# FireMines/zk_stark_project

Hardware: AMD Instinct MI355X
Metric: STARK proofs/sec + prove-time ms, MiMC AIR 2^20-step trace (higher is better)
Workload: dtype f128 (u128 mod 2^128-45*2^40+1); 1 GPU; MiMC AIR 2^20-step trace, blowup=8 (BASELINE configs[1]); trace_length=1048576, trace_width=1, blowup=8, num_queries=40, grinding=21, fri_folding=16, fri_remainder_max_degree=7, parallelism=replicas1

## Files before the change

### __graft_entry__.py

```python
import os
import subprocess
import sys

ROOT = os.path.dirname(os.path.abspath(__file__))


def build() -> None:
    env = dict(os.environ)
    jobs = str(min(16, os.cpu_count() or 1))
    subprocess.check_call(["make", "-j", jobs, "-C", os.path.join(ROOT, "zk_stark_project_amd", "csrc")], env=env)
    subprocess.check_call(["make", "-j", jobs, "-C", os.path.join(ROOT, "oracle")], env=env)
    subprocess.check_call(["make", "-j", jobs, "-C", os.path.join(ROOT, "tests", "native")], env=env)
    subprocess.check_call(["make", "-j", jobs, "-C", os.path.join(ROOT, "tests", "native"), "-f", "deep_inv_check.mk"],
                          env=env)
    subprocess.check_call(["make", "-j", jobs, "-C", os.path.join(ROOT, "tests", "native"), "-f",
                           "column_degrees_check.mk"], env=env)
    if ROOT not in sys.path:
        sys.path.insert(0, ROOT)
    import zk_stark_project_amd
    from zk_stark_project_amd import _native
    _native.load()


def smoke() -> None:
    for p in (ROOT, os.path.join(ROOT, "tests")):
        if p not in sys.path:
            sys.path.insert(0, p)
    from zk_stark_project_amd import AIR_MIMC, MimcProver, ProofOptions, _native
    from zk_stark_project_amd.field import to_bytes
    import oracle_ref

    ctx = _native.Context(0)
    opts = ProofOptions(40, 8, 12)
    prover = MimcProver(opts, ctx)
    n = 1 << 12
    trace = prover.build_trace(42 * 10**6, n)
    pub = prover.get_pub_inputs(trace).to_elements()
    proof = prover.prove(trace)
    ref, _ = oracle_ref.prove(AIR_MIMC, trace.to_bytes(), 1, n, to_bytes(pub), opts)
    assert proof.to_bytes() == ref, "GPU proof differs from the CPU oracle"
    assert oracle_ref.verify(AIR_MIMC, proof.to_bytes(), to_bytes(pub), opts) == 0, "proof rejected"
    _native.verify(AIR_MIMC, proof.to_bytes(), pub, opts)
    ctx.close()
    print(f"smoke ok: MiMC 2^12 proof, {len(proof)} bytes, bit-exact vs oracle")


if __name__ == "__main__":
    build()
    if len(sys.argv) > 1 and sys.argv[1] == "smoke":
        smoke()
```

### zk_stark_project_amd/csrc/abi.cpp

```cpp
#include "prover_internal.hpp"

#include <mutex>

using namespace zkpi;

namespace {
bool device_is_gfx950(int device) {
  static std::mutex mu;
  static std::map<int, bool> known;
  std::lock_guard<std::mutex> lk(mu);
  auto it = known.find(device);
  if (it != known.end()) return it->second;
  hipDeviceProp_t prop;
  if (hipGetDeviceProperties(&prop, device) != hipSuccess) return false;
  const bool ok = strncmp(prop.gcnArchName, "gfx950", 6) == 0;
  known[device] = ok;
  return ok;
}

constexpr uint32_t TU_STATE = TU_W / 2;

int tu_build(zkp_ctx* ctx, const zkp_training_client* cl, uint32_t K, uint64_t bs, uint64_t n) {
  HIP_CHECK(hipSetDevice(ctx->device));
  ctx->err.clear();
// ... 63 lines not shown
  const TuClient* dcl = (const TuClient*)dp;
  const felt* dinit = (const felt*)(dp + off_init);
  if (bs)
    launch_tu_states(ctx->prof, ctx->stream, dcl, K, dinit, (const felt*)(dp + off_batch), ds, (uint32_t)bs,
                     inv(felt_u64(TU_AC * 1000000ull)));
  const felt* states = bs ? ds : dinit;
  launch_tu_write(ctx->prof, ctx->stream, dcl, K, states, bs, n, dfl);
  bool want_fl = false, want_raw = false;
  for (uint32_t k = 0; k < K; k++) {
    want_fl |= cl[k].first_last != nullptr;
    want_raw |= cl[k].raw_states != nullptr;
  }
  const size_t fl_bytes = (size_t)K * 2 * TU_STATE * 16, raw_bytes = (size_t)K * (bs + 1) * TU_STATE * 16;
  uint8_t* hp = (uint8_t*)ctx->pinned((want_fl ? fl_bytes : 0) + (want_raw ? raw_bytes : 0));
  uint8_t* hraw = hp + (want_fl ? fl_bytes : 0);
  if (want_fl) HIP_CHECK(hipMemcpyAsync(hp, dfl, fl_bytes, hipMemcpyDeviceToHost, ctx->stream));
  if (want_raw) HIP_CHECK(hipMemcpyAsync(hraw, states, raw_bytes, hipMemcpyDeviceToHost, ctx->stream));
  ctx->sync();
  for (uint32_t k = 0; k < K; k++) {
    if (cl[k].first_last) memcpy(cl[k].first_last, hp + (size_t)k * 2 * TU_STATE * 16, 2 * TU_STATE * 16);
    if (cl[k].raw_states)
      memcpy(cl[k].raw_states, hraw + (size_t)k * (bs + 1) * TU_STATE * 16, (bs + 1) * TU_STATE * 16);
  }
  ctx->collect_prof();
  ctx->free_retired();
  return 0;
}
}

extern "C" {

int zkp_ctx_create(int device, zkp_ctx** out) {
  if (!out) return ZKP_ERR_ARGUMENT;
  *out = nullptr;
  using clk = std::chrono::steady_clock;
  auto t = clk::now();
  std::vector<std::pair<const char*, double>> phases;
  auto lap = [&](const char* name) {
    const auto now = clk::now();
    phases.emplace_back(name, std::chrono::duration<double, std::milli>(now - t).count());
    t = now;
  };
  int count = 0;
  if (hipGetDeviceCount(&count) != hipSuccess || count <= device || device < 0) return ZKP_ERR_DEVICE;
  if (hipSetDevice(device) != hipSuccess) return ZKP_ERR_DEVICE;
  if (!device_is_gfx950(device)) return ZKP_ERR_DEVICE;
  lap("host_ctx_device_check");
  zkp_ctx* c = new_ctx(device);
  if (!c) return ZKP_ERR_DEVICE;
  lap("host_ctx_streams");
  preload_kernels_module();
  preload_merkle_module();
  preload_ntt_module();
  lap("host_ctx_code_objects");
  try {
    c->pinned(1u << 20);
    lap("host_ctx_pinned");
    const felt zero[1]{};
    c->upload(c->buf<felt>("ring_warm", 1), zero, 16);
    drain_streams(c);
    lap("host_ctx_first_copy");
  } catch (const ZkpFail& f) {
    delete c;
    return f.code;
  }
  for (auto& ph : phases) {
    auto& st = c->stats[ph.first];
    st.launches += 1;
    st.ms += ph.second;
  }
  *out = c;
  return ZKP_OK;
}

void zkp_ctx_destroy(zkp_ctx* ctx) {
  if (!ctx) return;
  (void)hipSetDevice(ctx->device);
  for (zkp_ctx* sc : ctx->session_pool) {
    drain_streams(sc);
    delete sc;
  }
  ctx->session_pool.clear();
  drain_streams(ctx);
  delete ctx;
}

int zkp_ctx_trim(zkp_ctx* ctx) {
  if (!ctx) return ZKP_ERR_ARGUMENT;
  (void)hipSetDevice(ctx->device);
  for (zkp_ctx* sc : ctx->session_pool) {
    drain_streams(sc);
    delete sc;
  }
  ctx->session_pool.clear();
  return ZKP_OK;
}

const char* zkp_last_error(const zkp_ctx* ctx) { return ctx ? ctx->err.c_str() : "null context"; }

void zkp_free(void* p) { free(p); }

int zkp_device_alloc(zkp_ctx* ctx, uint64_t bytes, void** d_ptr) {
  return guarded(ctx, [&] {
    if (!d_ptr) return (int)ZKP_ERR_ARGUMENT;
    HIP_CHECK(hipSetDevice(ctx->device));
    HIP_CHECK(hipMalloc(d_ptr, bytes ? bytes : 16));
    ctx->user_allocs.push_back(*d_ptr);
    return 0;
  });
}

int zkp_device_free(zkp_ctx* ctx, void* d_ptr) {
  return guarded(ctx, [&] {
    auto it = std::find(ctx->user_allocs.begin(), ctx->user_allocs.end(), d_ptr);
    if (it == ctx->user_allocs.end()) return (int)ZKP_ERR_ARGUMENT;
    ctx->user_allocs.erase(it);
    HIP_CHECK(hipFree(d_ptr));
    return 0;
  });
}

int zkp_copy_to_device(zkp_ctx* ctx, void* d_dst, const void* h_src, uint64_t bytes) {
  return guarded(ctx, [&] {
    HIP_CHECK(hipMemcpyAsync(d_dst, h_src, bytes, hipMemcpyHostToDevice, ctx->stream));
    ctx->sync();
    return 0;
  });
}

int zkp_copy_to_host(zkp_ctx* ctx, void* h_dst, const void* d_src, uint64_t bytes) {
  return guarded(ctx, [&] {
    ctx->download(h_dst, d_src, bytes);
    return 0;
  });
}

int zkp_trace_lde_commit(zkp_ctx* ctx, const zkp_felt* trace, uint32_t w, uint64_t n, uint32_t blowup,
                         zkp_felt* lde_out, uint8_t root[32]) {
  return guarded(ctx, [&] {
    HIP_CHECK(hipSetDevice(ctx->device));
    if (!trace || !root) return (int)ZKP_ERR_ARGUMENT;
    if (n < 8 || (n & (n - 1)) || w == 0 || w > 255) return (int)ZKP_ERR_TRACE_SHAPE;
    if (blowup < 2 || (blowup & (blowup - 1)) || blowup > 128) return (int)ZKP_ERR_INVALID_OPTIONS;
    uint32_t logn = ilog2(n), logB = ilog2(blowup);
    if (logn + logB > MAX_LOG_DOMAIN) return (int)ZKP_ERR_TRACE_SHAPE;
    uint64_t N = n * blowup;
    felt* d = ctx->buf<felt>("trace_in", (size_t)w * n);
    ctx->upload(d, trace, (size_t)w * n * 16);
    felt* coef = ctx->buf<felt>("coef", (size_t)w * n);
    felt* lde = ctx->buf<felt>("tlde", (size_t)w * N);
    ctx->ensure_coset(logn, logB, 1);
    const uint32_t logN = logn + logB;
    NttBatch ib{d, coef, nullptr, n, n, 1, 1, w};
    launch_ntt(ctx->prof, ctx->stream, ib, logn, false, ctx->itws(logN), logN);
    NttBatch lb{coef, lde, ctx->S(logn, logB), n, n, blowup, blowup, w * blowup};
    launch_ntt(ctx->prof, ctx->stream, lb, logn, true, ctx->tws(logN), logN);
    TreeShard tr;
    commit_rows(ctx, ctx->self_comm(), 0, lde, n, w, logB, logn, false, "ttree", tr, root);
    if (lde_out) {
      std::vector<felt> h((size_t)w * N);
      ctx->download(h.data(), lde, h.size() * 16);
      for (uint32_t c = 0; c < w; c++)
        for (uint64_t i = 0; i < N; i++) {
          felt v = h[((size_t)c * blowup + (i & (blowup - 1))) * n + (i >> logB)];
          lde_out[(size_t)c * N + i].lo = v.lo;
          lde_out[(size_t)c * N + i].hi = v.hi;
        }
    }
    ctx->collect_prof();
    return 0;
  });
}

int zkp_merkle_commit_rows(zkp_ctx* ctx, const zkp_felt* cols, uint32_t w, uint64_t rows, uint8_t root[32]) {
  return guarded(ctx, [&] {
    HIP_CHECK(hipSetDevice(ctx->device));
    if (!cols || !root) return (int)ZKP_ERR_ARGUMENT;
    if (rows < 2 || (rows & (rows - 1)) || w == 0 || w > 255) return (int)ZKP_ERR_TRACE_SHAPE;
    felt* d = ctx->buf<felt>("mrows", (size_t)w * rows);
    ctx->upload(d, cols, (size_t)w * rows * 16);
    uint32_t* tree = ctx->buf<uint32_t>("mtree", (size_t)16 * rows);
    launch_merkle_lde(ctx->prof, ctx->stream, d, w, 0, rows, tree, rows);
    ctx->download(root, tree + 8, 32);
    ctx->collect_prof();
    return 0;
  });
}

int zkp_grind(zkp_ctx* ctx, const uint8_t seed[32], uint32_t bits, uint64_t* nonce) {
  return guarded(ctx, [&] {
    HIP_CHECK(hipSetDevice(ctx->device));
    if (!seed || !nonce || bits > 64) return (int)ZKP_ERR_ARGUMENT;
    uint32_t sw[8];
    for (int i = 0; i < 8; i++)
      sw[i] = (uint32_t)seed[4 * i] | ((uint32_t)seed[4 * i + 1] << 8) | ((uint32_t)seed[4 * i + 2] << 16) |
              ((uint32_t)seed[4 * i + 3] << 24);
    unsigned long long* dres = ctx->buf<unsigned long long>("grind_res", 1);
    uint32_t* dseed = ctx->buf<uint32_t>("grind_seed", 8);
    ctx->upload(dseed, sw, 32);
    HIP_CHECK(hipMemsetAsync(dres, 0xff, 8, ctx->stream));
    unsigned long long res = ~0ull;
    for (uint64_t base = 1; base <= (1ull << 40) && res == ~0ull; base += 1ull << 32) {
      launch_grind_all(ctx->prof, ctx->stream, dseed, base, base + (1ull << 32) - 1, bits, dres);
      ctx->download(&res, dres, 8);
    }
    if (res == ~0ull) return (int)ZKP_ERR_NONCE;
    *nonce = res;
    ctx->collect_prof();
    return 0;
  });
}

int zkp_build_global_update_trace(zkp_ctx* ctx, const zkp_felt* raw_global, const zkp_felt* blinding,
                                  const zkp_felt* local_updates, uint64_t ndev, zkp_felt k, uint64_t n,
                                  void* d_trace_out, zkp_felt* final_state) {
  return guarded(ctx, [&] {
    HIP_CHECK(hipSetDevice(ctx->device));
    if (!raw_global || !blinding || !d_trace_out || (ndev && !local_updates)) return (int)ZKP_ERR_ARGUMENT;
    if (n < 8 || (n & (n - 1)) || n < ndev + 2) return (int)ZKP_ERR_TRACE_SHAPE;
    const felt kf = make(k.lo, k.hi);
    if (ge_p(kf)) return (int)ZKP_ERR_PUB_INPUTS;
    auto canon = [](const zkp_felt* v, uint64_t cnt) {
      for (uint64_t i = 0; i < cnt; i++)
        if (ge_p(make(v[i].lo, v[i].hi))) return false;
      return true;
    };
    if (!canon(raw_global, GU_D) || !canon(blinding, GU_D) || !canon(local_updates, ndev * GU_D))
      return (int)ZKP_ERR_ARGUMENT;
    std::vector<felt> hm(2 * GU_D);
    for (uint32_t c = 0; c < GU_D; c++) {
      hm[c] = add(make(raw_global[c].lo, raw_global[c].hi), make(blinding[c].lo, blinding[c].hi));
      hm[GU_D + c] = make(raw_global[c].lo, raw_global[c].hi);
    }
    felt* dm = ctx->buf<felt>("gu_masked_raw", 2 * GU_D);
    ctx->upload(dm, hm.data(), hm.size() * 16);
    felt* dl = ctx->buf<felt>("gu_local", ndev ? ndev * GU_D : 1);
    if (ndev) HIP_CHECK(hipMemcpyAsync(dl, local_updates, ndev * GU_D * 16, hipMemcpyHostToDevice, ctx->stream));
    const uint64_t tiles = (n + 4095) / 4096;
    felt* tb = ctx->buf<felt>("gu_tiles", tiles * GU_D);
    launch_gu_trace(ctx->prof, ctx->stream, dm, dm + GU_D, dl, ndev, inv(kf), n, tb, (felt*)d_trace_out);
    if (final_state)
      HIP_CHECK(hipMemcpy2DAsync(final_state, 16, (const felt*)d_trace_out + ndev + 1, n * 16, 16, GU_D,
                                 hipMemcpyDeviceToHost, ctx->stream));
    ctx->sync();
    ctx->collect_prof();
    return 0;
  });
}

int zkp_build_training_update_trace(zkp_ctx* ctx, const zkp_felt* initial_state, const zkp_felt* x_batch,
                                    const zkp_felt* x_sign, const zkp_felt* y_batch, uint64_t bs,
                                    zkp_felt learning_rate, zkp_felt precision, const uint64_t* masks, uint64_t n,
                                    void* d_trace_out, zkp_felt* first_last, zkp_felt* raw_states) {
  return guarded(ctx, [&] {
    if (!masks) return (int)ZKP_ERR_ARGUMENT;
    zkp_training_client c{};
    c.initial_state = initial_state;
    c.x_batch = x_batch;
    c.x_sign = x_sign;
    c.y_batch = y_batch;
    c.learning_rate = learning_rate;
    c.precision = precision;
    c.masks = masks;
    c.d_trace_out = d_trace_out;
    c.first_last = first_last;
    c.raw_states = raw_states;
    return tu_build(ctx, &c, 1, bs, n);
  });
}

int zkp_build_training_update_traces(zkp_ctx* ctx, const zkp_training_client* clients, uint32_t num_clients,
                                     uint64_t bs, uint64_t n) {
  return guarded(ctx, [&] {
    if (!clients || num_clients == 0 || num_clients > ZKP_TU_MAX_CLIENTS) {
      ctx->err = "clients must be non-null and 1.." + std::to_string(ZKP_TU_MAX_CLIENTS) + " in number";
      return (int)ZKP_ERR_ARGUMENT;
    }
    return tu_build(ctx, clients, num_clients, bs, n);
  });
}

int zkp_pcg64_masks(const uint64_t state[2], const uint64_t inc[2], uint64_t first_index, uint64_t count,
                    uint64_t* out) {
  if (!state || !inc || (count && !out)) return ZKP_ERR_ARGUMENT;
  pcg::u128 s{state[0], state[1]}, a{pcg::MUL_LO, pcg::MUL_HI}, c{inc[0], inc[1]};
  const pcg::u128 step_a = a, step_c = c;
  for (uint64_t k = first_index; k; k >>= 1) {
    if (k & 1) s = pcg::affine(s, a, c);
    c = pcg::mul(c, pcg::add(a, {1, 0}));
    a = pcg::mul(a, a);
  }
  for (uint64_t i = 0; i < count; i++) {
    s = pcg::affine(s, step_a, step_c);
    out[i] = pcg::out(s);
  }
  return ZKP_OK;
}

int zkp_set_profiling(zkp_ctx* ctx, int enabled) {
  return guarded(ctx, [&] {
    ctx->prof.enabled = enabled != 0;
    return 0;
  });
}

int zkp_set_profiling_kernel(zkp_ctx* ctx, const char* kernel_name) {
  return guarded(ctx, [&] {
    ctx->prof.only = kernel_name ? kernel_name : "";
    return 0;
// ... 40 lines not shown
}

int zkp_air_check_trace_device_pub(zkp_ctx* ctx, int air_id, const zkp_felt* pub_elems, uint64_t n_pub,
                                   const void* d_trace_cols, uint32_t width, uint64_t n, uint64_t* bad_row,
                                   uint32_t* bad_constraint, uint32_t* bad_assertion) {
  if (!ctx || !d_trace_cols || !bad_row || !bad_constraint || !bad_assertion || (n_pub && !pub_elems))
    return ZKP_ERR_ARGUMENT;
  return guarded(ctx, [&] {
    if (air_id == ZKP_AIR_MIMC || air_id == ZKP_AIR_GLOBAL_UPDATE || air_id == ZKP_AIR_TRAINING_UPDATE)
      return (int)ZKP_ERR_UNSUPPORTED_AIR;
    if (n < 8 || (n & (n - 1)) || width == 0 || width > 255) return (int)ZKP_ERR_TRACE_SHAPE;
    AirDesc air;
    std::vector<felt> pub(n_pub);
    for (uint64_t i = 0; i < n_pub; i++) pub[i] = make(pub_elems[i].lo, pub_elems[i].hi);
    const int rc = build_air(air, air_id, width, n, pub);
    if (rc) return rc;
    if (!air.prog->num_pub && n_pub) return (int)ZKP_ERR_PUB_INPUTS;
    if (n > (1ull << MAX_LOG_TRACE)) return (int)ZKP_ERR_TRACE_SHAPE;
    const airp::Program& pr = *air.prog;
    HIP_CHECK(hipSetDevice(ctx->device));
    const ProgCodeLayout lay(pr, 1);
    const size_t A = pr.a_col.size(), o_col = lay.end();
    static_assert(sizeof(ProgStridedCells) == 48, "three 16-byte units");
    const std::vector<airp::Strided>& sv = pr.strided;
    const size_t S = sv.size();
    size_t seq_felts = 0;
    for (const airp::Strided& a : sv) seq_felts += a.pub < 0 ? a.values.size() : 0;
    const size_t o_step = o_col + (A + 3) / 4, o_val = o_step + (A + 3) / 4, o_sdesc = o_val + A,
                 o_svals = o_sdesc + 3 * S, total = o_svals + seq_felts;
    uint64_t strided_blocks = 0;
    for (const airp::Strided& a : sv) strided_blocks += (n / a.stride + 63) / 64;
    felt* dimg = ctx->buf<felt>("check_image", total);
    std::vector<felt>& tag = ctx->host_cache["check_image_tag"];
    const felt want = make((uint64_t)air_id | (S ? n << 32 : 0), total);
    if (tag.size() != 1 || !eq(tag[0], want)) {
      tag.clear();
      std::vector<felt> img(total, zero());
      lay.write(img.data());
      for (size_t p = 0; p < pr.periodic.size(); p++)
        memcpy(img.data() + lay.tab[p], pr.periodic[p].data(), pr.periodic[p].size() * 16);
      uint32_t* steps = reinterpret_cast<uint32_t*>(img.data() + o_step);
      for (size_t k = 0; k < A; k++) steps[k] = (uint32_t)pr.a_step[k];
      if (A) {
        memcpy(img.data() + o_col, pr.a_col.data(), A * 4);
        if (!pr.num_pub) memcpy(img.data() + o_val, pr.a_val.data(), A * 16);
      }
      ProgStridedCells* cells = reinterpret_cast<ProgStridedCells*>(img.data() + o_sdesc);
      uint32_t blk = 0, voff = 0;
      for (size_t j = 0; j < S; j++) {
        const uint32_t count = (uint32_t)(n / sv[j].stride);
        const bool bound = sv[j].pub >= 0;
        cells[j] = ProgStridedCells{sv[j].col, (uint32_t)sv[j].first, (uint32_t)sv[j].stride, count, blk,
                                    sv[j].sequence() ? voff : 0xffffffffu, bound ? (uint32_t)sv[j].pub + 1 : 0, 0,
                                    bound ? zero() : sv[j].val};
        if (sv[j].sequence() && !bound) {
          memcpy(img.data() + o_svals + voff, sv[j].values.data(), (size_t)count * 16);
          voff += count;
        }
        blk += (count + 63) / 64;
      }
      ctx->upload(dimg, img.data(), total * 16);
      if (total * 16 > (1u << 20)) ctx->sync();
      tag.assign(1, want);
    }
    ProgCheckArgs ca{};
    ca.code = lay.code(dimg);
    ca.nassert = (uint32_t)A;
    ca.a_col = reinterpret_cast<const uint32_t*>(dimg + o_col);
    ca.a_step = reinterpret_cast<const uint32_t*>(dimg + o_step);
    ca.a_val = dimg + o_val;
    if (pr.num_pub) {
      felt* dpub = ctx->buf<felt>("check_pub", pr.num_pub);
      ctx->upload(dpub, pr.pub.data(), (size_t)pr.num_pub * 16);
      ca.code.pub = dpub;
      felt* dval = ctx->buf<felt>("check_aval", A);
      if (A) ctx->upload(dval, pr.a_val.data(), A * 16);
      ca.a_val = dval;
    }
    ca.n = n;
    ca.nstrided = (uint32_t)S;
    ca.sdesc = reinterpret_cast<const ProgStridedCells*>(dimg + o_sdesc);
    ca.svals = dimg + o_svals;
    unsigned long long* dres = ctx->buf<unsigned long long>("check_result", 2);
    HIP_CHECK(hipMemsetAsync(dres, 0xff, 16, ctx->stream));
    launch_check_program(ctx->prof, ctx->stream, ca, width, (const felt*)d_trace_cols, dres, strided_blocks);
    unsigned long long res[2];
    ctx->download(res, dres, 16);
    ctx->collect_prof();
    ctx->free_retired();
    *bad_row = UINT64_MAX;
    *bad_constraint = UINT32_MAX;
    *bad_assertion = UINT32_MAX;
    if (res[0] != ~0ull) {
      *bad_row = res[0] >> 10;
      *bad_constraint = (uint32_t)(res[0] & 1023);
    } else if (res[1] != ~0ull) {
      *bad_row = res[1] & 0xffffffffull;
      *bad_assertion = (uint32_t)(res[1] >> 32);
    }
    return 0;
  });
}

int zkp_air_constraint_degrees_device(zkp_ctx* ctx, int air_id, const zkp_felt* pub_elems, uint64_t n_pub,
                                      const void* d_trace_cols, uint32_t width, uint64_t n, uint64_t* degrees,
                                      uint32_t capacity, zkp_air_degree_report* report) {
  return guarded(ctx, [&] {
    if (!d_trace_cols || !degrees || !report || (n_pub && !pub_elems)) {
      ctx->err = "d_trace_cols, degrees, report or (with n_pub set) pub_elems: null";
      return (int)ZKP_ERR_ARGUMENT;
    }
    DegreesPlan pl;
    const int rc = degrees_plan(air_id, pub_elems, n_pub, width, n, pl, ctx->err);
    if (rc) return rc;
    const airp::Program& pr = *pl.air.prog;
    if (capacity < pr.num_t) {
      ctx->err = "capacity: below num_constraints (" + std::to_string(pr.num_t) + ")";
      return (int)ZKP_ERR_ARGUMENT;
    }
    HIP_CHECK(hipSetDevice(ctx->device));
    const uint32_t E = pl.E, logE = ilog2(E), logn = ilog2(n), logN = logn + logE;
    const uint64_t M = n * E;
    ctx->ensure_coset(logn, logE, logE);
    const ProgCodeLayout lay(pr, E);
    const size_t total = lay.end();
    felt* dimg = ctx->buf<felt>("deg_image", total);
    std::vector<felt>& tag = ctx->host_cache["deg_image_tag"];
    const felt want[2] = {make((uint64_t)air_id, logn), make(logE, total)};
    if (tag.size() != 2 || !eq(tag[0], want[0]) || !eq(tag[1], want[1])) {
      tag.clear();
      std::vector<felt> img(total, zero());
      lay.write(img.data());
      const felt g = felt_u64(3);
      for (size_t p = 0; p < pr.periodic.size(); p++) {
        const size_t cyc = pr.periodic[p].size();
        std::vector<felt> kc = pr.periodic[p];
        host_interpolate(kc, one());
        const std::vector<felt> kv = host_evaluate(kc, cyc * E, pow_u64(g, n / cyc));
        memcpy(img.data() + lay.tab[p], kv.data(), kv.size() * 16);
      }
      ctx->upload(dimg, img.data(), total * 16);
      if (total * 16 > (1u << 20)) ctx->sync();
      tag.assign(want, want + 2);
    }
    ProgCode code = lay.code(dimg);
    if (pr.num_pub) {
      felt* dpub = ctx->buf<felt>("deg_pub", pr.num_pub);
      ctx->upload(dpub, pr.pub.data(), (size_t)pr.num_pub * 16);
      code.pub = dpub;
    }
    felt* coef = ctx->buf<felt>("deg_coef", (size_t)width * n);
    felt* ext = ctx->buf<felt>("deg_ext", (size_t)width * M);
    NttBatch ib{(const felt*)d_trace_cols, coef, nullptr, n, n, 1, 1, width};
    launch_ntt(ctx->prof, ctx->stream, ib, logn, false, ctx->itws(logN), logN);
    NttBatch lb{coef, ext, ctx->S(logn, logE), n, n, E, E, width * E};
    launch_ntt(ctx->prof, ctx->stream, lb, logn, true, ctx->tws(logN), logN);
    const std::string dkey = "deg_dft_" + std::to_string(logn) + "_" + std::to_string(logE);
    felt* dcoefs = ctx->buf<felt>(dkey + "_coefs", (size_t)E + E / 2);
    uint32_t* dblk = ctx->buf<uint32_t>(dkey + "_blk", E);
    if (!ctx->have_cached(dkey)) {
      const std::vector<felt> dc = comp_dft_consts(n, logE, E);
      std::vector<uint32_t> blk(E);
      for (uint32_t u = 0; u < E; u++) blk[u] = u;
      ctx->upload(dcoefs, dc.data(), dc.size() * 16);
      ctx->upload(dblk, blk.data(), blk.size() * 4);
    }
    const uint32_t K = std::min(pl.K, pr.num_t);
    felt* vals = ctx->buf<felt>("deg_vals", (size_t)K * M);
    felt* cf = ctx->buf<felt>("deg_coefs", (size_t)K * M);
    long long* ddeg = ctx->buf<long long>("deg_result", pr.num_t);
    HIP_CHECK(hipMemsetAsync(ddeg, 0xff, (size_t)pr.num_t * 8, ctx->stream));
    for (uint32_t i0 = 0; i0 < pr.num_t; i0 += K) {
      const uint32_t k = std::min(K, pr.num_t - i0);
      launch_program_columns(ctx->prof, ctx->stream, code, ext, width, logn, logE, i0, k, vals);
      NttBatch cb{vals, vals, nullptr, n, n, 1, 1, k * E};
      launch_ntt(ctx->prof, ctx->stream, cb, logn, false, ctx->itws(logN), logN);
      for (uint32_t c = 0; c < k; c++)
        launch_comp_dft(ctx->prof, ctx->stream, vals + (size_t)c * M, dblk, ctx->Si(logn, logE, logE), dcoefs, E, E,
                        logn, 0, n, cf + (size_t)c * M);
      launch_column_degrees(ctx->prof, ctx->stream, cf, logn, logE, k, ddeg + i0);
    }
    std::vector<uint64_t> h(pr.num_t);
    ctx->download(h.data(), ddeg, (size_t)pr.num_t * 8);
    ctx->collect_prof();
    ctx->free_retired();
    zkp_air_degree_report r{};
    r.num_constraints = pr.num_t;
    r.eval_blowup = E;
    r.columns = pl.air.comp_cols();
    r.max_degree = ZKP_DEGREE_ZERO;
    r.first_under = UINT32_MAX;
    for (uint32_t i = 0; i < pr.num_t; i++) {
      degrees[i] = h[i];
      if (h[i] == ZKP_DEGREE_ZERO) continue;
      if (r.max_degree == ZKP_DEGREE_ZERO || h[i] > r.max_degree) r.max_degree = h[i];
      if (r.first_under == UINT32_MAX && h[i] > (uint64_t)pr.degrees[i] * (n - 1)) r.first_under = i;
    }
    r.columns_needed = 1;
    r.proof_fits = 1;
    if (r.max_degree != ZKP_DEGREE_ZERO) {
      if (r.max_degree + 2 > n) r.columns_needed = (uint32_t)((r.max_degree + 2 - n + n - 1) / n);
      if (r.columns_needed < 1) r.columns_needed = 1;
      r.proof_fits = r.max_degree <= ((uint64_t)r.columns + 1) * n - 2;
    }
    *report = r;
    return 0;
  });
}

int zkp_build_mimc_trace(const uint8_t seed[16], uint64_t n, zkp_felt* out) {
  if (!seed || !out || n == 0) return ZKP_ERR_ARGUMENT;
  felt v = from_u128_bytes(seed);
  if (ge_p(v)) v = sub(v, make(P_LO, P_HI));
  for (uint64_t i = 0; i < n; i++) {
    out[i].lo = v.lo;
    out[i].hi = v.hi;
    felt u = add(v, felt_u64((i % 64 + 1) * 1000000ull));
    felt u2 = sqr(u), u3 = mul(u2, u), u6 = sqr(u3);
    v = mul(u6, u);
  }
  return 0;
}

}
```

### zk_stark_project_amd/csrc/felt_dev.hpp

```cpp
#pragma once
#include <stdint.h>

#define ZKP_ASM asm

namespace fpd {

__device__ __forceinline__ uint32_t add_co(uint32_t a, uint32_t b, uint64_t& co) {
  uint32_t r;
  ZKP_ASM("v_add_co_u32_e64 %0, %1, %2, %3" : "=v"(r), "=s"(co) : "v"(a), "v"(b));
  return r;
}
__device__ __forceinline__ uint32_t addc_co(uint32_t a, uint32_t b, uint64_t ci, uint64_t& co) {
  uint32_t r;
  ZKP_ASM("v_addc_co_u32_e64 %0, %1, %2, %3, %4" : "=v"(r), "=s"(co) : "v"(a), "v"(b), "s"(ci));
  return r;
}
__device__ __forceinline__ uint32_t addc(uint32_t a, uint32_t b, uint64_t ci) {
  uint32_t r;
  uint64_t dead;
  ZKP_ASM("v_addc_co_u32_e64 %0, %1, %2, %3, %4" : "=v"(r), "=s"(dead) : "v"(a), "v"(b), "s"(ci));
  return r;
}
__device__ __forceinline__ uint32_t sub_co(uint32_t a, uint32_t b, uint64_t& bo) {
  uint32_t r;
// ... 244 lines not shown
  const uint64_t u = mul_wide(r4, 0x2d00u);
  uint64_t c, b;
  const uint32_t s1 = add_co(r1, (uint32_t)u, c);
  const uint32_t s2 = addc_co(r2, (uint32_t)(u >> 32), c, c);
  const uint32_t s3 = addc_co_0(r3, c, c);
  const uint32_t z0 = sub_co(r0, r4, b);
  const uint32_t z1 = subb_co_0(s1, b, b);
  const uint32_t z2 = subb_co_0(s2, b, b);
  const uint32_t z3 = subb_co_0(s3, b, b);
  uint64_t kk;
  ZKP_ASM("s_andn2_b64 %0, %1, %2" : "=s"(kk) : "s"(c), "s"(b) : "scc");
  return canon_rare(z0, z1, z2, z3, kk);
}


__device__ __forceinline__ void mul256x2(L4 x, L4 y, L4 u, L4 v, uint32_t r[8], uint32_t s[8]) {
  uint64_t acc, c, bcc, d;
  uint32_t ov, bov;
  acc = mul_wide(x.w0, y.w0);
  bcc = mul_wide(u.w0, v.w0);
  r[0] = (uint32_t)acc; acc >>= 32;
  s[0] = (uint32_t)bcc; bcc >>= 32;
#define ZKP_COL_BEGIN(i0, j0)                      \
  acc = mad_co(x.w##i0, y.w##j0, acc, c);          \
  bcc = mad_co(u.w##i0, v.w##j0, bcc, d);          \
  ov = carry_0(c);                                 \
  bov = carry_0(d);
#define ZKP_COL_STEP(i0, j0)                       \
  acc = mad_co(x.w##i0, y.w##j0, acc, c);          \
  bcc = mad_co(u.w##i0, v.w##j0, bcc, d);          \
  ov = addc_0(ov, c);                              \
  bov = addc_0(bov, d);
#define ZKP_COL_END(k)                             \
  r[k] = (uint32_t)acc;                            \
  s[k] = (uint32_t)bcc;                            \
  acc = (acc >> 32) | ((uint64_t)ov << 32);        \
  bcc = (bcc >> 32) | ((uint64_t)bov << 32);
  ZKP_COL_BEGIN(0, 1) ZKP_COL_STEP(1, 0) ZKP_COL_END(1)
  ZKP_COL_BEGIN(0, 2) ZKP_COL_STEP(1, 1) ZKP_COL_STEP(2, 0) ZKP_COL_END(2)
  ZKP_COL_BEGIN(0, 3) ZKP_COL_STEP(1, 2) ZKP_COL_STEP(2, 1) ZKP_COL_STEP(3, 0) ZKP_COL_END(3)
  ZKP_COL_BEGIN(1, 3) ZKP_COL_STEP(2, 2) ZKP_COL_STEP(3, 1) ZKP_COL_END(4)
  ZKP_COL_BEGIN(2, 3) ZKP_COL_STEP(3, 2) ZKP_COL_END(5)
#undef ZKP_COL_BEGIN
#undef ZKP_COL_STEP
#undef ZKP_COL_END
  acc = mad(x.w3, y.w3, acc);
  bcc = mad(u.w3, v.w3, bcc);
  r[6] = (uint32_t)acc; r[7] = (uint32_t)(acc >> 32);
  s[6] = (uint32_t)bcc; s[7] = (uint32_t)(bcc >> 32);
}

__device__ __forceinline__ void reduce_x2_core(const uint32_t r[8], const uint32_t s[8], uint32_t z[4], uint32_t Z[4],
                                               uint64_t& k1, uint64_t& k2) {
  const uint32_t K = 0x2d00u;
  uint64_t t = mul_wide(r[4], K), tt = mul_wide(s[4], K);
  uint32_t q0 = (uint32_t)t, p0 = (uint32_t)tt;
  t = mad(r[5], K, t >> 32); tt = mad(s[5], K, tt >> 32);
  uint32_t q1 = (uint32_t)t, p1 = (uint32_t)tt;
  t = mad(r[6], K, t >> 32); tt = mad(s[6], K, tt >> 32);
  uint32_t q2 = (uint32_t)t, p2 = (uint32_t)tt;
  t = mad(r[7], K, t >> 32); tt = mad(s[7], K, tt >> 32);
  uint32_t q3 = (uint32_t)t, q4 = (uint32_t)(t >> 32), p3 = (uint32_t)tt, p4 = (uint32_t)(tt >> 32);
  uint64_t c, e, b, f;
  uint32_t s1 = add_co(r[1], q0, c);
  uint32_t S1 = add_co(s[1], p0, e);
  uint32_t x0 = sub_co(r[0], r[4], b);
  uint32_t X0 = sub_co(s[0], s[4], f);
  uint32_t s2 = addc_co(r[2], q1, c, c);
  uint32_t S2 = addc_co(s[2], p1, e, e);
  uint32_t x1 = subb_co(s1, r[5], b, b);
  uint32_t X1 = subb_co(S1, s[5], f, f);
  uint32_t s3 = addc_co(r[3], q2, c, c);
  uint32_t S3 = addc_co(s[3], p2, e, e);
  uint32_t x2 = subb_co(s2, r[6], b, b);
  uint32_t X2 = subb_co(S2, s[6], f, f);
  uint32_t s4 = addc_co_0(q3, c, c);
  uint32_t S4 = addc_co_0(p3, e, e);
  uint32_t x3 = subb_co(s3, r[7], b, b);
  uint32_t X3 = subb_co(S3, s[7], f, f);
  uint32_t s5 = addc_0(q4, c);
  uint32_t S5 = addc_0(p4, e);
  uint32_t x4 = subb_co_0(s4, b, b);
  uint32_t X4 = subb_co_0(S4, f, f);
  uint32_t x5 = subb_0(s5, b);
  uint32_t X5 = subb_0(S5, f);
  uint64_t uu = mul_wide(x4, K), UU = mul_wide(X4, K);
  uint32_t u0 = (uint32_t)uu, U0 = (uint32_t)UU;
  uint32_t u1 = (uint32_t)(uu >> 32) + x5 * K, U1 = (uint32_t)(UU >> 32) + X5 * K;
  uint32_t y1 = add_co(x1, u0, c);
  uint32_t Y1 = add_co(X1, U0, e);
  z[0] = sub_co(x0, x4, b);
  Z[0] = sub_co(X0, X4, f);
  uint32_t y2 = addc_co(x2, u1, c, c);
  uint32_t Y2 = addc_co(X2, U1, e, e);
  z[1] = subb_co(y1, x5, b, b);
  Z[1] = subb_co(Y1, X5, f, f);
  uint32_t y3 = addc_co_0(x3, c, c);
  uint32_t Y3 = addc_co_0(X3, e, e);
  z[2] = subb_co_0(y2, b, b);
  Z[2] = subb_co_0(Y2, f, f);
  z[3] = subb_co_0(y3, b, b);
  Z[3] = subb_co_0(Y3, f, f);
  ZKP_ASM("s_andn2_b64 %0, %1, %2" : "=s"(k1) : "s"(c), "s"(b) : "scc");
  ZKP_ASM("s_andn2_b64 %0, %1, %2" : "=s"(k2) : "s"(e), "s"(f) : "scc");
}

__device__ __forceinline__ void reduce_x2(const uint32_t r[8], const uint32_t s[8], felt& out_r, felt& out_s) {
  uint32_t z[4], Z[4];
  uint64_t k1, k2;
  reduce_x2_core(r, s, z, Z, k1, k2);
  const uint64_t rare = k1 | k2 | __builtin_amdgcn_ballot_w64(max(z[3], Z[3]) == 0xffffffffu);
  if (rare) {
    out_r = canon_from(z[0], z[1], z[2], z[3], k1);
    out_s = canon_from(Z[0], Z[1], Z[2], Z[3], k2);
  } else {
    out_r = join(z[0], z[1], z[2], z[3]);
    out_s = join(Z[0], Z[1], Z[2], Z[3]);
  }
}

__device__ __forceinline__ void mul_x2(felt a, felt b, felt c, felt d, felt& ab, felt& cd) {
  uint32_t r[8], s[8];
  mul256x2(split(a), split(b), split(c), split(d), r, s);
  reduce_x2(r, s, ab, cd);
}

struct Rare {
  uint64_t k = 0;
  uint32_t top = 0;
  __device__ __forceinline__ bool any() const { return (k | __builtin_amdgcn_ballot_w64(top == 0xffffffffu)) != 0; }
};

__device__ __forceinline__ felt mul_z(felt a, felt b, Rare& q) {
  uint32_t r[8], z0, z1, z2, z3;
  uint64_t k;
  mul256(split(a), split(b), r);
  reduce_core(r, z0, z1, z2, z3, k);
  q.k |= k;
  q.top = max(q.top, z3);
  return join(z0, z1, z2, z3);
}

__device__ __forceinline__ void mul_x2_z(felt a, felt b, felt c, felt d, felt& ab, felt& cd, Rare& q) {
  uint32_t r[8], s[8], z[4], Z[4];
  uint64_t k1, k2;
  mul256x2(split(a), split(b), split(c), split(d), r, s);
  reduce_x2_core(r, s, z, Z, k1, k2);
  q.k |= k1 | k2;
  q.top = max(q.top, max(z[3], Z[3]));
  ab = join(z[0], z[1], z[2], z[3]);
  cd = join(Z[0], Z[1], Z[2], Z[3]);
}

__device__ __forceinline__ felt add_z(felt a, felt b, Rare& q) {
  L4 x = split(a), y = split(b);
  uint64_t c, g;
  const uint32_t s0 = add_co(x.w0, y.w0, c);
  const uint32_t s1 = addc_co(x.w1, y.w1, c, c);
  const uint32_t s2 = addc_co(x.w2, y.w2, c, c);
  const uint32_t s3 = addc_co(x.w3, y.w3, c, c);
  q.top = max(q.top, s3);
  const uint32_t m0 = sel_0_m1(c), m1 = m0 & C1;
  const uint32_t t0 = add_co(s0, m0, g);
  const uint32_t t1 = addc_co(s1, m1, g, g);
  const uint32_t t2 = addc_co_0(s2, g, g);
  const uint32_t t3 = addc_0(s3, g);
  return join(t0, t1, t2, t3);
}
}
```

### zk_stark_project_amd/csrc/kernels_common.hpp

```cpp
#pragma once
#include "../../include/zkp.h"
#include "zkp_internal.hpp"
#include "blake3.hpp"

#include <algorithm>
#include <type_traits>

using namespace fp;

#define TPB 256

#define LAUNCH(prof, name, stream, bytes, ...)                 \
  do {                                                          \
    (prof).begin(name, stream, (double)(bytes));                \
    __VA_ARGS__;                                                \
    (prof).end(stream);                                         \
  } while (0)

#if defined(__HIP_DEVICE_COMPILE__)
using Rare = fpd::Rare;
#else
struct Rare {
  bool any() const { return false; }
};
#endif

template <bool FAST>
__device__ __forceinline__ felt dmul(felt a, felt b, Rare& q) {
#if defined(__HIP_DEVICE_COMPILE__)
  if constexpr (FAST) return fpd::mul_z(a, b, q);
#endif
  (void)q;
  return mul(a, b);
}
template <bool FAST>
__device__ __forceinline__ felt dadd(felt a, felt b, Rare& q) {
#if defined(__HIP_DEVICE_COMPILE__)
  if constexpr (FAST) return fpd::add_z(a, b, q);
#endif
  (void)q;
  return add(a, b);
}

namespace kc {

template <bool FAST>
__device__ __forceinline__ uint32_t opaque_tid() {
  uint32_t t = threadIdx.x;
  if constexpr (!FAST) asm volatile("" : "+v"(t));
  return t;
}

__device__ __forceinline__ uint32_t rev_bits(uint32_t x, uint32_t bits) {
  return bits == 0 ? 0u : (__brev(x) >> (32 - bits));
}

template <int B, int E, typename F>
__device__ __forceinline__ void static_for(F&& f) {
  if constexpr (B < E) {
    f(std::integral_constant<int, B>{});
    static_for<B + 1, E>(f);
  }
}

constexpr int ilog2_const(int v) { return v <= 1 ? 0 : 1 + ilog2_const(v / 2); }
constexpr int rev_const(int x, int bits) { return bits == 0 ? 0 : ((x & 1) << (bits - 1)) | rev_const(x >> 1, bits - 1); }

inline uint32_t ilog2_u64(uint64_t v) {
  uint32_t l = 0;
  while ((1ull << l) < v) l++;
  return l;
}

}
```

### zk_stark_project_amd/csrc/ntt.hip

```cpp
#include "kernels_common.hpp"
#include "ntt_plan.hpp"

#include <mutex>

using kc::static_for;
using kc::rev_bits;

namespace {

struct NttKArgs {
  const felt* src;
  felt* dst;
  const felt* scale;
  const felt* tw;
  uint64_t src_stride, dst_stride;
  uint32_t src_div, scale_mod;
  uint32_t logn, s0, K, lo, T, Tl, logT, logTl, dit;
};

__global__ __launch_bounds__(TPB) void k_ntt_pass(NttKArgs a) {
  extern __shared__ felt lds[];
  const uint32_t bidx = blockIdx.y;
  const felt* src = a.src + (uint64_t)(bidx / a.src_div) * a.src_stride;
  felt* dst = a.dst + (uint64_t)bidx * a.dst_stride;
  const felt* scale = a.scale ? a.scale + ((uint64_t)(bidx % a.scale_mod) << a.logn) : nullptr;
  const uint32_t K = a.K, T = a.T, Tl = a.Tl, lo = a.lo;
  const uint32_t E = T << K;
  const uint64_t g0 = (uint64_t)blockIdx.x * T;
  const uint64_t hi0 = g0 >> lo;
  const uint64_t l0 = (Tl == T) ? (g0 & ((1ull << lo) - 1)) : 0;
  const uint32_t qmask = (1u << K) - 1;

  for (uint32_t e = threadIdx.x; e < E; e += TPB) {
    uint32_t ll = e & (Tl - 1);
    uint32_t rest = e >> a.logTl;
    uint32_t q = rest & qmask;
    uint32_t hl = rest >> K;
    uint64_t addr = ((hi0 + hl) << (lo + K)) + ((uint64_t)q << lo) + l0 + ll;
    felt v = src[addr];
    if (scale) v = mul(v, scale[addr]);
    lds[(q << a.logT) + (hl * Tl) + ll] = v;
  }
  __syncthreads();
  for (uint32_t ls = 0; ls < K; ls++) {
    const uint32_t s = a.s0 + ls;
    const uint32_t pbit = a.dit ? ls : (K - 1 - ls);
    const uint32_t lev = a.dit ? s : (a.logn - 1 - s);
    const felt* twl = a.tw + ((1ull << lev) - 1);
    const uint32_t pmask = (1u << pbit) - 1;
    for (uint32_t bf = threadIdx.x; bf < (E >> 1); bf += TPB) {
      uint32_t gg = bf & (T - 1);
      uint32_t qq = bf >> a.logT;
      uint32_t q = ((qq >> pbit) << (pbit + 1)) | (qq & pmask);
      uint32_t q2 = q | (1u << pbit);
      uint64_t l = l0 + (gg & (Tl - 1));
      uint64_t j = ((uint64_t)(q & pmask) << lo) | l;
      felt w = twl[j];
      uint32_t i0 = (q << a.logT) + gg, i1 = (q2 << a.logT) + gg;
      felt x = lds[i0], y = lds[i1];
      if (a.dit) {
        felt t = mul(y, w);
        lds[i0] = add(x, t);
        lds[i1] = sub(x, t);
      } else {
        lds[i0] = add(x, y);
        lds[i1] = mul(sub(x, y), w);
      }
    }
    __syncthreads();
  }
  for (uint32_t e = threadIdx.x; e < E; e += TPB) {
    uint32_t ll = e & (Tl - 1);
    uint32_t rest = e >> a.logTl;
    uint32_t q = rest & qmask;
    uint32_t hl = rest >> K;
    uint64_t addr = ((hi0 + hl) << (lo + K)) + ((uint64_t)q << lo) + l0 + ll;
    dst[addr] = lds[(q << a.logT) + (hl * Tl) + ll];
  }
}

struct Ntt8Args {
  const felt* src;
  felt* dst;
  const felt* scale;
  const felt* tw;
  uint64_t src_stride, dst_stride;
  uint32_t src_div, scale_mod;
  uint32_t logn, s0, K, lo, logT, logTl;
  uint32_t tile_major;
};

template <bool DIT>
__device__ __forceinline__ felt ntt_tw(const Ntt8Args& a, uint32_t j, uint32_t pbit) {
  uint32_t s = DIT ? a.s0 + pbit : a.s0 + a.K - 1 - pbit;
  uint32_t lev = DIT ? s : a.logn - 1 - s;
  return a.tw[((1u << lev) - 1) + j];
}

#ifdef ZKP_NTT_NOGMEM
#define NTT_LD(p) (make((uint64_t)(uintptr_t)(p), (uint64_t)threadIdx.x))
#define NTT_ST(p, v)                                               \
  do {                                                            \
    const felt v_ = (v);                                          \
    if (v_.lo == 0x123456789ull && v_.hi == 0xabcdefull) *(p) = v_; \
  } while (0)
#else
#define NTT_LD(p) (*(p))
#define NTT_ST(p, v) (*(p) = (v))
#endif

#ifdef ZKP_NTT_NOBFLY
template <bool FAST>
__device__ __forceinline__ felt bmul(felt a, felt b, Rare& q) { return make(a.lo ^ b.lo, a.hi ^ b.hi); }
template <bool FAST>
__device__ __forceinline__ felt badd(felt a, felt b, Rare& q) { return make(a.lo + b.lo, a.hi + b.hi); }
__device__ __forceinline__ felt nsub(felt a, felt b) { return make(a.lo - b.lo, a.hi - b.hi); }
#else
template <bool FAST>
__device__ __forceinline__ felt bmul(felt a, felt b, Rare& q) { return dmul<FAST>(a, b, q); }
template <bool FAST>
__device__ __forceinline__ felt badd(felt a, felt b, Rare& q) { return dadd<FAST>(a, b, q); }
__device__ __forceinline__ felt nsub(felt a, felt b) { return sub(a, b); }
#endif

template <bool DIT, bool FAST>
__device__ __forceinline__ void bfly(felt& x, felt& y, felt w, Rare& q) {
  if (DIT) {
    felt t = bmul<FAST>(y, w, q);
    y = nsub(x, t);
    x = badd<FAST>(x, t, q);
  } else {
    felt d = nsub(x, y);
    x = badd<FAST>(x, y, q);
    y = bmul<FAST>(d, w, q);
  }
}

template <bool DIT, bool FAST>
__device__ __forceinline__ void bfly1(felt& x, felt& y, Rare& q) {
  felt d = nsub(x, y);
  x = badd<FAST>(x, y, q);
  y = d;
}

#ifdef ZKP_COUNT_REDO
__device__ unsigned long long zkp_ntt_redo_waves[5];
#define ZKP_NTT_REDO_TAKEN(site)                                                       \
  do {                                                                                 \
    if ((threadIdx.x & 63) == 0) atomicAdd(&zkp_ntt_redo_waves[site], 1ull);           \
  } while (0)
#else
#define ZKP_NTT_REDO_TAKEN(site) \
  do {                           \
  } while (0)
#endif

template <int K>
struct NttRounds {
  static constexpr int n = (K + 2) / 3;
  static constexpr int bits(int r) {
    int rem = K;
    for (int i = 0; i < r; i++) {
      int left = n - i;
      int b = (rem + left - 1) / left;
      rem -= b > 3 ? 3 : b;
    }
    int left = n - r;
    int b = (rem + left - 1) / left;
    return b > 3 ? 3 : b;
  }
};

template <bool DIT, bool FAST>
__device__ __forceinline__ void bfly2(felt& x0, felt& y0, felt w0, felt& x1, felt& y1, felt w1, Rare& q) {
#if defined(__HIP_DEVICE_COMPILE__) && !defined(ZKP_NTT_NOBFLY)
  auto mx2 = [&](felt a, felt b, felt c, felt d, felt& ab, felt& cd) {
    if constexpr (FAST) fpd::mul_x2_z(a, b, c, d, ab, cd, q);
    else fpd::mul_x2(a, b, c, d, ab, cd);
  };
  if (DIT) {
    felt t0, t1;
    mx2(y0, w0, y1, w1, t0, t1);
    y0 = sub(x0, t0); x0 = badd<FAST>(x0, t0, q);
    y1 = sub(x1, t1); x1 = badd<FAST>(x1, t1, q);
  } else {
    felt d0 = sub(x0, y0), d1 = sub(x1, y1);
    x0 = badd<FAST>(x0, y0, q); x1 = badd<FAST>(x1, y1, q);
    mx2(d0, w0, d1, w1, y0, y1);
  }
#else
  bfly<DIT, FAST>(x0, y0, w0, q);
  bfly<DIT, FAST>(x1, y1, w1, q);
#endif
}

template <bool DIT, int NT, int KC, bool SMALL>
__device__ __forceinline__ void ntt8_tile(const Ntt8Args& a, uint32_t bidx, uint32_t tile, felt* lds) {
  constexpr int E = NT * 8;
  constexpr uint32_t K = KC;
  constexpr uint32_t LOGNT = NT == 512 ? 9 : 8;
  constexpr uint32_t logT = LOGNT + 3 - KC;
  constexpr uint32_t T = 1u << logT;
  static_assert(T == 1 || T >= 4, "the LDS swizzles take rows of 1 or >= 4 felts");
  const uint32_t Tl = 1u << a.logTl, lo = a.lo;
  auto lidx = [](uint32_t q, uint32_t x) -> uint32_t {
    if constexpr (T == 1) {
      (void)x;
      return q ^ ((q >> 3) & 7u) ^ (((q >> 6) & 1u) << 3);
    } else if constexpr (T >= 32) {
      return q * T + (x ^ (q & 15u));
    } else if constexpr (T == 16 && DIT) {
      return q * T + (x ^ (q & 7u));
    } else if constexpr (T == 16) {
      return q * T + (x ^ ((q & 7u) | ((((q >> 2) ^ (q >> 4)) & 1u) << 3)));
    } else if constexpr (T == 8) {
      return (q ^ (((q >> 2) ^ (q >> 3)) & 1u)) * T + (x ^ (q & 7u));
    } else {
      const uint32_t b1 = (q >> 1) & 1u, b23 = ((q >> 2) ^ (q >> 3)) & 1u, b25 = ((q >> 2) ^ (q >> 5)) & 1u;
      return (q ^ (b23 | (b25 << 1))) * T + (x ^ (b1 | (b23 << 1)));
    }
  };
  const felt* src = a.src + (uint64_t)(bidx / a.src_div) * a.src_stride;
  felt* dst = a.dst + (uint64_t)bidx * a.dst_stride;
  const felt* scale = a.scale ? a.scale + ((uint64_t)(bidx % a.scale_mod) << a.logn) : nullptr;
  const uint64_t g0 = (uint64_t)tile << logT;
  const uint32_t hi0 = (uint32_t)(g0 >> lo);
  const uint32_t l0 = (Tl == T) ? (uint32_t)(g0 & ((1ull << lo) - 1)) : 0;
  const uint32_t qmask = (1u << K) - 1;
  const uint32_t tid = threadIdx.x;

  auto gaddr = [&](uint32_t gg, uint32_t q) -> uint32_t {
    uint32_t hl = gg >> a.logTl, ll = gg & (Tl - 1);
    return ((hi0 + hl) << (lo + K)) + (q << lo) + l0 + ll;
  };
  (void)qmask;
  const bool staged = a.logTl < (T >= 8 ? 3u : 2u);
  auto staged_elem = [&](uint32_t e, uint32_t& slot) -> uint32_t {
    uint32_t ll = e & (Tl - 1), rest = e >> a.logTl;
    uint32_t q = rest & ((1u << K) - 1), hl = rest >> K;
    slot = lidx(q, hl * Tl + ll);
    return ((hi0 + hl) << (lo + K)) + (q << lo) + l0 + ll;
  };
  if (staged) {
    auto stage_in = [&](auto fast_c, Rare& q) {
      constexpr bool FAST = decltype(fast_c)::value;
#pragma unroll
      for (int i = 0; i < 8; i++) {
        uint32_t slot;
        uint32_t ad = staged_elem(tid + i * NT, slot);
        felt v = NTT_LD(src + ad);
        if (scale) v = bmul<FAST>(v, NTT_LD(scale + ad), q);
        lds[slot] = v;
      }
    };
    Rare q;
    stage_in(std::true_type{}, q);
    if (scale && q.any()) {
      ZKP_NTT_REDO_TAKEN(0);
      stage_in(std::false_type{}, q);
    }
    __syncthreads();
  }
  uint32_t b0 = DIT ? 0 : K;
  static_for<0, NttRounds<KC>::n>([&](auto rr) {
    constexpr int r = decltype(rr)::value;
    constexpr uint32_t rb = NttRounds<KC>::bits(r);
    if (!DIT) b0 -= rb;
    constexpr bool first = r == 0, last = r + 1 == NttRounds<KC>::n;
    if (!first) __syncthreads();
    felt x[8];
    uint32_t ggs[2], qlow[2];
    auto coord_gg = [&](int m, uint32_t tr) { return ((uint32_t)(m >> rb) << LOGNT | tr) & (T - 1); };
    auto coord_q = [&](int m, uint32_t tr) {
      uint32_t extra = m >> rb, bf = m & ((1u << rb) - 1);
      uint32_t qo = ((extra << LOGNT) | tr) >> logT;
      uint32_t ql = qo & ((1u << b0) - 1);
      return ((qo >> b0) << (b0 + rb)) | (bf << b0) | ql;
    };
    auto round = [&](auto fast_c, Rare& qq) {
    constexpr bool FAST = decltype(fast_c)::value;
    uint32_t tr = tid;
    if constexpr (!FAST) asm volatile("" : "+v"(tr));
    const uint32_t zo = tr - tid;
#pragma unroll
    for (int m = 0; m < 8; m++) {
      uint32_t extra = m >> rb, bf = m & ((1u << rb) - 1);
      uint32_t c = (extra << LOGNT) | tr;
      if (first && !staged) {
        uint32_t ad = gaddr(coord_gg(m, tr), coord_q(m, tr));
        felt v = NTT_LD(src + ad);
        if (scale) v = bmul<FAST>(v, NTT_LD(scale + ad), qq);
        x[m] = v;
      } else {
        x[m] = lds[lidx(coord_q(m, tr), coord_gg(m, tr))];
      }
      if (bf == 0 && extra < 2) { ggs[extra] = c & (T - 1); qlow[extra] = (c >> logT) & ((1u << b0) - 1); }
    }
    if constexpr (rb == 3) {
      const uint32_t l = l0 + (ggs[0] & (Tl - 1));
      const uint32_t jb = (qlow[0] << lo) | l;
      const uint32_t jstep = 1u << (b0 + lo);
      constexpr bool smallest = SMALL && (DIT ? first : last);
      if constexpr (DIT && smallest) {
        bfly1<true, FAST>(x[0], x[1], qq); bfly1<true, FAST>(x[2], x[3], qq); bfly1<true, FAST>(x[4], x[5], qq); bfly1<true, FAST>(x[6], x[7], qq);
        const felt w1 = ntt_tw<true>(a, 1 + zo, 1);
        bfly1<true, FAST>(x[0], x[2], qq); bfly1<true, FAST>(x[4], x[6], qq);
        bfly2<true, FAST>(x[1], x[3], w1, x[5], x[7], w1, qq);
        const felt w21 = ntt_tw<true>(a, 1 + zo, 2), w22 = ntt_tw<true>(a, 2 + zo, 2), w23 = ntt_tw<true>(a, 3 + zo, 2);
        bfly1<true, FAST>(x[0], x[4], qq);
        bfly2<true, FAST>(x[1], x[5], w21, x[2], x[6], w22, qq);
        bfly<true, FAST>(x[3], x[7], w23, qq);
      } else if constexpr (!DIT && smallest) {
        const felt w21 = ntt_tw<false>(a, 1 + zo, 2), w22 = ntt_tw<false>(a, 2 + zo, 2), w23 = ntt_tw<false>(a, 3 + zo, 2);
        bfly1<false, FAST>(x[0], x[4], qq);
        bfly2<false, FAST>(x[1], x[5], w21, x[2], x[6], w22, qq);
        bfly<false, FAST>(x[3], x[7], w23, qq);
        const felt w1 = ntt_tw<false>(a, 1 + zo, 1);
        bfly1<false, FAST>(x[0], x[2], qq); bfly1<false, FAST>(x[4], x[6], qq);
        bfly2<false, FAST>(x[1], x[3], w1, x[5], x[7], w1, qq);
        bfly1<false, FAST>(x[0], x[1], qq); bfly1<false, FAST>(x[2], x[3], qq); bfly1<false, FAST>(x[4], x[5], qq); bfly1<false, FAST>(x[6], x[7], qq);
      } else if constexpr (DIT) {
        {
          felt w0 = ntt_tw<true>(a, jb, b0);
          bfly2<true, FAST>(x[0], x[1], w0, x[2], x[3], w0, qq); bfly2<true, FAST>(x[4], x[5], w0, x[6], x[7], w0, qq);
        }
        {
          felt w1a = ntt_tw<true>(a, jb, b0 + 1);
          felt w1b = ntt_tw<true>(a, jb | jstep, b0 + 1);
          bfly2<true, FAST>(x[0], x[2], w1a, x[1], x[3], w1b, qq); bfly2<true, FAST>(x[4], x[6], w1a, x[5], x[7], w1b, qq);
        }
        static_for<0, 2>([&](auto k2) {
          felt w2a = ntt_tw<true>(a, jb | ((uint32_t)(2 * k2) << (b0 + lo)), b0 + 2);
          felt w2b = ntt_tw<true>(a, jb | ((uint32_t)(2 * k2 + 1) << (b0 + lo)), b0 + 2);
          bfly2<true, FAST>(x[2 * k2], x[2 * k2 + 4], w2a, x[2 * k2 + 1], x[2 * k2 + 5], w2b, qq);
        });
      } else {
        static_for<0, 2>([&](auto k2) {
          felt w2a = ntt_tw<false>(a, jb | ((uint32_t)(2 * k2) << (b0 + lo)), b0 + 2);
          felt w2b = ntt_tw<false>(a, jb | ((uint32_t)(2 * k2 + 1) << (b0 + lo)), b0 + 2);
          bfly2<false, FAST>(x[2 * k2], x[2 * k2 + 4], w2a, x[2 * k2 + 1], x[2 * k2 + 5], w2b, qq);
        });
        {
          felt w1a = ntt_tw<false>(a, jb, b0 + 1);
          felt w1b = ntt_tw<false>(a, jb | jstep, b0 + 1);
          bfly2<false, FAST>(x[0], x[2], w1a, x[1], x[3], w1b, qq); bfly2<false, FAST>(x[4], x[6], w1a, x[5], x[7], w1b, qq);
        }
        {
          felt w0 = ntt_tw<false>(a, jb, b0);
          bfly2<false, FAST>(x[0], x[1], w0, x[2], x[3], w0, qq); bfly2<false, FAST>(x[4], x[5], w0, x[6], x[7], w0, qq);
        }
      }
    } else if constexpr (rb == 2) {
      if constexpr (!DIT && SMALL && last) {
        const felt w1 = ntt_tw<false>(a, 1 + zo, 1);
#pragma unroll
        for (int u = 0; u < 2; u++) {
          felt* y = x + 4 * u;
          bfly1<false, FAST>(y[0], y[2], qq);
          bfly<false, FAST>(y[1], y[3], w1, qq);
          bfly1<false, FAST>(y[0], y[1], qq); bfly1<false, FAST>(y[2], y[3], qq);
        }
      } else {
#pragma unroll
      for (int u = 0; u < 2; u++) {
        const uint32_t l = l0 + (ggs[u] & (Tl - 1));
        const uint32_t jb = (qlow[u] << lo) | l;
        felt w0 = ntt_tw<DIT>(a, jb, b0);
        felt w1a = ntt_tw<DIT>(a, jb, b0 + 1), w1b = ntt_tw<DIT>(a, jb | (1u << (b0 + lo)), b0 + 1);
        felt* y = x + 4 * u;
        if (DIT) {
          bfly2<true, FAST>(y[0], y[1], w0, y[2], y[3], w0, qq);
          bfly2<true, FAST>(y[0], y[2], w1a, y[1], y[3], w1b, qq);
        } else {
          bfly2<false, FAST>(y[0], y[2], w1a, y[1], y[3], w1b, qq);
          bfly2<false, FAST>(y[0], y[1], w0, y[2], y[3], w0, qq);
        }
      }
      }
    } else {
#pragma unroll
      for (int u = 0; u < 4; u++) {
        uint32_t c = ((uint32_t)u << LOGNT) | tr;
        uint32_t gg = c & (T - 1);
        uint32_t ql = (c >> logT) & ((1u << b0) - 1);
        const uint32_t jb = (ql << lo) | (l0 + (gg & (Tl - 1)));
        bfly<DIT, FAST>(x[2 * u], x[2 * u + 1], ntt_tw<DIT>(a, jb, b0), qq);
      }
    }
    };
    Rare qq;
    round(std::true_type{}, qq);
    if (qq.any()) {
      ZKP_NTT_REDO_TAKEN(1 + r);
      round(std::false_type{}, qq);
    }
    if (!last || staged) __syncthreads();
#pragma unroll
    for (int m = 0; m < 8; m++) {
      if (last && !staged) NTT_ST(dst + gaddr(coord_gg(m, tid), coord_q(m, tid)), x[m]);
      else lds[lidx(coord_q(m, tid), coord_gg(m, tid))] = x[m];
    }
    if (DIT) b0 += rb;
  });
  if (staged) {
    __syncthreads();
#pragma unroll
    for (int i = 0; i < 8; i++) {
      uint32_t slot;
      uint32_t ad = staged_elem(tid + i * NT, slot);
      NTT_ST(dst + ad, lds[slot]);
    }
  }
  (void)E;
}

template <bool DIT, int NT, int KC, bool SMALL>
__global__ __launch_bounds__(NT, (NT == 256 && KC == 11) ? 5 : 1) void k_ntt8(Ntt8Args a) {
  extern __shared__ felt lds[];
  uint32_t bidx = blockIdx.x, tile = blockIdx.y;
  if (a.tile_major) {
    const uint32_t B = gridDim.x, i = blockIdx.y * B + blockIdx.x, k = i >> 3;
    tile = (k / B) * 8 + (i & 7);
    bidx = k % B;
  }
  ntt8_tile<DIT, NT, KC, SMALL>(a, bidx, tile, lds);
}

}

void preload_ntt_module() {
  hipFuncAttributes fa;
  (void)hipFuncGetAttributes(&fa, (const void*)k_ntt_pass);
}

#ifdef ZKP_COUNT_REDO
void zkp_ntt_redo_waves_take(unsigned long long out[5]) {
  const unsigned long long z[5] = {0, 0, 0, 0, 0};
  (void)hipMemcpyFromSymbol(out, HIP_SYMBOL(zkp_ntt_redo_waves), sizeof z);
  (void)hipMemcpyToSymbol(HIP_SYMBOL(zkp_ntt_redo_waves), z, sizeof z);
}
int zkp_ntt_round_bits(int K, int r) {
  switch (K) {
#define ZKP_ROUND_BITS(KK) \
  case KK:                 \
    return r < NttRounds<KK>::n ? NttRounds<KK>::bits(r) : 0;
    ZKP_ROUND_BITS(6) ZKP_ROUND_BITS(7) ZKP_ROUND_BITS(8) ZKP_ROUND_BITS(9) ZKP_ROUND_BITS(11)
#undef ZKP_ROUND_BITS
  }
  return -1;
}
#endif

static void launch_ntt_radix2(Prof& prof, hipStream_t s, const NttBatch& b, uint32_t logn, bool dit,
                              const felt* tw) {
  bool first = true;
  for (const NttPass& ps : ntt_plan(logn, dit, b.batches)) {
    NttKArgs a;
    a.src = first ? b.src : b.dst;
    a.dst = b.dst;
    a.scale = first ? b.scale : nullptr;
    a.tw = tw;
    a.src_stride = first ? b.src_stride : b.dst_stride;
    a.dst_stride = b.dst_stride;
    a.src_div = first ? b.src_div : 1;
    a.scale_mod = b.scale_mod ? b.scale_mod : 1;
    a.logn = logn;
    a.s0 = ps.s0;
    a.K = ps.K;
    a.lo = ps.lo;
    a.T = 1u << ps.logT;
    a.Tl = 1u << ps.logTl;
    a.logT = ps.logT;
    a.logTl = ps.logTl;
    a.dit = dit ? 1 : 0;
    uint64_t groups = 1ull << (logn - ps.K);
    dim3 grid((uint32_t)(groups >> ps.logT), b.batches);
    size_t shmem = (size_t)(a.T << ps.K) * sizeof(felt);
    LAUNCH(prof, dit ? "ntt_dit_r2" : "ntt_dif_r2", s, (double)b.batches * (1ull << logn) * 16.0 * (a.scale ? 3 : 2),
           hipLaunchKernelGGL(k_ntt_pass, grid, dim3(TPB), shmem, s, a));
    first = false;
  }
}

#define ZKP_NTT8_KERNELS(X)                                                                \
  X(true, 256, 6, true) X(true, 256, 8, true) X(true, 256, 11, true)                       \
  X(true, 256, 6, false) X(true, 256, 7, false) X(true, 256, 8, false)                     \
  X(true, 256, 9, false) X(true, 512, 9, false)                                            \
  X(false, 256, 6, true) X(false, 256, 7, true) X(false, 256, 8, true) X(false, 256, 11, true) \
  X(false, 256, 6, false) X(false, 256, 7, false) X(false, 256, 8, false)                  \
  X(false, 256, 9, false) X(false, 512, 9, false)

void launch_ntt(Prof& prof, hipStream_t s, const NttBatch& b, uint32_t logn, bool dit, const felt* tw,
                uint32_t logN, int only_pass) {
  if (logN > 28)
    launch_fail(ZKP_ERR_TRACE_SHAPE, "NTT domain over 2^28 points (n * blowup)");
  if (logn < 11) {
    if (only_pass <= 0) launch_ntt_radix2(prof, s, b, logn, dit, tw);
    return;
  }
  static std::mutex attr_mu;
  static uint64_t attr_devs = 0;
  int dev = 0;
  (void)hipGetDevice(&dev);
  {
  std::lock_guard<std::mutex> attr_lock(attr_mu);
  if (!(attr_devs >> (dev & 63) & 1)) {
#define X(D, NT, KK, S) \
  (void)hipFuncSetAttribute((const void*)k_ntt8<D, NT, KK, S>, hipFuncAttributeMaxDynamicSharedMemorySize, NT * 8 * 16);
    ZKP_NTT8_KERNELS(X)
#undef X
    attr_devs |= 1ull << (dev & 63);
  }
  }
  const NttPlan plan = ntt_plan(logn, dit, b.batches);
  for (uint32_t p = 0; p < plan.n; p++) {
    const NttPass& ps = plan.pass[p];
    if (only_pass >= 0 && (uint32_t)only_pass != p) continue;
    Ntt8Args a;
    bool first = p == 0;
    a.src = first ? b.src : b.dst;
    a.dst = b.dst;
    a.scale = first ? b.scale : nullptr;
    a.tw = tw;
    a.src_stride = first ? b.src_stride : b.dst_stride;
    a.dst_stride = b.dst_stride;
    a.src_div = first ? b.src_div : 1;
    a.scale_mod = b.scale_mod ? b.scale_mod : 1;
    a.logn = logn;
    a.s0 = ps.s0;
    a.K = ps.K;
    a.lo = ps.lo;
    a.logT = ps.logT;
    a.logTl = ps.logTl;
    uint64_t groups = 1ull << (logn - ps.K);
    dim3 grid(b.batches, (uint32_t)(groups >> a.logT));
    a.tile_major = first && b.src_div > 1 && grid.y % 8 == 0;
    size_t shmem = (size_t)(1u << ps.K) * (1u << a.logT) * sizeof(felt);
    const double arr = (double)(1ull << logn) * 16.0;
    const uint32_t src_arrays = first ? (b.batches + a.src_div - 1) / a.src_div : b.batches;
    const uint32_t scale_rows = a.scale ? (a.scale_mod < b.batches ? a.scale_mod : b.batches) : 0;
    const double bytes = arr * ((double)src_arrays + scale_rows + b.batches);
    const uint32_t nt = 1u << ps.lognt;
#define X(D, NT, KK, S)                                                              \
  if (dit == D && nt == NT && ps.K == KK && ps.small == S)                           \
    LAUNCH(prof, D ? "ntt_dit" : "ntt_dif", s, bytes,                                \
           hipLaunchKernelGGL((k_ntt8<D, NT, KK, S>), grid, dim3(NT), shmem, s, a)); \
  else
    ZKP_NTT8_KERNELS(X)
    launch_fail(ZKP_ERR_DEVICE, "internal: NTT pass of an unplanned size");
#undef X
  }
}
```

### zk_stark_project_amd/csrc/prover.cpp

```cpp
#include "prover_internal.hpp"

#include <mutex>

using namespace zkpi;

namespace zkpi {

int ProofRun::init(int air_id, const felt* d_trace_in, uint32_t width, uint64_t n_rows, const zkp_felt* pub_elems,
                   uint64_t n_pub, uint8_t** proof, uint64_t* proof_len) {
  d_trace = d_trace_in;
  w = width;
  n = n_rows;
  int rc = check_options(o);
  if (rc) return rc;
  if (n < 8 || (n & (n - 1)) || w == 0 || w > 255) return ZKP_ERR_TRACE_SHAPE;
  if (!proof || !proof_len || (n_pub && !pub_elems)) return ZKP_ERR_ARGUMENT;
  B = o->blowup_factor; F = o->fri_folding_factor;
  logn = ilog2(n); logB = ilog2(B); logN = logn + logB;
  N = 1ull << logN;
  if (logN > MAX_LOG_DOMAIN || logn > MAX_LOG_TRACE) return ZKP_ERR_TRACE_SHAPE;
  rc = check_fri_shape(n, o);
  if (rc) return rc;
  R = (uint32_t)cm->world; rank = (uint32_t)cm->rank;
  if (R == 0 || (R & (R - 1)) || R > B || rank >= R) return ZKP_ERR_ARGUMENT;
  logR = ilog2(R); Bl = B >> logR; logBl = logB - logR; j0 = rank * Bl;
  if (R > 1 && logn < logR + 8) return ZKP_ERR_TRACE_SHAPE;
  pub.resize(n_pub);
  for (uint64_t i = 0; i < n_pub; i++) pub[i] = make(pub_elems[i].lo, pub_elems[i].hi);
  rc = build_air(air, air_id, w, n, pub);
  if (rc) return rc;
  ce = air.ce_blowup(); C = air.comp_cols();
  if (B < ce) return ZKP_ERR_INVALID_OPTIONS;
  logce = ilog2(ce);
  if (ce > 16 || C > ce) return ZKP_ERR_UNSUPPORTED_AIR;
  cstep = logB - logce;
  u0 = ce_first(rank);
  cel = 0;
  while (u0 + cel < ce && ce_owner(u0 + cel) == rank) cel++;
  celmax = ce >= R ? ce / R : 1;
  g = felt_u64(3);
  ood_trace.assign(2 * (size_t)w, felt{});
  ood_comp.assign(C, felt{});
  return 0;
}

void ProofRun::setup() {
  ctx->sync();
  ctx->ring_reset();
  ctx->stage_begin();
  {
    std::vector<felt> se = context_elements(air, o);
    se.insert(se.end(), pub.begin(), pub.end());
    coin.init(se);
  }
  ncoef = air.num_t + (uint32_t)air.num_assertions();
  dt_seed = ctx->buf<uint32_t>("dt_seed", 8);
  dt_cc = ctx->buf<felt>("dt_cc", ncoef);
  dt_zz = ctx->buf<felt>("dt_zz", 2);
  dt_pw = ctx->buf<felt>("dt_pw", 2 * (size_t)logn);
  dt_aval = ctx->buf<felt>("dt_aval", air.a_val.size());
  {
    uint32_t sw[8];
    for (int i = 0; i < 8; i++)
      sw[i] = (uint32_t)coin.seed[4 * i] | ((uint32_t)coin.seed[4 * i + 1] << 8) |
              ((uint32_t)coin.seed[4 * i + 2] << 16) | ((uint32_t)coin.seed[4 * i + 3] << 24);
    ctx->upload(dt_seed, sw, 32);
    if (!air.a_val.empty()) ctx->upload(dt_aval, air.a_val.data(), air.a_val.size() * 16);
  }
  ctx->stage_end("0a_seed");
  ctx->ensure_coset(logn, logB, logce);
  ctx->stage_end("0b_coset");
  Sj0 = ctx->S(logn, logB) + (uint64_t)j0 * n;
  cx = coset_points(ctx, logn, logB, logce);
  twn = ctx->tws(logN) + ((1ull << (logn - 1)) - 1);
  ctx->stage_end("0_setup");
}

void ProofRun::trace_stage(const zkp_felt* h_trace) {
  coef = ctx->buf<felt>("coef", (size_t)(w + C) * n);
  tlde = ctx->buf<felt>("tlde", (size_t)w * Bl * n);
  bool coeffs_drawn = false;
  static const bool no_pair = getenv("ZKP_NO_GU_PAIR") != nullptr;
  paired = allow_shortcuts && !no_pair && air.id == ZKP_AIR_GLOBAL_UPDATE && w == 2 * GU_D && (R == 1 || !h_trace);
  const uint32_t d = w / 2;
  uint32_t wi = paired && R > 1 ? (d + R - 1) / R * R : w;
  uint32_t cpt = (R > 1 && wi % R == 0 && wi >= 2 * R && wi <= w) ? wi / R : 0;
  if (R > 1 && !cpt) wi = w, cpt = (w % R == 0 && w >= 2 * R) ? w / R : 0;
  if (paired) {
    gu_cval = ctx->buf<felt>("gu_cval", d);
    gu_bad = ctx->buf<uint32_t>("gu_bad", 4);
    HIP_CHECK(hipMemsetAsync(gu_bad, 0, 16, st));
    gu_lazy_on = w >= DEEP_COEF_MIN_W;
    gu_lazy = GuLazy{gu_cval, l0_table(), air.k, d, R > 1 && cpt && wi < w ? wi : d,
                     (uint32_t)(air.k.hi == 0 && (air.k.lo >> 32) == 0)};
  }
  if (cpt) {
    trace_column_sharded(h_trace, cpt, wi, d);
  } else {
    if (h_trace && R > 1) h_trace = gather_host_slices(h_trace);
    const uint32_t wd = paired ? d : w;
    std::vector<std::pair<uint32_t, uint32_t>> grp;
    constexpr uint32_t growth = 150;
    if (h_trace && wd >= 4) {
      uint32_t cw = std::min(std::max({1u, w / 40, (uint32_t)((1ull << 19) >> std::min(logn, 19u))}),
                             std::max(1u, wd / 2));
      for (uint32_t c = 0; c < wd;) {
        cw = std::min(cw, wd - c);
        grp.push_back({c, cw});
        c += cw;
        cw = std::max(cw + 1, cw * growth / 100);
      }
    } else {
      grp.push_back({0u, wd});
    }
    const bool late_pairs = paired && h_trace;
    if (paired && !h_trace) grp.push_back({d, d});
    const bool early_pairs = paired && !h_trace && R == 1;
    if (early_pairs) {
      HIP_CHECK(hipEventRecord(ctx->ev_fork, st));
      HIP_CHECK(hipStreamWaitEvent(ctx->side, ctx->ev_fork, 0));
      launch_gu_check(pf, ctx->side, d_trace, d, logn, air.k, 0, d, 0, logn, gu_cval, gu_bad);
      early_check_launch(gu_bad, ctx->side);
    }
    const bool mimc_check = air.id == ZKP_AIR_MIMC && w == 1 && R == 1 && lastcol_shape();
    const bool piped = h_trace && grp.size() > 1;
    const size_t G = grp.size();
    if (piped) {
      ctx->events(G + 2);
      HIP_CHECK(hipEventRecord(ctx->ev_fork, st));
      HIP_CHECK(hipStreamWaitEvent(ctx->side, ctx->ev_fork, 0));
    }
    if (late_pairs) {
      if (!piped) throw ZkpFail{ZKP_ERR_DEVICE, "paired host trace without column groups"};
      HIP_CHECK(hipMemcpy2DAsync(const_cast<felt*>(d_trace) + (size_t)d * n, n * 16, h_trace + (size_t)d * n, n * 16,
                                 16, d, hipMemcpyHostToDevice, ctx->side));
      HIP_CHECK(hipEventRecord(ctx->up_ev[G], ctx->side));
    }
    for (uint32_t g = 0; g < grp.size(); g++) {
      const uint32_t c0 = grp[g].first, cw = grp[g].second;
      felt* dcol = const_cast<felt*>(d_trace) + (size_t)c0 * n;
      if (piped) {
        HIP_CHECK(hipMemcpyAsync(dcol, h_trace + (size_t)c0 * n, (size_t)cw * n * 16, hipMemcpyHostToDevice,
                                 ctx->side));
        HIP_CHECK(hipEventRecord(ctx->up_ev[g], ctx->side));
        HIP_CHECK(hipStreamWaitEvent(st, ctx->up_ev[g], 0));
      } else if (h_trace && g == 0) {
        ctx->upload(dcol, h_trace, (size_t)w * n * 16);
      }
      if (g == 0 && mimc_check) {
        uint32_t* dflag = ctx->buf<uint32_t>("mimc_bad", 4);
        HIP_CHECK(hipEventRecord(ctx->ev_fork, st));
        HIP_CHECK(hipStreamWaitEvent(ctx->side, ctx->ev_fork, 0));
        HIP_CHECK(hipMemsetAsync(dflag, 0, 16, ctx->side));
        launch_mimc_check(pf, ctx->side, d_trace, n, air.a_val[0], air.a_val[1], dflag);
        early_check_launch(dflag, ctx->side);
      }
      if (c0 >= wd && early_pairs) HIP_CHECK(hipStreamWaitEvent(st, ctx->ev_check, 0));
      if (c0 >= wd && early_pairs && early_check_failed()) {
        paired = false;
        gu_lazy_on = false;
      } else if (c0 >= wd) {
        const uint32_t i0 = c0 - d;
        if (!early_pairs) launch_gu_check(pf, st, d_trace, d, logn, air.k, i0, cw, 0, logn, gu_cval, gu_bad);
        launch_gu_coef(pf, st, coef, d, logn, air.k, ctx->itws(logN) + ((n >> 1) - 1), i0, cw, 0, n, gu_cval);
        if (!gu_lazy_on) launch_gu_lde(pf, st, tlde, d, logn, logBl, air.k, i0, cw, gu_cval, l0_table());
        continue;
      }
      NttBatch ib{dcol, coef + (size_t)c0 * n, nullptr, n, n, 1, 1, cw};
      launch_ntt(pf, st, ib, logn, false, ctx->itws(logN), logN);
      NttBatch lb{coef + (size_t)c0 * n, tlde + (size_t)c0 * Bl * n, Sj0, n, n, Bl, Bl, cw * Bl};
      launch_ntt(pf, st, lb, logn, true, ctx->tws(logN), logN);
    }
    if (late_pairs) {
      HIP_CHECK(hipStreamWaitEvent(st, ctx->up_ev[G], 0));
      launch_gu_check(pf, st, d_trace, d, logn, air.k, 0, d, 0, 0, gu_cval, gu_bad);
      launch_gu_coef(pf, st, coef, d, logn, air.k, ctx->itws(logN) + ((n >> 1) - 1), 0, d, 0, n, gu_cval);
      if (!gu_lazy_on) launch_gu_lde(pf, st, tlde, d, logn, logBl, air.k, 0, d, gu_cval, l0_table());
      HIP_CHECK(hipEventRecord(ctx->up_ev[G + 1], ctx->side));
      HIP_CHECK(hipStreamWaitEvent(ctx->copy, ctx->up_ev[G + 1], 0));
      late_h_trace = h_trace;
    }
  }
  {
    MerkleTail draw{};
    draw.op = MERKLE_TAIL_DRAW_COEFFS;
    draw.coin_seed = dt_seed;
    draw.method = o->batching_constraints;
    draw.ncoef = ncoef;
    draw.out = dt_cc;
    const bool late_first = host_channel && late_h_trace && R == 1;
    coeffs_drawn = commit_rows(ctx, cm, 0, tlde, n, w, logB, logn, R > 1, "ttree", ttree, T.trace_root,
                               host_channel && !late_first, host_channel ? nullptr : &draw, nullptr,
                               gu_lazy_on ? &gu_lazy : nullptr);
    if (late_first) {
      late_pairs_upload();
      ctx->download(T.trace_root, ttree.nodes + 8, 32);
      memcpy(ttree.top[1].data(), T.trace_root, 32);
    }
  }
  troot_d = R > 1 ? ttree.top_d + 8 : ttree.nodes + 8;
  if (!coeffs_drawn && !host_channel)
    launch_dt_draw_coeffs(pf, st, dt_seed, troot_d, o->batching_constraints, ncoef, dt_cc);
  ctx->stage_end("1_trace_commit");
}

void ProofRun::constraint_stage() {
  eval_stage();
  composition_stage();
}

void ProofRun::eval_stage() {
  comp = ctx->buf<felt>("comp", (size_t)(cel ? cel : 1) * n);
  constraint_eval(ctx, air, logn, logB, logce, u0, cel, j0, logBl, cx, twn, dt_cc, dt_aval, tlde, comp, coef, cm);
}

bool ProofRun::lastcol_shape() const {
  static const bool no_derive = getenv("ZKP_NO_DERIVE_LAST") != nullptr;
  return allow_shortcuts && !no_derive && logce == logB && C >= 2 && C <= 8 && cel == Bl && u0 == j0;
}

void ProofRun::composition_stage() {
  comp = ctx->buf<felt>("comp", (size_t)(cel ? cel : 1) * n);
  acoef = coef + (size_t)w * n;
  clde = ctx->buf<felt>("clde", (size_t)C * Bl * n);
  bool z_drawn = false;
  wn_root = root_of_unity(logn);
  {
    const uint64_t nR = n >> logR, p0 = (uint64_t)rank * nR;
    const bool derive = lastcol_shape() && !(pre_checked && early_check_failed());
    derive_last = derive;
    if (derive) {
      lc_bad = ctx->buf<uint32_t>("lc_bad", 4);
      HIP_CHECK(hipMemsetAsync(lc_bad, 0, 16, st));
    }
    felt* cint = derive ? ctx->buf<felt>("comp_int", (size_t)(cel ? cel : 1) * n) : comp;
    if (cel) {
      NttBatch ib{comp, cint, nullptr, n, n, 1, 1, cel};
      launch_ntt(pf, st, ib, logn, false, ctx->itws(logN), logN);
    }
    felt* recv = cint;
    if (R > 1) recv = composition_exchange(cint, nR);
    const std::string dkey = "comp_dft_" + std::to_string(logn) + "_" + std::to_string(logce) + "_" +
                             std::to_string(C) + "_" + std::to_string(R) + "_" + std::to_string(celmax);
    felt* dcoefs = ctx->buf<felt>(dkey + "_coefs", (size_t)C + ce / 2);
    uint32_t* dblk = ctx->buf<uint32_t>(dkey + "_blk", ce);
    if (!ctx->have_cached(dkey)) {
      const std::vector<felt> dc = comp_dft_consts(n, logce, C);
      std::vector<uint32_t> blk(ce);
      for (uint32_t u = 0; u < ce; u++) {
        uint32_t s = ce_owner(u);
        blk[u] = s * celmax + (u - ce_first(s));
      }
      ctx->upload(dcoefs, dc.data(), dc.size() * 16);
      ctx->upload(dblk, blk.data(), blk.size() * 4);
    }
    felt* slice = R > 1 ? ctx->buf<felt>("comp_ag_send", (size_t)C * nR) : acoef;
    launch_comp_dft(pf, st, recv, dblk, ctx->Si(logn, logB, logce), dcoefs, ce, C, logn, p0, nR, slice,
                    derive ? lc_bad : nullptr);
    if (R > 1 && derive) {
      lc_flags = ctx->buf<uint32_t>("lc_flags", 4 * (size_t)R);
      cm->all_gather(st, lc_bad, lc_flags, 16);
    }
    if (R > 1) {
      composition_gather_lde(slice, derive, nR, p0);
    } else {
      NttBatch lb{acoef, clde, Sj0, n, n, Bl, Bl, (derive ? C - 1 : C) * Bl};
      launch_ntt(pf, st, lb, logn, true, ctx->tws(logN), logN);
    }
    LastCol lc{};
    if (derive) lc = LastCol{comp, last_col_kappa(ctx, logn, logB, C) + 2 * (size_t)j0, clde + (size_t)(C - 1) * Bl * n};
    MerkleTail draw{};
    draw.op = MERKLE_TAIL_DRAW_Z;
    draw.coin_seed = dt_seed;
    draw.wn = wn_root;
    draw.logn = logn;
    draw.out = dt_zz;
    draw.pw = dt_pw;
    z_drawn = commit_rows(ctx, cm, 0, clde, n, C, logB, logn, R > 1, "ctree", ctree, T.constraint_root,
                          host_channel, host_channel ? nullptr : &draw, derive ? &lc : nullptr);
  }
  croot_d = R > 1 ? ctree.top_d + 8 : ctree.nodes + 8;
  if (!z_drawn && !host_channel) launch_dt_draw_z(pf, st, dt_seed, croot_d, wn_root, logn, dt_zz, dt_pw);
  ctx->stage_end("2_constraints_commit");
}

void ProofRun::ood_values() {
  const uint64_t cnt = (uint64_t)Bl * n;
  deep_inv = ctx->buf<felt>("deep_inv", cnt);
  felt* scratch = ctx->buf<felt>("deep_inv_scratch", deep_den_scratch(cnt));
  const PointMap pm{cx + j0, twn, logn};
  const PointMap pm8{coset_points8(ctx, logn, logB) + j0,
                     logn > 3 ? ctx->tws(logN) + ((1ull << (logn - 4)) - 1) : nullptr, logn - 3};
  const felt w8 = root_of_unity(3), w8_2 = sqr(w8);
  ctx->events(1);
  HIP_CHECK(hipEventRecord(ctx->ev_fork, st));
  HIP_CHECK(hipStreamWaitEvent(ctx->side, ctx->ev_fork, 0));
  HIP_CHECK(hipStreamWaitEvent(ctx->copy, ctx->ev_fork, 0));
  launch_deep_denominators(pf, ctx->side, ctx->copy, ctx->up_ev[0], pm, pm8, DeepRoots{w8, w8_2, mul(w8_2, w8)}, cnt,
                           dt_zz, dt_pw, scratch, deep_inv);
  HIP_CHECK(hipEventRecord(ctx->ev_join, ctx->side));
  dv = ood_launch(ctx, coef, w + C, w, logn, dt_pw, cm);
}

void ProofRun::ood_stage() {
  ood_values();
  dgam = ctx->buf<felt>("gamma", w + C);
  dk = ctx->buf<felt>("dt_dk", 4);
  HIP_CHECK(hipMemcpyAsync(dk, dt_zz, 32, hipMemcpyDeviceToDevice, st));
  launch_dt_deep_coeffs(pf, st, dt_seed, dv, w, C, o->batching_deep, dgam, dk);
  ctx->stage_end("3_ood");
}

void ProofRun::deep_stage() {
  deep = ctx->buf<felt>("deep", (size_t)Bl * n);
  {
    DeepArgs da;
    da.w = w; da.C = C; da.logB = logB; da.logn = logn; da.logN = logN;
    da.j0 = j0; da.logBl = logBl;
    da.tlde = tlde; da.clde = clde; da.gamma = dgam; da.dk = dk; da.g = g;
    da.inv = deep_inv;
    da.ginv = deep_ginv(logn);
    HIP_CHECK(hipStreamWaitEvent(st, ctx->ev_join, 0));
    deep_evaluations(ctx, cm, st, da, coef, n, Sj0, logN, deep);
  }
  ctx->stage_end("4_deep_launch");
}

void ProofRun::fri_stage() {
  const FriCursor c = fri_layers();
  fri_round_trip(c);
  ctx->stage_end("5_fri");
}

FriCursor ProofRun::fri_layers() {
  L = fri_num_layers(N, o);
  layers.assign(L + 1, FriLayer{});
  dres = ctx->buf<unsigned long long>("grind_res", 1);
  {
    uint64_t tot_e = 0, D = N;
    for (uint32_t l = 0; l < L; l++) { tot_e += D / F; D /= F; }
    felt* fe = ctx->buf<felt>("fri_evals", tot_e + 1);
    const felt* deps = fold_constants(ctx);
    felt* E = deep;
    uint64_t m = n, eo = 0;
    uint32_t Bc = Bl, jc = j0;
    bool sh = R > 1;
    D = N;
    felt off = g;
    auto replicate = [&](uint32_t l) {
      felt* full = ctx->buf<felt>("fri_full_" + std::to_string(l), (size_t)B * m);
      cm->all_gather(st, E, full, (size_t)Bl * m * 16);
      E = full;
      Bc = B;
      jc = 0;
      sh = false;
    };
    uint32_t* coin_d = ctx->buf<uint32_t>("fri_coin", 8 + 12 * (size_t)(L + 1));
    felt* alphas_d = reinterpret_cast<felt*>(coin_d + 8);
    uint32_t* roots_d = coin_d + 8 + 4 * (size_t)L;
    HIP_CHECK(hipMemcpyAsync(coin_d, dt_seed, 32, hipMemcpyDeviceToDevice, st));
    static const bool no_fri_tail = getenv("ZKP_NO_FRI_TAIL") != nullptr;
    const bool fuse_tail = R == 1 && o->grinding_factor > 0 && (N >> (ilog2(F) * L)) <= 256 && !no_fri_tail;
    FriTailArgs fta{};
    fta.F = F;
    for (uint32_t l = 0; l < L; l++) {
      const uint64_t m16 = m / F;
      if (sh && (m16 >> logR) < 16) replicate(l);
      FriLayer& ly = layers[l];
      ly.E = E; ly.m = m; ly.Bc = Bc; ly.jc = jc; ly.sharded = sh;
      if (fuse_tail && (m16 << logB) <= 128) {
        if (fta.nl >= FRI_TAIL_MAX) throw ZkpFail{ZKP_ERR_DEVICE, "FRI tail: too many small layers"};
        ly.tree.logR = 0;
        ly.tree.Lr = m16 << logB;
        ly.tree.nodes = ctx->buf<uint32_t>("ftree_" + std::to_string(l), (size_t)16 * ly.tree.Lr);
        ly.tree.top.assign(2, {});
        FriTailLayer& y = fta.ly[fta.nl++];
        y.E = E;
        y.nodes = ly.tree.nodes;
        y.logm16 = ilog2(m16);
        y.off_inv = inv(off);
        y.lev = ctx->itws(logN) + ((1ull << (ilog2(D) - 1)) - 1);
        y.out = fe + eo;
        y.alpha_out = alphas_d + l;
        y.root_out = roots_d + 8 * (size_t)l;
        E = fe + eo;
        eo += (uint64_t)Bc * m16;
        m = m16;
        D /= F;
        off = pow_u64(off, F);
        continue;
      }
      if (fta.nl) throw ZkpFail{ZKP_ERR_DEVICE, "FRI tail: a large layer after a small one"};
      MerkleTail coin{};
      coin.op = MERKLE_TAIL_FRI_COIN;
      coin.coin_seed = coin_d;
      coin.alpha_out = alphas_d + l;
      coin.root_out = roots_d + 8 * (size_t)l;
      const bool coin_done = commit_rows(ctx, cm, 1, E, 0, F, logB, ilog2(m16), sh, "ftree_" + std::to_string(l),
                                         ly.tree, T.fri_roots[l], false, &coin);
      if (!coin_done)
        launch_coin_fri_layer(pf, st, coin_d, sh ? ly.tree.top_d + 8 : ly.tree.nodes + 8, alphas_d + l,
                              roots_d + 8 * (size_t)l);
      felt* nxt = fe + eo;
      launch_fri_fold(pf, st, E, m16, Bc, jc, logB, F, alphas_d + l, inv(off), ctx->itws(logN), ilog2(D), deps,
                      nxt);
      eo += (uint64_t)Bc * m16;
      E = nxt;
      m = m16;
      D /= F;
      off = pow_u64(off, F);
    }
    if (sh) replicate(L);
    layers[L].E = E; layers[L].m = m; layers[L].Bc = B; layers[L].jc = 0; layers[L].sharded = false;
    const uint64_t Dlast = (uint64_t)B * m;
    dev_tail = Dlast <= 256 && o->grinding_factor > 0;
    if (fuse_tail && !dev_tail) throw ZkpFail{ZKP_ERR_DEVICE, "FRI tail fused without a device remainder"};
    dev_query = dev_tail && R == 1 && L <= GATHER_MAX_LAYERS;
    if (dev_tail) {
      rem_d = ctx->buf<felt>("rem_d", m + 1);
      rcommit_d = ctx->buf<uint32_t>("rem_commit", 8);
// ... 396 lines not shown
```

### zk_stark_project_amd/csrc/prover_internal.hpp

```cpp
#pragma once
#include <algorithm>
#include <array>
#include <chrono>
#include <cstdio>
#include <cstdlib>
#include <cstring>
#include <map>
#include <memory>
#include <stdexcept>
#include <string>
#include <utility>
#include <vector>

#include "../../include/zkp.h"
#include "blake3.hpp"
#include "comm.hpp"
#include "zkp_internal.hpp"

using namespace fp;

#include "host_stark.hpp"

using namespace zkh;

// ... 58 lines not shown
      b.p = nullptr;
      HIP_CHECK(hipMalloc(&b.p, bytes));
      b.bytes = bytes;
      if (prof.enabled) {
        auto& s = stats["host_alloc"];
        s.launches += 1;
        s.ms += std::chrono::duration<double, std::milli>(std::chrono::steady_clock::now() - t0).count();
        s.bytes += (double)bytes;
      }
    }
    return reinterpret_cast<T*>(b.p);
  }
  std::vector<void*> retired;
  void free_retired() {
    if (retired.empty()) return;
    for (hipStream_t s : {stream, side, copy}) HIP_CHECK(hipStreamSynchronize(s));
    for (void* p : retired) (void)hipFree(p);
    retired.clear();
  }
  void sync() { HIP_CHECK(hipStreamSynchronize(stream)); }
  std::map<std::string, bool> cached;
  std::map<std::string, std::vector<felt>> host_cache;
  bool have_cached(const std::string& key) {
    bool had = cached[key];
    cached[key] = true;
    return had;
  }
  uint8_t* ring_p = nullptr;
  size_t ring_cap = 0, ring_off = 0;
  void ring_reset() { ring_off = 0; }
  void upload(void* d, const void* h, size_t bytes) {
    if (bytes > (1u << 20)) {
      HIP_CHECK(hipMemcpyAsync(d, h, bytes, hipMemcpyHostToDevice, stream));
      return;
    }
    if (!ring_p) {
      ring_cap = 8u << 20;
      HIP_CHECK(hipHostMalloc((void**)&ring_p, ring_cap, hipHostMallocDefault));
    }
    size_t need = (bytes + 255) & ~(size_t)255;
    if (ring_off + need > ring_cap) {
      sync();
      ring_off = 0;
    }
    memcpy(ring_p + ring_off, h, bytes);
    HIP_CHECK(hipMemcpyAsync(d, ring_p + ring_off, bytes, hipMemcpyHostToDevice, stream));
    ring_off += need;
  }
  void download(void* h, const void* d, size_t bytes) {
    if (bytes > (1u << 20)) {
      HIP_CHECK(hipMemcpyAsync(h, d, bytes, hipMemcpyDeviceToHost, stream));
      sync();
      return;
    }
    void* hp = pinned(bytes);
    HIP_CHECK(hipMemcpyAsync(hp, d, bytes, hipMemcpyDeviceToHost, stream));
    sync();
    memcpy(h, hp, bytes);
  }
  std::chrono::steady_clock::time_point stage_t0;
  void stage_begin() { if (prof.enabled) stage_t0 = std::chrono::steady_clock::now(); }
  void stage_end(const char* name) {
    if (!prof.enabled) return;
    auto t = std::chrono::steady_clock::now();
    auto& s = stats[std::string("host_") + name];
    s.launches += 1;
    s.ms += std::chrono::duration<double, std::milli>(t - stage_t0).count();
    stage_t0 = t;
  }
  void collect_prof() {
    if (prof.pending.empty()) return;
    sync();
    static const bool timeline = getenv("ZKP_TIMELINE") != nullptr;
    if (timeline) {
      const hipEvent_t t0 = prof.pending.front().start;
      float prev_end = 0;
      for (auto& r : prof.pending) {
        float st = 0, en = 0;
        (void)hipEventElapsedTime(&st, t0, r.start);
        (void)hipEventElapsedTime(&en, t0, r.stop);
        fprintf(stderr, "TL %-18s start %8.3f dur %7.3f gap %7.3f\n", r.name, st, en - st, st - prev_end);
        prev_end = en;
      }
      fprintf(stderr, "TL end\n");
    }
    if (prof.only.empty()) {
      const hipEvent_t t0 = prof.pending.front().start;
      std::vector<std::pair<float, float>> iv;
      iv.reserve(prof.pending.size());
      for (auto& r : prof.pending) {
        float st = 0, en = 0;
        HIP_CHECK(hipEventElapsedTime(&st, t0, r.start));
        HIP_CHECK(hipEventElapsedTime(&en, t0, r.stop));
        iv.emplace_back(st, en);
      }
      std::sort(iv.begin(), iv.end());
      double busy = 0;
      float cs = iv[0].first, ce = iv[0].second;
      for (size_t i = 1; i < iv.size(); i++) {
        if (iv[i].first > ce) {
          busy += ce - cs;
          cs = iv[i].first;
          ce = iv[i].second;
        } else if (iv[i].second > ce) {
          ce = iv[i].second;
        }
      }
      busy += ce - cs;
      auto& b = stats["host_device_busy"];
      b.launches += 1;
      b.ms += busy;
    }
    for (auto& r : prof.pending) {
      float ms = 0;
      HIP_CHECK(hipEventElapsedTime(&ms, r.start, r.stop));
      auto& s = stats[r.name];
      s.launches += 1;
      s.ms += ms;
      s.bytes += r.bytes;
      prof.pool.push_back(r.start);
      prof.pool.push_back(r.stop);
    }
    prof.pending.clear();
  }

  std::map<uint32_t, bool> have_tw;
  void ensure_twiddles(uint32_t logN) {
    if (have_tw[logN]) return;
    stage_end("0_pre_tw");
    uint64_t half = 1ull << (logN - 1);
    for (int dir = 0; dir < 2; dir++) {
      felt w = root_of_unity(logN);
      if (dir) w = inv(w);
      std::vector<felt> lo(2048), hi((half + 2047) / 2048 + 1);
      lo[0] = one();
      for (int i = 1; i < 2048; i++) lo[i] = mul(lo[i - 1], w);
      felt step = mul(lo[2047], w);
      hi[0] = one();
      for (size_t i = 1; i < hi.size(); i++) hi[i] = mul(hi[i - 1], step);
      felt* dlo = buf<felt>("tmp_lo", lo.size());
      felt* dhi = buf<felt>("tmp_hi", hi.size());
      upload(dlo, lo.data(), lo.size() * 16);
      upload(dhi, hi.data(), hi.size() * 16);
      felt* t = buf<felt>((dir ? "itw_" : "tw_") + std::to_string(logN), 2 * half);
      launch_expand_powers(prof, stream, t + (half - 1), half, dlo, dhi);
      if (logN > 1) launch_build_levels(prof, stream, t, logN - 1);
      sync();
      stage_end(dir ? "0_tw_inv" : "0_tw_fwd");
    }
    have_tw[logN] = true;
  }
  felt* tws(uint32_t logN) { return reinterpret_cast<felt*>(bufs["tw_" + std::to_string(logN)].p); }
  felt* itws(uint32_t logN) { return reinterpret_cast<felt*>(bufs["itw_" + std::to_string(logN)].p); }
  felt* tw(uint32_t logN) { return tws(logN) + ((1ull << (logN - 1)) - 1); }
  felt* itw(uint32_t logN) { return itws(logN) + ((1ull << (logN - 1)) - 1); }

  std::map<std::tuple<uint32_t, uint32_t, uint32_t>, bool> have_coset;
  void ensure_coset(uint32_t logn, uint32_t logB, uint32_t logce) {
    auto key = std::make_tuple(logn, logB, logce);
    if (have_coset[key]) return;
    uint32_t logN = logn + logB;
    ensure_twiddles(logN);
    uint64_t n = 1ull << logn;
    felt g = felt_u64(3);
    for (int dir = 0; dir < 2; dir++) {
      felt base = dir ? inv(g) : g;
      std::vector<felt> lo(2048), hi(n / 2048 + 2);
      lo[0] = one();
      for (int i = 1; i < 2048; i++) lo[i] = mul(lo[i - 1], base);
      felt step = mul(lo[2047], base);
      hi[0] = one();
      for (size_t i = 1; i < hi.size(); i++) hi[i] = mul(hi[i - 1], step);
      felt* dlo = buf<felt>("tmp_lo", lo.size());
      felt* dhi = buf<felt>("tmp_hi", hi.size());
      upload(dlo, lo.data(), lo.size() * 16);
      upload(dhi, hi.data(), hi.size() * 16);
      std::string sfx = std::to_string(logn) + "_" + std::to_string(logB);
      if (dir == 0) {
        felt* S = buf<felt>("S_" + sfx, n << logB);
        launch_build_coset_scale(prof, stream, S, logn, 1u << logB, tw(logN), logN, dlo, dhi, inv(felt_u64(n)));
      } else {
        const uint32_t logM = logn + logce;
        felt* Si = buf<felt>("Si_" + sfx + "_" + std::to_string(logce), n << logce);
        launch_build_coset_scale(prof, stream, Si, logn, 1u << logce, itws(logN) + ((1ull << (logM - 1)) - 1), logM,
                                 dlo, dhi, one());
      }
      sync();
    }
    have_coset[key] = true;
  }
  felt* S(uint32_t logn, uint32_t logB) {
    return reinterpret_cast<felt*>(bufs["S_" + std::to_string(logn) + "_" + std::to_string(logB)].p);
  }
  felt* Si(uint32_t logn, uint32_t logB, uint32_t logce) {
    return reinterpret_cast<felt*>(
        bufs["Si_" + std::to_string(logn) + "_" + std::to_string(logB) + "_" + std::to_string(logce)].p);
  }

  void drop(const std::string& prefix) {
    sync();
    for (auto it = bufs.begin(); it != bufs.end();) {
      if (it->first.compare(0, prefix.size(), prefix) == 0) {
        if (it->second.p) HIP_CHECK(hipFree(it->second.p));
        it = bufs.erase(it);
      } else {
        ++it;
      }
    }
    for (auto it = cached.begin(); it != cached.end();)
      it = it->first.compare(0, prefix.size(), prefix) == 0 ? cached.erase(it) : std::next(it);
  }
  std::vector<zkp_ctx*> session_pool;
  std::vector<hipEvent_t> up_ev;
  void events(size_t k) {
    while (up_ev.size() < k) {
      hipEvent_t e;
      HIP_CHECK(hipEventCreateWithFlags(&e, hipEventDisableTiming));
      up_ev.push_back(e);
    }
  }

  zkp_comm* self = nullptr;
  zkp_comm* self_comm() {
    if (!self) self = make_self_comm();
    return self;
  }

  ~zkp_ctx() {
    delete self;
    for (void* p : retired) (void)hipFree(p);
    for (auto& kv : bufs)
      if (kv.second.p) (void)hipFree(kv.second.p);
    for (void* p : user_allocs) (void)hipFree(p);
    if (pinned_p) (void)hipHostFree(pinned_p);
    if (ring_p) (void)hipHostFree(ring_p);
    for (auto e : prof.pool) (void)hipEventDestroy(e);
    for (auto e : up_ev) (void)hipEventDestroy(e);
    if (ev_fork) (void)hipEventDestroy(ev_fork);
    if (ev_check) (void)hipEventDestroy(ev_check);
    if (flag_h) (void)hipHostFree(flag_h);
    if (ev_join) (void)hipEventDestroy(ev_join);
    if (stream && side && copy) {
      const hipStream_t ss[3] = {stream, side, copy};
      release_streams(device, ss);
    } else {
      if (copy) (void)hipStreamDestroy(copy);
      if (side) (void)hipStreamDestroy(side);
      if (stream) (void)hipStreamDestroy(stream);
    }
  }
  static bool acquire_streams(int device, hipStream_t out[3]);
  static void release_streams(int device, const hipStream_t s[3]);
};

zkp_ctx* new_ctx(int device);

struct ProgCodeLayout {
  const airp::Program& pr;
  size_t o_const, o_desc;
  std::vector<size_t> tab;
  ProgCodeLayout(const airp::Program& program, size_t scale) : pr(program) {
    o_const = (pr.ops.size() + 1) / 2;
    o_desc = o_const + pr.consts.size();
    tab.push_back(o_desc + (pr.periodic.size() + 1) / 2);
    for (const auto& col : pr.periodic) tab.push_back(tab.back() + col.size() * scale);
  }
  size_t end() const { return tab.back(); }
  void write(felt* img) const {
    memcpy(img, pr.ops.data(), pr.ops.size() * 8);
    if (!pr.consts.empty()) memcpy(img + o_const, pr.consts.data(), pr.consts.size() * 16);
    ProgPeriodic* desc = reinterpret_cast<ProgPeriodic*>(img + o_desc);
    for (size_t p = 0; p + 1 < tab.size(); p++)
      desc[p] = ProgPeriodic{(uint32_t)(tab[p] - tab[0]), (uint32_t)(tab[p + 1] - tab[p] - 1)};
  }
  ProgCode code(const felt* dimg) const {
    return ProgCode{reinterpret_cast<const uint64_t*>(dimg), (uint32_t)pr.ops.size(), pr.nreg, dimg + o_const,
                    reinterpret_cast<const ProgPeriodic*>(dimg + o_desc), dimg + tab[0], nullptr};
  }
};

namespace zkpi {

struct TreeShard {
  uint32_t* nodes = nullptr;
  uint64_t Lr = 0;
  uint32_t logR = 0;
  std::vector<std::array<uint8_t, 32>> top;
  uint32_t* top_d = nullptr;
  struct Loc {
    bool host;
    uint32_t owner;
    uint64_t local;
  };
  Loc locate(uint64_t k) const {
    uint32_t d = 63 - __builtin_clzll(k);
    if (d <= logR && logR > 0) return {true, 0, k};
    uint32_t below = d - logR;
    uint64_t s = (k >> below) - (1ull << logR);
    return {false, (uint32_t)s, (1ull << below) + (k & ((1ull << below) - 1))};
  }
};

struct Fetch {
  void* host;
  const void* dev;
  size_t bytes;
};

constexpr uint32_t DEEP_COEF_MIN_W = 16;

struct FriLayer {
  felt* E = nullptr;
  uint64_t m = 0;
  uint32_t Bc = 0, jc = 0;
  bool sharded = false;
// ... 219 lines not shown
```

### zk_stark_project_amd/csrc/prover_shard.cpp

```cpp
#include "prover_internal.hpp"

using namespace zkpi;

namespace zkpi {

bool commit_rows_sharded(zkp_ctx* ctx, zkp_comm* cm, int mode, const felt* src, uint64_t n, uint32_t cols,
                         uint32_t logB, uint32_t logrows, const std::string& name, TreeShard& tr, uint8_t root[32],
                         bool fetch_root, const MerkleTail* coin, const LastCol* lc, const GuLazy* gl) {
  Prof& pf = ctx->prof;
  hipStream_t st = ctx->stream;
  const uint32_t R = cm->world, logR = ilog2(R), logBl = logB - logR;
  const uint32_t logrr = logrows - logR;
  tr.logR = logR;
  tr.Lr = 1ull << (logB + logrr);
  uint32_t* send = ctx->buf<uint32_t>("shard_send", (size_t)8 << (logBl + logrows));
  uint32_t* recv = ctx->buf<uint32_t>("shard_recv", (size_t)8 << (logBl + logrows));
  const uint32_t logK = logrr >= 12 ? 2u : 0u, K = 1u << logK;
  const size_t chunk_words = (size_t)8 << (logBl + logrows - logK), block = (size_t)32 << (logBl + logrr - logK);
  ctx->events(K + 1);
  for (uint32_t k = 0; k < K; k++) {
    launch_leaf_hash_shard(pf, st, mode, src, n, cols, logBl, logrows, logrr, logK, k, send + k * chunk_words, lc,
                           gl);
    HIP_CHECK(hipEventRecord(ctx->up_ev[k], st));
  }
  for (uint32_t k = 0; k < K; k++) {
    HIP_CHECK(hipStreamWaitEvent(ctx->side, ctx->up_ev[k], 0));
    cm->all_to_all(ctx->side, send + k * chunk_words, recv + k * chunk_words, block);
  }
  HIP_CHECK(hipEventRecord(ctx->up_ev[K], ctx->side));
  HIP_CHECK(hipStreamWaitEvent(st, ctx->up_ev[K], 0));
  tr.nodes = ctx->buf<uint32_t>(name, (size_t)16 * tr.Lr);
  uint32_t* done = ctx->buf<uint32_t>("merkle_done", 1);
  if (!ctx->have_cached("merkle_done")) HIP_CHECK(hipMemsetAsync(done, 0, 4, st));
  launch_merkle_from_shards(pf, st, recv, logB, logrr, logK, tr.nodes, done);
  uint32_t* roots = ctx->buf<uint32_t>("shard_roots", (size_t)8 * R);
  cm->all_gather(st, tr.nodes + 8, roots, 32);
  tr.top_d = ctx->buf<uint32_t>(name + "_top", (size_t)16 * R);
  launch_shard_top(pf, st, roots, R, tr.top_d, coin);
  tr.top.assign(2 * R, {});
  if (fetch_root) {
    ctx->download(tr.top.data(), tr.top_d, (size_t)64 * R);
    memcpy(root, tr.top[1].data(), 32);
  }
  return coin && coin->op != MERKLE_TAIL_NONE;
}

felt* ood_launch_sharded(zkp_ctx* ctx, const felt* arrays, uint32_t narrays, uint32_t ntwo, uint32_t logn,
                         const felt* dpw, zkp_comm* cm, felt* part, felt* dv) {
  const uint32_t logE = logn < 11 ? logn : 11, nb = 1u << (logn - logE), R = (uint32_t)cm->world;
  const felt ninv = inv(felt_u64(1ull << logn));
  const uint32_t nbl = nb / R;
  felt* mine = ctx->buf<felt>("ood_part_rank", (size_t)2 * narrays * nbl);
  launch_eval_bitrev_blocks(ctx->prof, ctx->stream, arrays, narrays, ntwo, logn, dpw, dpw + logn,
                            (uint32_t)cm->rank * nbl, nbl, mine);
  cm->all_gather(ctx->stream, mine, part, (size_t)2 * narrays * nbl * 16);
  launch_eval_bitrev_tail(ctx->prof, ctx->stream, part, narrays, logn, nbl, dpw, dpw + logn, ninv, dv);
  return dv;
}



void ProofRun::trace_column_sharded(const zkp_felt* h_trace, uint32_t cpt, uint32_t wi, uint32_t d) {
  uint32_t K = 6;
  while (cpt % K) K--;
  const uint32_t cpr = cpt / K;
  felt* own = ctx->buf<felt>("coef_own", (size_t)cpt * n);
  ctx->events(3 * (size_t)K);
  HIP_CHECK(hipEventRecord(ctx->ev_fork, st));
  HIP_CHECK(hipStreamWaitEvent(ctx->copy, ctx->ev_fork, 0));
  HIP_CHECK(hipStreamWaitEvent(ctx->side, ctx->ev_fork, 0));
  for (uint32_t k = 0; k < K; k++) {
    const uint64_t cown = (uint64_t)k * R * cpr + (uint64_t)rank * cpr, c0 = (uint64_t)k * R * cpr;
    felt* dcol = const_cast<felt*>(d_trace) + cown * n;
    if (h_trace) {
      HIP_CHECK(hipMemcpyAsync(dcol, h_trace + cown * n, (size_t)cpr * n * 16, hipMemcpyHostToDevice, ctx->copy));
      h_partial = true;
    }
    NttBatch ib{dcol, own + (size_t)k * cpr * n, nullptr, n, n, 1, 1, cpr};
    launch_ntt(pf, ctx->copy, ib, logn, false, ctx->itws(logN), logN);
    HIP_CHECK(hipEventRecord(ctx->up_ev[k], ctx->copy));
    HIP_CHECK(hipStreamWaitEvent(ctx->side, ctx->up_ev[k], 0));
    cm->all_gather(ctx->side, own + (size_t)k * cpr * n, coef + c0 * n, (size_t)cpr * n * 16);
    HIP_CHECK(hipEventRecord(ctx->up_ev[K + k], ctx->side));
    HIP_CHECK(hipStreamWaitEvent(st, ctx->up_ev[K + k], 0));
    NttBatch lb{coef + c0 * n, tlde + c0 * Bl * n, Sj0, n, n, Bl, Bl, R * cpr * Bl};
    launch_ntt(pf, st, lb, logn, true, ctx->tws(logN), logN);
  }
  HIP_CHECK(hipEventRecord(ctx->up_ev[2 * K], ctx->copy));
  HIP_CHECK(hipStreamWaitEvent(st, ctx->up_ev[2 * K], 0));
  if (paired && wi < w) {
    const uint32_t i0 = wi - d, np = w - wi;
    const uint64_t nR = n >> logR;
    launch_gu_check(pf, st, d_trace, d, logn, air.k, i0, np, (uint64_t)rank * nR, logn - logR, gu_cval, gu_bad);
    if (rank) launch_gu_check(pf, st, d_trace, d, logn, air.k, i0, np, 0, 0, gu_cval, gu_bad);
    gu_flags = ctx->buf<uint32_t>("gu_flags", 4 * (size_t)R);
    cm->all_gather(st, gu_bad, gu_flags, 16);
    const bool slice = (n >> std::min(logn, 11u)) >= R;
    launch_gu_coef(pf, st, coef, d, logn, air.k, ctx->itws(logN) + ((n >> 1) - 1), i0, np,
                   slice ? (uint64_t)rank * nR : 0, slice ? nR : n, gu_cval);
    if (!gu_lazy_on) launch_gu_lde(pf, st, tlde, d, logn, logBl, air.k, i0, np, gu_cval, l0_table());
  } else {
    paired = false;
    gu_lazy_on = false;
  }
}

const zkp_felt* ProofRun::gather_host_slices(const zkp_felt* h_trace) {
  const uint64_t nR = n >> logR;
  felt* dfull = const_cast<felt*>(d_trace);
  felt* slice = ctx->buf<felt>("trace_slice", (size_t)w * nR);
  HIP_CHECK(hipMemcpy2DAsync(slice, nR * 16, h_trace + (size_t)rank * nR, n * 16, nR * 16, w,
                             hipMemcpyHostToDevice, st));
  if (w == 1) {
    cm->all_gather(st, slice, dfull, nR * 16);
  } else {
    felt* gat = ctx->buf<felt>("trace_gather", (size_t)w * n);
    cm->all_gather(st, slice, gat, (size_t)w * nR * 16);
    for (uint32_t sr = 0; sr < R; sr++)
      HIP_CHECK(hipMemcpy2DAsync(dfull + (size_t)sr * nR, n * 16, gat + (size_t)sr * w * nR, nR * 16, nR * 16, w,
                                 hipMemcpyDeviceToDevice, st));
  }
  return nullptr;
}

felt* ProofRun::composition_exchange(felt* cint, uint64_t nR) {
  felt* send = ctx->buf<felt>("comp_send", (size_t)celmax * n);
  felt* recv = ctx->buf<felt>("comp_recv", (size_t)celmax * n);
  for (uint32_t ul = 0; ul < cel; ul++)
    HIP_CHECK(hipMemcpy2DAsync(send + (size_t)ul * nR, (size_t)celmax * nR * 16, cint + (size_t)ul * n, nR * 16,
                               nR * 16, R, hipMemcpyDeviceToDevice, st));
  cm->all_to_all(st, send, recv, (size_t)celmax * nR * 16);
  return recv;
}

void ProofRun::composition_gather_lde(felt* slice, bool derive, uint64_t nR, uint64_t p0) {
  ctx->events(C + 1);
  HIP_CHECK(hipEventRecord(ctx->ev_fork, st));
  HIP_CHECK(hipStreamWaitEvent(ctx->side, ctx->ev_fork, 0));
  HIP_CHECK(hipStreamWaitEvent(ctx->copy, ctx->ev_fork, 0));
  bool on_copy = false;
  const bool ood_split = (n >> std::min(logn, 11u)) >= R;
  for (uint32_t m = 0; m < C; m++) {
    if (derive && ood_split && m == C - 1) {
      HIP_CHECK(hipMemcpyAsync(acoef + (size_t)m * n + p0, slice + (size_t)m * nR, nR * 16,
                               hipMemcpyDeviceToDevice, st));
      break;
    }
    cm->all_gather(ctx->side, slice + (size_t)m * nR, acoef + (size_t)m * n, nR * 16);
    HIP_CHECK(hipEventRecord(ctx->up_ev[m], ctx->side));
    if (derive && m == C - 1) {
      HIP_CHECK(hipStreamWaitEvent(st, ctx->up_ev[m], 0));
      break;
    }
    hipStream_t ls = (m & 1) ? ctx->copy : st;
    on_copy = on_copy || ls == ctx->copy;
    HIP_CHECK(hipStreamWaitEvent(ls, ctx->up_ev[m], 0));
    NttBatch lb{acoef + (size_t)m * n, clde + (size_t)m * Bl * n, Sj0, n, n, Bl, Bl, Bl};
    launch_ntt(pf, ls, lb, logn, true, ctx->tws(logN), logN);
  }
  if (on_copy) {
    HIP_CHECK(hipEventRecord(ctx->up_ev[C], ctx->copy));
    HIP_CHECK(hipStreamWaitEvent(st, ctx->up_ev[C], 0));
  }
}

}

namespace {
bool sharded_factor_refused(const zkp_comm* comm, const zkp_proof_options* o) {
  return comm && o && comm->world > 1 && check_options(o) == 0 && o->fri_folding_factor != 16;
}
bool sharded_air_refused(const zkp_comm* comm, int air) { return comm && comm->world > 1 && air >= ZKP_AIR_FIRST_ID; }
}

extern "C" {

int zkp_prove_sharded(zkp_ctx* ctx, zkp_comm* comm, zkp_air_id air, const zkp_felt* trace, uint32_t width,
                      uint64_t n, const zkp_felt* pub, uint64_t n_pub, const zkp_proof_options* opts, uint8_t** proof,
                      uint64_t* proof_len, zkp_transcript* transcript) {
  if (ctx && sharded_air_refused(comm, air)) return ZKP_ERR_UNSUPPORTED_AIR;
  if (ctx && sharded_factor_refused(comm, opts)) return ZKP_ERR_INVALID_OPTIONS;
  int rc = guarded(ctx, [&] {
    ctx->err.clear();
    HIP_CHECK(hipSetDevice(ctx->device));
    if (!trace || !comm) return (int)ZKP_ERR_ARGUMENT;
    if (n < 8 || (n & (n - 1)) || width == 0 || width > 255) return (int)ZKP_ERR_TRACE_SHAPE;
    felt* d = ctx->buf<felt>("trace_in", (size_t)width * n);
    return prove_impl(ctx, comm, air, d, width, n, pub, n_pub, opts, proof, proof_len, transcript, trace);
  });
  if (rc && comm) comm->abort();
  return rc;
}

int zkp_prove_sharded_device(zkp_ctx* ctx, zkp_comm* comm, zkp_air_id air, const void* d_trace, uint32_t width,
                             uint64_t n, const zkp_felt* pub, uint64_t n_pub, const zkp_proof_options* opts,
                             uint8_t** proof, uint64_t* proof_len, zkp_transcript* transcript) {
  if (ctx && sharded_air_refused(comm, air)) return ZKP_ERR_UNSUPPORTED_AIR;
  if (ctx && sharded_factor_refused(comm, opts)) return ZKP_ERR_INVALID_OPTIONS;
  int rc = guarded(ctx, [&] {
    ctx->err.clear();
    HIP_CHECK(hipSetDevice(ctx->device));
    if (!d_trace || !comm) return (int)ZKP_ERR_ARGUMENT;
    return prove_impl(ctx, comm, air, (const felt*)d_trace, width, n, pub, n_pub, opts, proof, proof_len,
                      transcript);
  });
  if (rc && comm) comm->abort();
  return rc;
}

int zkp_comm_local_group(int world, zkp_comm** comms) {
  if (!comms || world < 1 || world > 64) return ZKP_ERR_ARGUMENT;
  try {
    make_local_group(world, comms);
  } catch (...) {
    return ZKP_ERR_OOM;
  }
  return ZKP_OK;
}

int zkp_comm_rccl_unique_id(uint8_t id[128]) {
  if (!id) return ZKP_ERR_ARGUMENT;
  try {
    rccl_unique_id(id);
  } catch (...) {
    return ZKP_ERR_DEVICE;
  }
  return ZKP_OK;
}

int zkp_comm_rccl_create(zkp_ctx* ctx, const uint8_t id[128], int world, int rank, zkp_comm** out) {
  return guarded(ctx, [&] {
    if (!id || !out || world < 1 || rank < 0 || rank >= world) return (int)ZKP_ERR_ARGUMENT;
    *out = make_rccl_comm(ctx->device, id, world, rank);
    return 0;
  });
}

int zkp_comm_host_create(int world, int rank, const zkp_host_transport* t, zkp_comm** out) {
  if (!t || !out || !t->all_to_all || !t->all_gather || world < 1 || world > 64 || rank < 0 || rank >= world)
    return ZKP_ERR_ARGUMENT;
  try {
    *out = make_host_comm(world, rank, *t);
  } catch (...) {
    return ZKP_ERR_OOM;
  }
  return ZKP_OK;
}

void zkp_comm_destroy(zkp_comm* comm) { delete comm; }

int zkp_comm_check(zkp_ctx* ctx, zkp_comm* comm, uint64_t block_bytes, double* a2a_ms, double* ag_ms) {
  int rc = guarded(ctx, [&] {
    ctx->err.clear();
    HIP_CHECK(hipSetDevice(ctx->device));
    if (!comm || block_bytes == 0 || (block_bytes & 3)) return (int)ZKP_ERR_ARGUMENT;
    const uint32_t W = (uint32_t)comm->world, me = (uint32_t)comm->rank;
    const uint64_t words = block_bytes / 4;
    auto tag = [](uint32_t src, uint32_t dst, uint64_t i) {
      return ((src + 1) * 0x9E3779B1u) ^ ((dst + 7) * 0x85EBCA77u) ^ ((uint32_t)i * 0xC2B2AE3Du) ^ (uint32_t)(i >> 32);
    };
    std::vector<uint32_t> h((size_t)W * words);
    for (uint32_t s = 0; s < W; s++)
      for (uint64_t i = 0; i < words; i++) h[s * words + i] = tag(me, s, i);
    uint32_t* send = ctx->buf<uint32_t>("cc_send", (size_t)W * words);
    uint32_t* recv = ctx->buf<uint32_t>("cc_recv", (size_t)W * words);
    ctx->upload(send, h.data(), h.size() * 4);
    ctx->sync();
    auto timed = [&](bool a2a) {
      double best = 1e30;
      for (int it = 0; it < 2; it++) {
        HIP_CHECK(hipMemsetAsync(recv, 0, (size_t)W * block_bytes, ctx->stream));
        ctx->sync();
        auto t0 = std::chrono::steady_clock::now();
        if (a2a) comm->all_to_all(ctx->stream, send, recv, block_bytes);
        else comm->all_gather(ctx->stream, send, recv, block_bytes);
        ctx->sync();
        best = std::min(best, std::chrono::duration<double, std::milli>(std::chrono::steady_clock::now() - t0).count());
      }
      ctx->download(h.data(), recv, h.size() * 4);
      for (uint32_t s = 0; s < W; s++)
        for (uint64_t i = 0; i < words; i++)
          if (h[s * words + i] != (a2a ? tag(s, me, i) : tag(s, 0, i)))
            throw ZkpFail{ZKP_ERR_DEVICE, std::string(a2a ? "all_to_all" : "all_gather") + ": block from rank " +
                                              std::to_string(s) + " differs at word " + std::to_string(i)};
      return best;
    };
    const double ta = timed(true), tg = timed(false);
    if (a2a_ms) *a2a_ms = ta;
    if (ag_ms) *ag_ms = tg;
    return 0;
  });
  if (rc && comm) comm->abort();
  return rc;
}

int zkp_comm_rank(const zkp_comm* comm) { return comm ? comm->rank : -1; }
int zkp_comm_world(const zkp_comm* comm) { return comm ? comm->world : -1; }

int zkp_comm_backend_world(const zkp_comm* comm) { return comm ? comm->backend_world() : -1; }

}
```

### zk_stark_project_amd/csrc/prover_stages.cpp

```cpp
#include "prover_internal.hpp"

using namespace zkpi;

namespace zkpi {

bool commit_rows(zkp_ctx* ctx, zkp_comm* cm, int mode, const felt* src, uint64_t n, uint32_t cols, uint32_t logB,
                 uint32_t logrows, bool sharded, const std::string& name, TreeShard& tr, uint8_t root[32],
                 bool fetch_root, const MerkleTail* coin, const LastCol* lc, const GuLazy* gl) {
  Prof& pf = ctx->prof;
  hipStream_t st = ctx->stream;
  const uint64_t L = 1ull << (logB + logrows);
  if (!sharded) {
    tr.logR = 0;
    tr.Lr = L;
    tr.nodes = ctx->buf<uint32_t>(name, (size_t)16 * L);
    uint32_t* done = ctx->buf<uint32_t>("merkle_done", 1);
    if (!ctx->have_cached("merkle_done")) HIP_CHECK(hipMemsetAsync(done, 0, 4, st));
    MerkleTail tail = coin ? *coin : MerkleTail{};
    tail.done = done;
    bool ran = mode == 0 ? launch_merkle_lde(pf, st, src, cols, logB, n, tr.nodes, L, &tail, lc, gl)
                         : launch_merkle_fri(pf, st, src, 1ull << logrows, logB, cols, tr.nodes, &tail);
    tr.top.assign(2, {});
    if (fetch_root) {
      ctx->download(root, tr.nodes + 8, 32);
// ... 79 lines not shown
  }
  return cx8;
}

felt deep_ginv(uint32_t logn) {
  static const std::vector<felt> tab = [] {
    std::vector<felt> t(MAX_LOG_TRACE + 1);
    for (uint32_t l = 0; l <= MAX_LOG_TRACE; l++) t[l] = inv(root_of_unity(l));
    return t;
  }();
  return tab[logn];
}

void constraint_eval(zkp_ctx* ctx, const AirDesc& air, uint32_t logn, uint32_t logB, uint32_t logce, uint32_t u0,
                     uint32_t cel, uint32_t j0, uint32_t logBl, const felt* cx, const felt* twn, const felt* dt_cc,
                     const felt* dt_aval, const felt* tlde, felt* comp, const felt* coef, zkp_comm* cm) {
  Prof& pf = ctx->prof;
  hipStream_t st = ctx->stream;
  const uint32_t B = 1u << logB, ce = 1u << logce, logN = logn + logB, w = air.w;
  const uint64_t n = 1ull << logn;
  const felt g = felt_u64(3);
  felt wn = root_of_unity(logn);
  EvalCommon ec;
  ec.logn = logn; ec.logB = logB; ec.logce = logce; ec.logN = logN;
  ec.u0 = u0; ec.cel = cel; ec.j0 = j0; ec.logBl = logBl;
  ec.g = g;
  ec.w_last = pow_u64(wn, n - 1);
  ec.pm = PointMap{cx + B + u0, twn, logn};
  const std::string zkey = "zinv_" + std::to_string(logn) + "_" + std::to_string(logce);
  std::vector<felt>& zinv = ctx->host_cache[zkey];
  if (zinv.empty()) {
    zinv.resize(ce);
    felt gn = pow_u64(g, n), wce = root_of_unity(logce);
    for (uint32_t s = 0; s < ce; s++) zinv[s] = inv(sub(mul(gn, pow_u64(wce, s)), one()));
  }
  felt* dz = ctx->buf<felt>(zkey, ce);
  if (!ctx->have_cached(zkey)) ctx->upload(dz, zinv.data(), ce * 16);
  const std::string dom = std::to_string(logn) + "_" + std::to_string(logB) + "_" + std::to_string(u0) + "_" +
                          std::to_string(cel);
  auto sce_rows = [&]() -> const felt* {
    const uint32_t cstep = logB - logce;
    const felt* S = ctx->S(logn, logB);
    if (!cstep) return S;
    const std::string skey = "Sce_" + std::to_string(logn) + "_" + std::to_string(logB) + "_" + std::to_string(logce);
    felt* t = ctx->buf<felt>(skey, (size_t)ce * n);
    if (!ctx->have_cached(skey))
      HIP_CHECK(hipMemcpy2DAsync(t, n * 16, S, (n << cstep) * 16, n * 16, ce, hipMemcpyDeviceToDevice, st));
    return t;
  };
  if (air.prog) {
    if (!cel) return;
    const airp::Program& pr = *air.prog;
    const ProgCodeLayout lay(pr, ce);
    const bool params = pr.num_pub != 0;
    const std::vector<airp::Strided>& sv = pr.strided;
    const size_t S = sv.size();
    size_t nseq = 0, seq_felts = 0;
    for (const airp::Strided& a : sv)
      if (a.sequence()) nseq++, seq_felts += a.nvals;
    const size_t o_col = lay.end(), o_scol = o_col + (pr.a_col.size() + 3) / 4, o_sval = o_scol + (S + 3) / 4,
                 o_sdesc = o_sval + S, o_stab = o_sdesc + (nseq + 1) / 2, o_pseq = o_stab + seq_felts,
                 total = o_pseq + (params ? nseq : 0);
    felt* dimg = ctx->buf<felt>("prog_image", total);
    std::vector<felt>& img = ctx->host_cache["prog_image"];
    std::vector<felt>& tag = ctx->host_cache["prog_image_tag"];
    const felt want[2] = {make((uint64_t)air.id, logn), make(logce, total)};
    if (tag.size() != 2 || !eq(tag[0], want[0]) || !eq(tag[1], want[1])) {
      const auto img_t0 = std::chrono::steady_clock::now();
      tag.clear();
      img.assign(total, zero());
      lay.write(img.data());
      if (!pr.a_col.empty()) memcpy(img.data() + o_col, pr.a_col.data(), pr.a_col.size() * 4);
      for (size_t p = 0; p < pr.periodic.size(); p++) {
        const size_t cyc = pr.periodic[p].size();
        std::vector<felt> kc = pr.periodic[p];
        host_interpolate(kc, one());
        const std::vector<felt> kv = host_evaluate(kc, cyc * ce, pow_u64(g, n / cyc));
        memcpy(img.data() + lay.tab[p], kv.data(), kv.size() * 16);
      }
      uint32_t* scol = reinterpret_cast<uint32_t*>(img.data() + o_scol);
      ProgSeq* sdesc = reinterpret_cast<ProgSeq*>(img.data() + o_sdesc);
      ProgPubSeq* pseq = reinterpret_cast<ProgPubSeq*>(img.data() + o_pseq);
      size_t soff = 0, q = 0;
      for (size_t j = 0; j < S; j++) {
        scol[j] = sv[j].col;
        img[o_sval + j] = params ? zero() : sv[j].val;
        if (!sv[j].sequence()) continue;
        if (params) {
          const uint32_t k = sv[j].nvals;
          if (sv[j].pub < 0) memcpy(img.data() + o_stab + soff, sv[j].values.data(), (size_t)k * 16);
          pseq[q] = ProgPubSeq{(uint32_t)soff, ilog2(k), (uint32_t)sv[j].first,
                               sv[j].pub < 0 ? 0u : (uint32_t)sv[j].pub + 1};
          sdesc[q++] = ProgSeq{(uint32_t)j, (uint32_t)soff};
          soff += k;
          continue;
        }
        std::vector<felt> pc = sv[j].values;
        host_interpolate(pc, one());
        const felt tw = inv(pow_u64(wn, sv[j].first));
        felt sc = felt_u64(n);
        for (size_t i = 0; i < pc.size(); i++) {
          img[o_stab + soff + i] = mul(pc[i], sc);
          sc = mul(sc, tw);
        }
        sdesc[q++] = ProgSeq{(uint32_t)j, (uint32_t)soff};
        soff += pc.size();
      }
      ctx->upload(dimg, img.data(), total * 16);
      tag.assign(want, want + 2);
      if (pf.enabled) {
        auto& hs = ctx->stats["host_prog_image"];
        hs.launches += 1;
        hs.ms += std::chrono::duration<double, std::milli>(std::chrono::steady_clock::now() - img_t0).count();
        hs.bytes += (double)total * 16;
      }
    }
    ec.zinv = dz;
    ProgEvalArgs pa{};
    pa.code = lay.code(dimg);
    const felt* dsval = dimg + o_sval;
    const felt* dstab = dimg + o_stab;
    if (params) {
      felt* dpub = ctx->buf<felt>("prog_pub", pr.num_pub);
      ctx->upload(dpub, pr.pub.data(), (size_t)pr.num_pub * 16);
      pa.code.pub = dpub;
      if (S) {
        std::vector<felt> sval(S);
        for (size_t j = 0; j < S; j++) sval[j] = sv[j].val;
        felt* d = ctx->buf<felt>("prog_sval", S);
        ctx->upload(d, sval.data(), S * 16);
        dsval = d;
      }
      if (nseq) {
        felt* vals = ctx->buf<felt>("prog_seq_vals", seq_felts);
        felt* ntt = ctx->buf<felt>("prog_seq_ntt", seq_felts);
        felt* tab = ctx->buf<felt>("prog_seq_tab", seq_felts);
        ProgPubSeqArgs ga{};
        ga.nseq = (uint32_t)nseq;
        ga.logn = logn;
        ga.desc = reinterpret_cast<const ProgPubSeq*>(dimg + o_pseq);
        ga.pub = dpub;
        ga.raw = dimg + o_stab;
        ga.itwn = ctx->itws(logN) + ((n >> 1) - 1);
        uint64_t maxk = 1;
        for (const airp::Strided& a : sv) maxk = std::max<uint64_t>(maxk, a.nvals);
        launch_prog_seq_gather(pf, st, ga, maxk, vals);
        size_t off = 0;
        for (size_t j = 0; j < S;) {
          size_t e = j, cnt = 0;
          while (e < S && sv[e].stride == sv[j].stride && sv[e].first == sv[j].first) cnt += sv[e++].sequence();
          const uint64_t k = n / sv[j].stride;
          if (cnt && k > 1) {
            NttBatch ib{vals + off, ntt + off, nullptr, k, k, 1, 1, (uint32_t)cnt};
            launch_ntt(pf, st, ib, ilog2(k), false, ctx->itws(logN), logN);
          } else if (cnt) {
            HIP_CHECK(hipMemcpyAsync(ntt + off, vals + off, cnt * 16, hipMemcpyDeviceToDevice, st));
          }
          off += cnt * k;
          j = e;
        }
        launch_prog_seq_twist(pf, st, ga, maxk, ntt, tab);
        dstab = tab;
      }
    }
    pa.num_t = pr.num_t;
    pa.a_col = reinterpret_cast<const uint32_t*>(dimg + o_col);
    pa.cc = dt_cc;
    pa.a_val = dt_aval;
    pa.col_stride = n << logBl;
    pa.binv = ctx->buf<felt>("binv_scratch", ((uint64_t)cel * n) / 2048 + 1);
    for (size_t k = 0; k < air.a_step.size(); k++) {
      if (k == 0 || air.a_step[k] != air.a_step[k - 1]) {
        if (pa.ngroups == PROG_MAX_GROUPS) throw ZkpFail{ZKP_ERR_UNSUPPORTED_AIR, "assertions over more than 4 steps"};
        const uint32_t gi = pa.ngroups++;
        const std::string key = "binv_prog_" + dom + "_" + std::to_string(air.a_step[k]);
        pa.w_step[gi] = pow_u64(wn, air.a_step[k]);
        pa.dinv[gi] = ctx->buf<felt>(key, (uint64_t)cel * n);
        pa.dinv_ready[gi] = ctx->have_cached(key);
      }
      pa.grp_end[pa.ngroups - 1] = (uint32_t)k + 1;
    }
    if (!S) {
      launch_eval_program(pf, st, ec, pa, tlde, comp);
      return;
    }
    ProgStridedArgs sa{};
    ProgSeqArgs qa{};
    sa.col = reinterpret_cast<const uint32_t*>(dimg + o_scol);
    sa.val = dsval;
    sa.cc = qa.cc = dt_cc + pr.num_t + pr.a_col.size();
    qa.desc = reinterpret_cast<const ProgSeq*>(dimg + o_sdesc);
    qa.tab = dstab;
    int wslot[PROG_MAX_STRIDED_GROUPS] = {-1, -1, -1, -1};
    uint32_t seqs = 0;
    for (size_t j = 0; j < S; j++) {
      const uint64_t k = n / sv[j].stride, len = sv[j].stride * ce;
      if (j == 0 || sv[j].stride != sv[j - 1].stride || sv[j].first != sv[j - 1].first) {
        if (sa.ngroups == PROG_MAX_STRIDED_GROUPS)
          throw ZkpFail{ZKP_ERR_UNSUPPORTED_AIR, "strided assertions over more than 4 groups"};
        const uint32_t gi = sa.ngroups++;
        sa.mask[gi] = (uint32_t)(len - 1);
        const std::string key = "dstr_" + std::to_string(logn) + "_" + std::to_string(logce) + "_" +
                                std::to_string(sv[j].stride) + "_" + std::to_string(sv[j].first);
        felt* tab = ctx->buf<felt>(key, len + 1);
        if (!ctx->have_cached(key)) {
          const felt gk = pow_u64(g, k);
          ctx->upload(tab + len, &gk, 16);
          launch_strided_den_table(pf, st, tab + len, ctx->tws(logN) + (len / 2 - 1), ilog2(len),
                                   pow_u64(wn, sv[j].first * k), pa.binv, tab);
        }
        sa.dtab[gi] = tab;
      }
      const uint32_t gi = sa.ngroups - 1;
      sa.grp_end[gi] = (uint32_t)j + 1;
      if (sv[j].sequence()) {
        if (wslot[gi] < 0) {
          wslot[gi] = (int)qa.ngroups++;
          qa.logk[wslot[gi]] = ilog2(k);
        }
        qa.seq_end[wslot[gi]] = ++seqs;
      }
    }
    if (qa.ngroups) {
      felt* wc = ctx->buf<felt>("strided_w_coef", (size_t)qa.ngroups * n);
      felt* wev = ctx->buf<felt>("strided_w_ev", (size_t)qa.ngroups * cel * n);
      launch_strided_combine(pf, st, qa, logn, wc);
      NttBatch eb{wc, wev, sce_rows() + (uint64_t)u0 * n, n, n, cel, cel, qa.ngroups * cel};
      launch_ntt(pf, st, eb, logn, true, ctx->tws(logN), logN);
      for (uint32_t gi = 0; gi < sa.ngroups; gi++)
        if (wslot[gi] >= 0) sa.W[gi] = wev + (size_t)wslot[gi] * cel * n;
    }
    launch_eval_program(pf, st, ec, pa, tlde, comp, &sa);
    return;
  }
  const uint32_t lw = air.id == ZKP_AIR_TRAINING_UPDATE ? w / 2 : w;
  felt* dconst = ctx->buf<felt>("eval_consts", air.id == ZKP_AIR_MIMC ? (size_t)ce + 4 : 4 * (size_t)lw + 2);
  launch_dt_eval_consts(pf, st, air.id, dt_cc, air.k, ec.w_last, dt_aval, dz, ce, w, air.num_t, dconst);
  ec.zinv = air.id == ZKP_AIR_MIMC ? dconst : dz;
  const bool coef_form = air.id != ZKP_AIR_MIMC && coef;
  if (!cel && !coef_form) return;
  auto linear = [&](LinearEvalArgs& la, const std::string& key) {
    la.binv = ctx->buf<felt>("binv_scratch", ((uint64_t)cel * n) / 2048 + 1);
    la.dinv = ctx->buf<felt>(key, (uint64_t)cel * n);
    la.binv_ready = ctx->have_cached(key);
    if (!coef_form) {
      launch_eval_linear(pf, st, ec, la, tlde, comp);
      return;
    }
    const uint32_t R = cm ? (uint32_t)cm->world : 1u, rank = cm ? (uint32_t)cm->rank : 0u;
    const uint32_t narr = (la.transition ? 1u : 0u) + 1u + (la.two_groups ? 1u : 0u);
    const uint64_t nR = n / R;
    felt* lc = ctx->buf<felt>("lin_coef", (size_t)narr * n);
    felt* mine = R > 1 ? ctx->buf<felt>("lin_mine", (size_t)narr * nR) : lc;
    felt* part = ctx->buf<felt>("lincomb_part", (size_t)4 * lincomb_groups(nR, la.width) * nR);
    launch_lin_lincomb(pf, st, la.transition, la.two_groups, coef, la.width, logn, (uint64_t)rank * nR, nR,
                       dconst, twn, mine, part);
    for (uint32_t i = 0; R > 1 && i < narr; i++) cm->all_gather(st, mine + i * nR, lc + i * n, nR * 16);
    if (!cel) return;
    const felt* Sce = sce_rows();
    felt* ev = ctx->buf<felt>("lin_ev", (size_t)narr * cel * n);
    NttBatch eb{lc, ev, Sce + (uint64_t)u0 * n, n, n, cel, cel, narr * cel};
    launch_ntt(pf, st, eb, logn, true, ctx->tws(logN), logN);
    launch_eval_linear_pts(pf, st, ec, la, ev, comp);
  };
  if (air.id == ZKP_AIR_MIMC) {
    const std::string kkey = "kper_" + std::to_string(logn) + "_" + std::to_string(logce);
    felt* dk = ctx->buf<felt>(kkey, 64 * (size_t)ce);
    if (!ctx->have_cached(kkey)) {
      std::vector<felt> kc(64);
      for (int j = 0; j < 64; j++) kc[j] = felt_u64((uint64_t)(j + 1) * 1000000ull);
      host_interpolate(kc, one());
      std::vector<felt> kv = host_evaluate(kc, 64 * ce, pow_u64(g, n / 64));
      ctx->upload(dk, kv.data(), kv.size() * 16);
    }
    MimcEvalArgs ma;
    ma.bcoef = dconst + ce;
    ma.kper = dk;
    std::string key = "binv_mimc_" + dom;
    ma.binv = ctx->buf<felt>("binv_scratch", ((uint64_t)cel * n) / 2048 + 1);
    ma.dinv = ctx->buf<felt>(key, (uint64_t)cel * n);
    ma.binv_ready = ctx->have_cached(key);
    launch_eval_mimc(pf, st, ec, ma, tlde, comp);
  } else if (air.id == ZKP_AIR_GLOBAL_UPDATE) {
    LinearEvalArgs la;
    la.width = w;
    la.transition = true;
    la.two_groups = false;
    la.coefs = dconst;
    la.w_bstep = pow_u64(wn, air.a_step[0]);
    la.w_bstep1 = zero();
    linear(la, "binv_lin_" + dom + "_" + std::to_string(air.a_step[0]));
  } else {
    const uint32_t half = w / 2;
    LinearEvalArgs la;
    la.width = half;
    la.transition = false;
    la.two_groups = true;
    la.coefs = dconst;
    la.w_bstep = one();
    la.w_bstep1 = ec.w_last;
    linear(la, "binv_tu_" + dom);
  }
}

const felt* last_col_kappa(zkp_ctx* ctx, uint32_t logn, uint32_t logB, uint32_t C) {
  const uint32_t B = 1u << logB;
  const std::string key = "lastcol_kap_" + std::to_string(logn) + "_" + std::to_string(logB) + "_" +
                          std::to_string(C);
  felt* d = ctx->buf<felt>(key, 2 * (size_t)B);
  if (!ctx->have_cached(key)) {
    std::vector<felt> h(2 * (size_t)B);
    const felt gn = pow_u64(felt_u64(3), 1ull << logn), wB = root_of_unity(logB);
    for (uint32_t j = 0; j < B; j++) {
      h[2 * j] = mul(gn, pow_u64(wB, j));
      h[2 * j + 1] = inv(pow_u64(h[2 * j], C - 1));
    }
    ctx->upload(d, h.data(), h.size() * 16);
  }
  return d;
}

std::vector<felt> comp_dft_consts(uint64_t n, uint32_t logce, uint32_t C) {
  const uint32_t ce = 1u << logce;
  std::vector<felt> dc((size_t)C + ce / 2);
  const felt g = felt_u64(3), ce_inv = inv(felt_u64(ce)), gn_inv = inv(pow_u64(g, n)),
             wce_inv = inv(root_of_unity(logce));
  for (uint32_t m = 0; m < C; m++) dc[m] = mul(pow_u64(gn_inv, m), ce_inv);
  for (uint32_t k = 0; k < ce / 2; k++) dc[C + k] = pow_u64(wce_inv, k);
  return dc;
}

void deep_evaluations(zkp_ctx* ctx, zkp_comm* cm, hipStream_t st, DeepArgs da, const felt* coef, uint64_t n,
                      const felt* Sj0, uint32_t logN, felt* out) {
  if (da.w < DEEP_COEF_MIN_W) {
    launch_deep(ctx->prof, st, da, out);
    return;
  }
  const uint32_t Bl = 1u << da.logBl;
  const uint32_t R = (uint32_t)cm->world;
  felt* acomb = ctx->buf<felt>("deep_acoef", n);
  const uint64_t nR = n / R;
  felt* part = ctx->buf<felt>("lincomb_part", (size_t)lincomb_groups(nR, da.w) * nR);
  if (R == 1) {
    launch_deep_lincomb(ctx->prof, st, coef, da.w, n, 0, n, da.gamma, acomb, part);
  } else {
    felt* mine = ctx->buf<felt>("deep_acoef_rank", nR);
    launch_deep_lincomb(ctx->prof, st, coef, da.w, n, (uint64_t)cm->rank * nR, nR, da.gamma, mine, part);
    cm->all_gather(st, mine, acomb, nR * 16);
  }
  felt* alde = ctx->buf<felt>("deep_alde", (size_t)Bl * n);
  NttBatch lb{acomb, alde, Sj0, n, n, Bl, Bl, Bl};
  launch_ntt(ctx->prof, st, lb, da.logn, true, ctx->tws(logN), logN);
  const std::string g1key = "deep_g1_" + std::to_string(da.C);
  felt* g1 = ctx->buf<felt>(g1key, (size_t)da.C + 1);
  if (!ctx->have_cached(g1key)) {
    const felt unit = one();
    ctx->upload(g1, &unit, 16);
  }
  HIP_CHECK(hipMemcpyAsync(g1 + 1, da.gamma + da.w, (size_t)da.C * 16, hipMemcpyDeviceToDevice, st));
  da.w = 1;
  da.tlde = alde;
  da.gamma = g1;
  launch_deep(ctx->prof, st, da, out);
}

void gather_openings(zkp_ctx* ctx, zkp_comm* cm, const std::vector<uint64_t>& pos, uint64_t n, uint32_t logB,
                     uint32_t j0, const felt* tlde, uint32_t w, const TreeShard& ttree, const felt* clde, uint32_t C,
                     const TreeShard& ctree, const std::vector<FriLayer>& layers, uint32_t L, uint32_t F,
                     Openings& op) {
  Prof& pf = ctx->prof;
  hipStream_t st = ctx->stream;
  const uint32_t R = (uint32_t)cm->world, rank = (uint32_t)cm->rank;
  const uint32_t B = 1u << logB, Bl = B / R;
  const uint64_t N = n << logB;
  struct SegPlan {
    const void* src;
    std::vector<uint64_t> idx;
    std::vector<int32_t> owner;
    std::vector<const uint8_t*> host_dig;
    uint32_t words;
  };
  auto row_owner = [&](uint64_t j) -> uint32_t { return R > 1 ? (uint32_t)(j / Bl) : 0; };
  auto lde_values = [&](const felt* src, uint32_t cols) {
    SegPlan sp{src, {}, {}, {}, 4};
    sp.idx.reserve(pos.size() * cols);
    sp.owner.reserve(pos.size() * cols);
    sp.host_dig.reserve(pos.size() * cols);
    for (uint64_t p : pos) {
      uint64_t j = p & (B - 1), t = p >> logB;
      uint32_t ow = row_owner(j);
      for (uint32_t c = 0; c < cols; c++) {
        sp.idx.push_back(ow == rank ? ((uint64_t)c * Bl + (j - j0)) * n + t : 0);
        sp.owner.push_back((int32_t)ow);
        sp.host_dig.push_back(nullptr);
      }
    }
    return sp;
  };
  auto path_nodes = [&](const TreeShard& tr, const BatchPlan& bp) {
    SegPlan sp{tr.nodes, {}, {}, {}, 8};
    for (auto& pth : bp.paths)
      for (uint64_t k : pth) {
        TreeShard::Loc lc = tr.locate(k);
        if (lc.host) {
          sp.idx.push_back(0);
          sp.owner.push_back(-1);
          sp.host_dig.push_back(tr.top[lc.local].data());
        } else {
          sp.idx.push_back(lc.owner == (tr.logR ? rank : 0u) ? lc.local : 0);
          sp.owner.push_back(tr.logR ? (int32_t)lc.owner : (int32_t)rank);
          sp.host_dig.push_back(nullptr);
        }
      }
    return sp;
  };
  op.bt = plan_batch(N, pos);
  const BatchPlan& bt = op.bt;
  const BatchPlan& bc = bt;
  std::vector<std::vector<uint64_t>> fpos(L);
  op.bf.assign(L, BatchPlan{});
  std::vector<BatchPlan>& bf = op.bf;
  std::vector<SegPlan> plan;
  plan.push_back(lde_values(tlde, w));
  plan.push_back(path_nodes(ttree, bt));
  plan.push_back(lde_values(clde, C));
  plan.push_back(path_nodes(ctree, bc));
  {
    std::vector<uint64_t> cur = pos;
    for (uint32_t l = 0; l < L; l++) {
      const FriLayer& ly = layers[l];
      const uint64_t m16 = ly.m / F, Rows = (uint64_t)B * m16;
      fpos[l] = fold_positions(cur, Rows);
      bf[l] = plan_batch(Rows, fpos[l]);
      SegPlan sp{ly.E, {}, {}, {}, 4};
      for (uint64_t r : fpos[l])
        for (uint32_t k = 0; k < F; k++) {
          uint64_t i = r + k * Rows;
          uint64_t j = i & (B - 1), tt = i >> logB;
          uint32_t ow = ly.sharded ? (uint32_t)(j / Bl) : rank;
          sp.idx.push_back(ow == rank ? (j - ly.jc) * ly.m + tt : 0);
          sp.owner.push_back((int32_t)ow);
          sp.host_dig.push_back(nullptr);
        }
      plan.push_back(sp);
      plan.push_back(path_nodes(ly.tree, bf[l]));
      cur = fpos[l];
    }
  }
  std::vector<GatherSeg>& segs = op.segs;
  segs.clear();
  std::vector<uint64_t> all_idx;
  uint64_t out_words = 0, max_count = 1;
  for (auto& sp : plan) {
    GatherSeg gs;
    gs.src = sp.src;
    gs.idx_off = all_idx.size();
    gs.count = sp.idx.size();
    gs.out_off = out_words;
    gs.words = sp.words;
    gs.pad = 0;
    all_idx.insert(all_idx.end(), sp.idx.begin(), sp.idx.end());
    out_words += gs.count * sp.words;
    max_count = std::max<uint64_t>(max_count, gs.count);
    segs.push_back(gs);
  }
  size_t seg_bytes = segs.size() * sizeof(GatherSeg), idx_bytes = all_idx.size() * 8;
  size_t up_bytes = seg_bytes + idx_bytes, down_bytes = out_words * 4;
  ctx->stage_end("7a_query_plan");
  uint8_t* hp = (uint8_t*)ctx->pinned(std::max(up_bytes, down_bytes * R) + 64);
  memcpy(hp, segs.data(), seg_bytes);
  memcpy(hp + seg_bytes, all_idx.data(), idx_bytes);
  uint8_t* dup = ctx->buf<uint8_t>("gather_in", up_bytes + 16);
  uint32_t* dout = ctx->buf<uint32_t>("gather_out", out_words + 4);
  uint32_t* dall = R > 1 ? ctx->buf<uint32_t>("gather_all", out_words * R + 4) : dout;
  HIP_CHECK(hipMemcpyAsync(dup, hp, up_bytes, hipMemcpyHostToDevice, st));
  launch_gather_multi(pf, st, (const GatherSeg*)dup, (uint32_t)segs.size(), max_count,
                      (const uint64_t*)(dup + seg_bytes), dout, (double)down_bytes * 2);
  if (R > 1) cm->all_gather(st, dout, dall, down_bytes);
  HIP_CHECK(hipMemcpyAsync(hp, dall, down_bytes * R, hipMemcpyDeviceToHost, st));
  ctx->sync();
  ctx->stage_end("7b_gather");
  op.gathered.assign(out_words, 0);
  std::vector<uint32_t>& gathered = op.gathered;
  {
    const uint32_t* all = reinterpret_cast<const uint32_t*>(hp);
    for (size_t si = 0; si < plan.size(); si++) {
      const SegPlan& sp = plan[si];
      const GatherSeg& gs = segs[si];
      for (size_t it = 0; it < sp.idx.size(); it++) {
        uint32_t* dst = gathered.data() + gs.out_off + it * sp.words;
        if (sp.owner[it] < 0) {
          memcpy(dst, sp.host_dig[it], 32);
        } else {
          uint32_t ow = R > 1 ? (uint32_t)sp.owner[it] : 0;
          memcpy(dst, all + (size_t)ow * out_words + gs.out_off + it * sp.words, sp.words * 4);
        }
      }
    }
  }
}

void openings_from_full(const std::vector<uint64_t>& raw, const std::vector<uint64_t>& pos, const uint32_t* full,
                        const FullGatherArgs& ga, const std::vector<FriLayer>& layers, uint32_t L, uint32_t F,
                        Openings& op) {
  const uint32_t w = ga.w, C = ga.C, nv = w + C, logN = ga.logN;
// ... 88 lines not shown
```

### zk_stark_project_amd/csrc/zkp_internal.hpp

```cpp
#pragma once
#include <hip/hip_runtime.h>
#include <stdint.h>

#include <string>
#include <vector>

#include "felt.hpp"
#include "pcg64.hpp"

struct ProfRec {
  const char* name;
  double bytes;
  hipEvent_t start, stop;
};
struct Prof {
  bool enabled = false;
  std::string only;
  bool open = false;
  std::vector<ProfRec> pending;
  std::vector<hipEvent_t> pool;
  hipEvent_t get_event();
  void begin(const char* name, hipStream_t s, double bytes);
  void end(hipStream_t s);
};

[[noreturn]] void launch_fail(int code, const char* what);
constexpr uint32_t MAX_LOG_DOMAIN = 28, MAX_LOG_TRACE = 23;
void preload_kernels_module();
void preload_merkle_module();
void preload_ntt_module();
void warm_stream(hipStream_t s);

struct NttBatch {
  const felt* src;
  felt* dst;
  const felt* scale;
  uint64_t src_stride, dst_stride;
  uint32_t src_div, scale_mod, batches;
};

void launch_ntt(Prof& prof, hipStream_t s, const NttBatch& b, uint32_t logn, bool dit, const felt* tw,
                uint32_t logN, int only_pass = -1);

void launch_build_levels(Prof& prof, hipStream_t s, felt* tab, uint32_t top);
void launch_expand_powers(Prof& prof, hipStream_t s, felt* out, uint64_t count, const felt* lo_tab,
                          const felt* hi_tab);
void launch_build_coset_scale(Prof& prof, hipStream_t s, felt* S, uint32_t logn, uint32_t B,
                              const felt* tw, uint32_t logN, const felt* glo, const felt* ghi, felt ninv);

enum { MERKLE_TAIL_NONE = 0, MERKLE_TAIL_FRI_COIN = 1, MERKLE_TAIL_DRAW_COEFFS = 2, MERKLE_TAIL_DRAW_Z = 3 };
struct MerkleTail {
  uint32_t* done;
  uint32_t* coin_seed;
  felt* alpha_out;
  uint32_t* root_out;
  uint32_t op, method, ncoef, logn;
  felt wn;
  felt* out;
  felt* pw;
};
struct LastCol {
  const felt* H;
  const felt* kap;
  felt* out;
};
struct GuLazy {
  const felt* cval;
  const felt* l0;
  felt k;
  uint32_t d, wi, smallk;
};
bool launch_merkle_lde(Prof& prof, hipStream_t s, const felt* lde, uint32_t cols, uint32_t logB, uint64_t n,
                       uint32_t* nodes, uint64_t L, const MerkleTail* tail = nullptr, const LastCol* lc = nullptr,
                       const GuLazy* gl = nullptr);
bool launch_merkle_fri(Prof& prof, hipStream_t s, const felt* E, uint64_t m16, uint32_t logB, uint32_t F,
                       uint32_t* nodes, const MerkleTail* tail = nullptr);
bool merkle_upper(Prof& prof, hipStream_t s, uint32_t* nodes, uint64_t L, const MerkleTail* tail = nullptr);
void launch_leaf_hash_shard(Prof& prof, hipStream_t s, int mode, const felt* src, uint64_t n, uint32_t cols,
                            uint32_t logBl, uint32_t logrows, uint32_t logrr, uint32_t logK, uint32_t k,
                            uint32_t* send, const LastCol* lc = nullptr, const GuLazy* gl = nullptr);
void launch_shard_top(Prof& prof, hipStream_t s, const uint32_t* roots, uint32_t R, uint32_t* top,
                      const MerkleTail* tail);
void launch_merkle_from_shards(Prof& prof, hipStream_t s, const uint32_t* recv, uint32_t logB, uint32_t logrr,
                               uint32_t logK, uint32_t* nodes, uint32_t* done = nullptr);
constexpr uint32_t PACK_MAX = 16;
struct PackArgs {
  const void* src[PACK_MAX];
  uint64_t bytes[PACK_MAX], off[PACK_MAX];
  uint32_t n;
};
void launch_pack(Prof& prof, hipStream_t s, const PackArgs& a, void* dst);
void launch_grind(Prof& prof, hipStream_t s, const uint32_t* seed_words, const uint32_t* seed_dev, uint64_t base,
                  uint64_t count, uint32_t bits, unsigned long long* result);
void launch_fri_remainder(Prof& prof, hipStream_t s, const felt* E, uint32_t logB, uint32_t m, felt off_inv,
                          felt wd_inv, felt d_inv, uint32_t* seed, felt* rem_out, uint32_t* commit_out);

void launch_grind_all(Prof& prof, hipStream_t s, const uint32_t* seed_dev, uint64_t base, uint64_t limit,
                      uint32_t bits, unsigned long long* result);
void launch_query_positions(Prof& prof, hipStream_t s, const uint32_t* seed_dev, const unsigned long long* nonce,
                            uint32_t q, uint64_t N, uint64_t* pos);
constexpr uint32_t GATHER_MAX_LAYERS = 16;
struct FullGatherArgs {
  const felt* tlde;
  const felt* clde;
  const uint32_t* tnodes;
  const uint32_t* cnodes;
  uint64_t n;
  uint32_t w, C, logB, logN, nlayers;
  uint32_t F;
  const felt* E[GATHER_MAX_LAYERS];
  const uint32_t* fnodes[GATHER_MAX_LAYERS];
  uint64_t m[GATHER_MAX_LAYERS];
  uint32_t logrows[GATHER_MAX_LAYERS];
  uint64_t seg_off[GATHER_MAX_LAYERS + 1];
  uint32_t rec_words[GATHER_MAX_LAYERS + 1];
};
void launch_gather_full(Prof& prof, hipStream_t s, const FullGatherArgs& a, uint32_t q, const uint64_t* pos,
                        uint32_t* out);

void launch_dt_draw_coeffs(Prof& prof, hipStream_t s, uint32_t* seed, const uint32_t* root, uint32_t method,
                           uint32_t ncoef, felt* cc);
void launch_dt_eval_consts(Prof& prof, hipStream_t s, int air, const felt* cc, felt k, felt w_last, const felt* aval,
                           const felt* zinv, uint32_t ce, uint32_t w, uint32_t num_t, felt* out);
void launch_dt_deep_coeffs(Prof& prof, hipStream_t s, uint32_t* seed, const felt* ood, uint32_t w, uint32_t C,
                           uint32_t method, felt* gamma, felt* dk);
void launch_dt_draw_z(Prof& prof, hipStream_t s, uint32_t* seed, const uint32_t* root, felt wn, uint32_t logn,
                      felt* zz, felt* pw);

void launch_gu_trace(Prof& prof, hipStream_t s, const felt* masked, const felt* raw, const felt* local,
                     uint64_t ndev, felt kinv, uint64_t n, felt* tile_buf, felt* out);
struct TuClient {
  felt* out;
  const uint64_t* masks;
  felt pr_inv, lr_inv;
  pcg::u128 pcg_state;
  pcg::u128 pcg_mul[pcg::JUMP_BITS], pcg_inc[pcg::JUMP_BITS];
};
void launch_tu_states(Prof& prof, hipStream_t s, const TuClient* clients, uint32_t K, const felt* initial,
                      const felt* batch, felt* states, uint32_t bs, felt ac_inv);
void launch_tu_write(Prof& prof, hipStream_t s, const TuClient* clients, uint32_t K, const felt* states,
                     uint64_t bs, uint64_t n, felt* first_last);

struct PointMap {
  const felt* cx;
  const felt* twn;
  uint32_t logn;
};

struct EvalCommon {
  uint32_t logn, logB, logce, logN;
  uint32_t u0, cel, j0, logBl;
  felt g, w_last;
  PointMap pm;
  const felt* zinv;
};
struct MimcEvalArgs {
  const felt* bcoef;
  const felt* kper;
  felt* binv;
  felt* dinv;
  bool binv_ready;
};
void launch_eval_mimc(Prof& prof, hipStream_t s, const EvalCommon& c, const MimcEvalArgs& a, const felt* lde,
                      felt* comp);
struct LinearEvalArgs {
  uint32_t width;
  bool transition, two_groups;
  const felt* coefs;
  felt w_bstep, w_bstep1;
  felt* binv;
  felt* dinv;
  bool binv_ready;
};
void launch_eval_linear(Prof& prof, hipStream_t s, const EvalCommon& c, const LinearEvalArgs& a, const felt* lde,
                        felt* comp);
uint32_t lincomb_groups(uint64_t np, uint32_t W);
void launch_lin_lincomb(Prof& prof, hipStream_t s, bool trans, bool two, const felt* coef, uint32_t W, uint32_t logn,
                        uint64_t p0, uint64_t np, const felt* coefs, const felt* twn, felt* out, felt* scratch);
void launch_eval_linear_pts(Prof& prof, hipStream_t s, const EvalCommon& c, const LinearEvalArgs& a, const felt* ev,
                            felt* comp);

namespace airp {
constexpr uint32_t op_code(uint64_t op) { return (uint32_t)(op & 0xff); }
constexpr uint32_t op_dst(uint64_t op) { return (uint32_t)((op >> 8) & 0xff); }
constexpr uint32_t op_a(uint64_t op) { return (uint32_t)((op >> 16) & 0xffff); }
constexpr uint32_t op_b(uint64_t op) { return (uint32_t)((op >> 32) & 0xffff); }
constexpr uint32_t src_kind(uint32_t operand) { return operand >> 13; }
constexpr uint32_t src_index(uint32_t operand) { return operand & 0x1fff; }
}

struct ProgPeriodic {
  uint32_t off, mask;
};
struct ProgCode {
  const uint64_t* ops;
// ... 181 lines not shown
```

Measured before the change: 231.2 proofs/s.

## Use precomputed twiddle quotients for Shoup-style NTT butterfly multiplication

Adds a per-twiddle precomputed companion table (twq/itwq) and a new mul_pre path that multiplies by a fixed twiddle using the precomputed value, replacing the generic modular multiply inside NTT butterflies. The tables are built once per domain and passed to every launch_ntt call site. This aims to cut the reduction arithmetic per butterfly. In exchange it doubles twiddle memory traffic and table storage, and it adds a fallback path that allocates and frees a temporary table when none is supplied.

```diff
diff --git a/__graft_entry__.py b/__graft_entry__.py
--- a/__graft_entry__.py
+++ b/__graft_entry__.py
@@ -15,6 +15,8 @@
                           env=env)
     subprocess.check_call(["make", "-j", jobs, "-C", os.path.join(ROOT, "tests", "native"), "-f",
                            "column_degrees_check.mk"], env=env)
+    subprocess.check_call(["make", "-j", jobs, "-C", os.path.join(ROOT, "tests", "native"), "-f",
+                           "mul_pre_check.mk"], env=env)
     if ROOT not in sys.path:
         sys.path.insert(0, ROOT)
     import zk_stark_project_amd
diff --git a/zk_stark_project_amd/csrc/abi.cpp b/zk_stark_project_amd/csrc/abi.cpp
--- a/zk_stark_project_amd/csrc/abi.cpp
+++ b/zk_stark_project_amd/csrc/abi.cpp
@@ -239,9 +239,9 @@
     ctx->ensure_coset(logn, logB, 1);
     const uint32_t logN = logn + logB;
     NttBatch ib{d, coef, nullptr, n, n, 1, 1, w};
-    launch_ntt(ctx->prof, ctx->stream, ib, logn, false, ctx->itws(logN), logN);
+    launch_ntt(ctx->prof, ctx->stream, ib, logn, false, ctx->itws(logN), logN, -1, ctx->itwqs(logN, logn));
     NttBatch lb{coef, lde, ctx->S(logn, logB), n, n, blowup, blowup, w * blowup};
-    launch_ntt(ctx->prof, ctx->stream, lb, logn, true, ctx->tws(logN), logN);
+    launch_ntt(ctx->prof, ctx->stream, lb, logn, true, ctx->tws(logN), logN, -1, ctx->twqs(logN, logn));
     TreeShard tr;
     commit_rows(ctx, ctx->self_comm(), 0, lde, n, w, logB, logn, false, "ttree", tr, root);
     if (lde_out) {
@@ -588,9 +588,9 @@
     felt* coef = ctx->buf<felt>("deg_coef", (size_t)width * n);
     felt* ext = ctx->buf<felt>("deg_ext", (size_t)width * M);
     NttBatch ib{(const felt*)d_trace_cols, coef, nullptr, n, n, 1, 1, width};
-    launch_ntt(ctx->prof, ctx->stream, ib, logn, false, ctx->itws(logN), logN);
+    launch_ntt(ctx->prof, ctx->stream, ib, logn, false, ctx->itws(logN), logN, -1, ctx->itwqs(logN, logn));
     NttBatch lb{coef, ext, ctx->S(logn, logE), n, n, E, E, width * E};
-    launch_ntt(ctx->prof, ctx->stream, lb, logn, true, ctx->tws(logN), logN);
+    launch_ntt(ctx->prof, ctx->stream, lb, logn, true, ctx->tws(logN), logN, -1, ctx->twqs(logN, logn));
     const std::string dkey = "deg_dft_" + std::to_string(logn) + "_" + std::to_string(logE);
     felt* dcoefs = ctx->buf<felt>(dkey + "_coefs", (size_t)E + E / 2);
     uint32_t* dblk = ctx->buf<uint32_t>(dkey + "_blk", E);
@@ -610,7 +610,7 @@
       const uint32_t k = std::min(K, pr.num_t - i0);
       launch_program_columns(ctx->prof, ctx->stream, code, ext, width, logn, logE, i0, k, vals);
       NttBatch cb{vals, vals, nullptr, n, n, 1, 1, k * E};
-      launch_ntt(ctx->prof, ctx->stream, cb, logn, false, ctx->itws(logN), logN);
+      launch_ntt(ctx->prof, ctx->stream, cb, logn, false, ctx->itws(logN), logN, -1, ctx->itwqs(logN, logn));
       for (uint32_t c = 0; c < k; c++)
         launch_comp_dft(ctx->prof, ctx->stream, vals + (size_t)c * M, dblk, ctx->Si(logn, logE, logE), dcoefs, E, E,
                         logn, 0, n, cf + (size_t)c * M);
diff --git a/zk_stark_project_amd/csrc/felt_dev.hpp b/zk_stark_project_amd/csrc/felt_dev.hpp
--- a/zk_stark_project_amd/csrc/felt_dev.hpp
+++ b/zk_stark_project_amd/csrc/felt_dev.hpp
@@ -420,6 +420,150 @@
   cd = join(Z[0], Z[1], Z[2], Z[3]);
 }
 
+__device__ __forceinline__ void mul_pre_core(L4 x, L4 w, L4 v, uint32_t& z0, uint32_t& z1, uint32_t& z2, uint32_t& z3,
+                                             uint64_t& k) {
+  const uint32_t K = 0x2d00u;
+  uint64_t acc, c;
+  uint32_t ov;
+  acc = mul_wide(x.w0, w.w0);
+  acc = mad_co(x.w2, v.w0, acc, c); ov = carry_0(c);
+  const uint32_t r0 = (uint32_t)acc;
+  acc = (acc >> 32) | ((uint64_t)ov << 32);
+  acc = mad_co(x.w0, w.w1, acc, c); ov = carry_0(c);
+  acc = mad_co(x.w1, w.w0, acc, c); ov = addc_0(ov, c);
+  acc = mad_co(x.w2, v.w1, acc, c); ov = addc_0(ov, c);
+  acc = mad_co(x.w3, v.w0, acc, c); ov = addc_0(ov, c);
+  const uint32_t r1 = (uint32_t)acc;
+  acc = (acc >> 32) | ((uint64_t)ov << 32);
+  acc = mad_co(x.w0, w.w2, acc, c); ov = carry_0(c);
+  acc = mad_co(x.w1, w.w1, acc, c); ov = addc_0(ov, c);
+  acc = mad_co(x.w2, v.w2, acc, c); ov = addc_0(ov, c);
+  acc = mad_co(x.w3, v.w1, acc, c); ov = addc_0(ov, c);
+  const uint32_t r2 = (uint32_t)acc;
+  acc = (acc >> 32) | ((uint64_t)ov << 32);
+  acc = mad_co(x.w0, w.w3, acc, c); ov = carry_0(c);
+  acc = mad_co(x.w1, w.w2, acc, c); ov = addc_0(ov, c);
+  acc = mad_co(x.w2, v.w3, acc, c); ov = addc_0(ov, c);
+  acc = mad_co(x.w3, v.w2, acc, c); ov = addc_0(ov, c);
+  const uint32_t r3 = (uint32_t)acc;
+  acc = (acc >> 32) | ((uint64_t)ov << 32);
+  acc = mad_co(x.w1, w.w3, acc, c); ov = carry_0(c);
+  acc = mad_co(x.w3, v.w3, acc, c);
+  const uint32_t r6 = addc_0(ov, c);
+  const uint32_t r4 = (uint32_t)acc, r5 = (uint32_t)(acc >> 32);
+  uint64_t t = mul_wide(r4, K);
+  const uint32_t q0 = (uint32_t)t;
+  t = mad(r5, K, t >> 32);
+  const uint32_t q1 = (uint32_t)t;
+  const uint32_t q2 = (uint32_t)(t >> 32) + r6 * K;
+  uint64_t b;
+  const uint32_t y1 = add_co(r1, q0, c);
+  const uint32_t y2 = addc_co(r2, q1, c, c);
+  const uint32_t y3 = addc_co(r3, q2, c, c);
+  z0 = sub_co(r0, r4, b);
+  z1 = subb_co(y1, r5, b, b);
+  z2 = subb_co(y2, r6, b, b);
+  z3 = subb_co_0(y3, b, b);
+  ZKP_ASM("s_andn2_b64 %0, %1, %2" : "=s"(k) : "s"(c), "s"(b) : "scc");
+}
+
+__device__ __forceinline__ void mul_pre_x2_core(L4 x, L4 w, L4 v, L4 X, L4 W, L4 V, uint32_t z[4], uint32_t Z[4],
+                                                uint64_t& k1, uint64_t& k2) {
+  const uint32_t K = 0x2d00u;
+  uint64_t acc, c, bcc, d;
+  uint32_t ov, bov, r[4], s[4];
+  acc = mul_wide(x.w0, w.w0);
+  bcc = mul_wide(X.w0, W.w0);
+#define ZKP_COL_BEGIN(a0, i0, b0, j0)              \
+  acc = mad_co(x.w##i0, b0.w##j0, acc, c);         \
+  bcc = mad_co(X.w##i0, a0.w##j0, bcc, d);         \
+  ov = carry_0(c);                                 \
+  bov = carry_0(d);
+#define ZKP_COL_STEP(a0, i0, b0, j0)               \
+  acc = mad_co(x.w##i0, b0.w##j0, acc, c);         \
+  bcc = mad_co(X.w##i0, a0.w##j0, bcc, d);         \
+  ov = addc_0(ov, c);                              \
+  bov = addc_0(bov, d);
+#define ZKP_COL_END(n)                             \
+  r[n] = (uint32_t)acc;                            \
+  s[n] = (uint32_t)bcc;                            \
+  acc = (acc >> 32) | ((uint64_t)ov << 32);        \
+  bcc = (bcc >> 32) | ((uint64_t)bov << 32);
+  ZKP_COL_BEGIN(V, 2, v, 0) ZKP_COL_END(0)
+  ZKP_COL_BEGIN(W, 0, w, 1) ZKP_COL_STEP(W, 1, w, 0) ZKP_COL_STEP(V, 2, v, 1) ZKP_COL_STEP(V, 3, v, 0) ZKP_COL_END(1)
+  ZKP_COL_BEGIN(W, 0, w, 2) ZKP_COL_STEP(W, 1, w, 1) ZKP_COL_STEP(V, 2, v, 2) ZKP_COL_STEP(V, 3, v, 1) ZKP_COL_END(2)
+  ZKP_COL_BEGIN(W, 0, w, 3) ZKP_COL_STEP(W, 1, w, 2) ZKP_COL_STEP(V, 2, v, 3) ZKP_COL_STEP(V, 3, v, 2) ZKP_COL_END(3)
+  ZKP_COL_BEGIN(W, 1, w, 3) ZKP_COL_STEP(V, 3, v, 3)
+#undef ZKP_COL_BEGIN
+#undef ZKP_COL_STEP
+#undef ZKP_COL_END
+  const uint32_t r4 = (uint32_t)acc, r5 = (uint32_t)(acc >> 32), r6 = ov;
+  const uint32_t s4 = (uint32_t)bcc, s5 = (uint32_t)(bcc >> 32), s6 = bov;
+  uint64_t t = mul_wide(r4, K), tt = mul_wide(s4, K);
+  const uint32_t q0 = (uint32_t)t, p0 = (uint32_t)tt;
+  t = mad(r5, K, t >> 32); tt = mad(s5, K, tt >> 32);
+  const uint32_t q1 = (uint32_t)t, p1 = (uint32_t)tt;
+  const uint32_t q2 = (uint32_t)(t >> 32) + r6 * K, p2 = (uint32_t)(tt >> 32) + s6 * K;
+  uint64_t e, b, f;
+  const uint32_t y1 = add_co(r[1], q0, c);
+  const uint32_t Y1 = add_co(s[1], p0, e);
+  z[0] = sub_co(r[0], r4, b);
+  Z[0] = sub_co(s[0], s4, f);
+  const uint32_t y2 = addc_co(r[2], q1, c, c);
+  const uint32_t Y2 = addc_co(s[2], p1, e, e);
+  z[1] = subb_co(y1, r5, b, b);
+  Z[1] = subb_co(Y1, s5, f, f);
+  const uint32_t y3 = addc_co(r[3], q2, c, c);
+  const uint32_t Y3 = addc_co(s[3], p2, e, e);
+  z[2] = subb_co(y2, r6, b, b);
+  Z[2] = subb_co(Y2, s6, f, f);
+  z[3] = subb_co_0(y3, b, b);
+  Z[3] = subb_co_0(Y3, f, f);
+  ZKP_ASM("s_andn2_b64 %0, %1, %2" : "=s"(k1) : "s"(c), "s"(b) : "scc");
+  ZKP_ASM("s_andn2_b64 %0, %1, %2" : "=s"(k2) : "s"(e), "s"(f) : "scc");
+}
+
+__device__ __forceinline__ felt mul_pre(felt x, felt w, felt wq) {
+  uint32_t z0, z1, z2, z3;
+  uint64_t k;
+  mul_pre_core(split(x), split(w), split(wq), z0, z1, z2, z3, k);
+  return canon_rare(z0, z1, z2, z3, k);
+}
+
+__device__ __forceinline__ felt mul_pre_z(felt x, felt w, felt wq, Rare& q) {
+  uint32_t z0, z1, z2, z3;
+  uint64_t k;
+  mul_pre_core(split(x), split(w), split(wq), z0, z1, z2, z3, k);
+  q.k |= k;
+  q.top = max(q.top, z3);
+  return join(z0, z1, z2, z3);
+}
+
+__device__ __forceinline__ void mul_pre_x2(felt a, felt w, felt wq, felt c, felt u, felt uq, felt& aw, felt& cu) {
+  uint32_t z[4], Z[4];
+  uint64_t k1, k2;
+  mul_pre_x2_core(split(a), split(w), split(wq), split(c), split(u), split(uq), z, Z, k1, k2);
+  const uint64_t rare = k1 | k2 | __builtin_amdgcn_ballot_w64(max(z[3], Z[3]) == 0xffffffffu);
+  if (rare) {
+    aw = canon_from(z[0], z[1], z[2], z[3], k1);
+    cu = canon_from(Z[0], Z[1], Z[2], Z[3], k2);
+  } else {
+    aw = join(z[0], z[1], z[2], z[3]);
+    cu = join(Z[0], Z[1], Z[2], Z[3]);
+  }
+}
+
+__device__ __forceinline__ void mul_pre_x2_z(felt a, felt w, felt wq, felt c, felt u, felt uq, felt& aw, felt& cu,
+                                             Rare& q) {
+  uint32_t z[4], Z[4];
+  uint64_t k1, k2;
+  mul_pre_x2_core(split(a), split(w), split(wq), split(c), split(u), split(uq), z, Z, k1, k2);
+  q.k |= k1 | k2;
+  q.top = max(q.top, max(z[3], Z[3]));
+  aw = join(z[0], z[1], z[2], z[3]);
+  cu = join(Z[0], Z[1], Z[2], Z[3]);
+}
+
 __device__ __forceinline__ felt add_z(felt a, felt b, Rare& q) {
   L4 x = split(a), y = split(b);
   uint64_t c, g;
diff --git a/zk_stark_project_amd/csrc/kernels_common.hpp b/zk_stark_project_amd/csrc/kernels_common.hpp
--- a/zk_stark_project_amd/csrc/kernels_common.hpp
+++ b/zk_stark_project_amd/csrc/kernels_common.hpp
@@ -32,6 +32,17 @@
 #endif
   (void)q;
   return mul(a, b);
+}
+template <bool FAST>
+__device__ __forceinline__ felt dmul_pre(felt a, felt w, felt wq, Rare& q) {
+#if defined(__HIP_DEVICE_COMPILE__)
+  if constexpr (FAST) return fpd::mul_pre_z(a, w, wq, q);
+  else return fpd::mul_pre(a, w, wq);
+#else
+  (void)q;
+  (void)wq;
+  return mul(a, w);
+#endif
 }
 template <bool FAST>
 __device__ __forceinline__ felt dadd(felt a, felt b, Rare& q) {
diff --git a/zk_stark_project_amd/csrc/ntt.hip b/zk_stark_project_amd/csrc/ntt.hip
--- a/zk_stark_project_amd/csrc/ntt.hip
+++ b/zk_stark_project_amd/csrc/ntt.hip
@@ -84,17 +84,23 @@
   felt* dst;
   const felt* scale;
   const felt* tw;
+  const felt* twq;
   uint64_t src_stride, dst_stride;
   uint32_t src_div, scale_mod;
   uint32_t logn, s0, K, lo, logT, logTl;
   uint32_t tile_major;
 };
 
+struct Tw {
+  felt w, q;
+};
+
 template <bool DIT>
-__device__ __forceinline__ felt ntt_tw(const Ntt8Args& a, uint32_t j, uint32_t pbit) {
+__device__ __forceinline__ Tw ntt_tw(const Ntt8Args& a, uint32_t j, uint32_t pbit) {
   uint32_t s = DIT ? a.s0 + pbit : a.s0 + a.K - 1 - pbit;
   uint32_t lev = DIT ? s : a.logn - 1 - s;
-  return a.tw[((1u << lev) - 1) + j];
+  const uint32_t i = ((1u << lev) - 1) + j;
+  return {a.tw[i], a.twq[i]};
 }
 
 #ifdef ZKP_NTT_NOGMEM
@@ -113,26 +119,30 @@
 template <bool FAST>
 __device__ __forceinline__ felt bmul(felt a, felt b, Rare& q) { return make(a.lo ^ b.lo, a.hi ^ b.hi); }
 template <bool FAST>
+__device__ __forceinline__ felt bmul_tw(felt a, Tw t, Rare& q) { return make(a.lo ^ t.w.lo ^ t.q.lo, a.hi ^ t.w.hi ^ t.q.hi); }
+template <bool FAST>
 __device__ __forceinline__ felt badd(felt a, felt b, Rare& q) { return make(a.lo + b.lo, a.hi + b.hi); }
 __device__ __forceinline__ felt nsub(felt a, felt b) { return make(a.lo - b.lo, a.hi - b.hi); }
 #else
 template <bool FAST>
 __device__ __forceinline__ felt bmul(felt a, felt b, Rare& q) { return dmul<FAST>(a, b, q); }
 template <bool FAST>
+__device__ __forceinline__ felt bmul_tw(felt a, Tw t, Rare& q) { return dmul_pre<FAST>(a, t.w, t.q, q); }
+template <bool FAST>
 __device__ __forceinline__ felt badd(felt a, felt b, Rare& q) { return dadd<FAST>(a, b, q); }
 __device__ __forceinline__ felt nsub(felt a, felt b) { return sub(a, b); }
 #endif
 
 template <bool DIT, bool FAST>
-__device__ __forceinline__ void bfly(felt& x, felt& y, felt w, Rare& q) {
+__device__ __forceinline__ void bfly(felt& x, felt& y, Tw w, Rare& q) {
   if (DIT) {
-    felt t = bmul<FAST>(y, w, q);
+    felt t = bmul_tw<FAST>(y, w, q);
     y = nsub(x, t);
     x = badd<FAST>(x, t, q);
   } else {
     felt d = nsub(x, y);
     x = badd<FAST>(x, y, q);
-    y = bmul<FAST>(d, w, q);
+    y = bmul_tw<FAST>(d, w, q);
   }
 }
 
@@ -172,11 +182,11 @@
 };
 
 template <bool DIT, bool FAST>
-__device__ __forceinline__ void bfly2(felt& x0, felt& y0, felt w0, felt& x1, felt& y1, felt w1, Rare& q) {
+__device__ __forceinline__ void bfly2(felt& x0, felt& y0, Tw w0, felt& x1, felt& y1, Tw w1, Rare& q) {
 #if defined(__HIP_DEVICE_COMPILE__) && !defined(ZKP_NTT_NOBFLY)
-  auto mx2 = [&](felt a, felt b, felt c, felt d, felt& ab, felt& cd) {
-    if constexpr (FAST) fpd::mul_x2_z(a, b, c, d, ab, cd, q);
-    else fpd::mul_x2(a, b, c, d, ab, cd);
+  auto mx2 = [&](felt a, Tw b, felt c, Tw d, felt& ab, felt& cd) {
+    if constexpr (FAST) fpd::mul_pre_x2_z(a, b.w, b.q, c, d.w, d.q, ab, cd, q);
+    else fpd::mul_pre_x2(a, b.w, b.q, c, d.w, d.q, ab, cd);
   };
   if (DIT) {
     felt t0, t1;
@@ -303,56 +313,56 @@
       constexpr bool smallest = SMALL && (DIT ? first : last);
       if constexpr (DIT && smallest) {
         bfly1<true, FAST>(x[0], x[1], qq); bfly1<true, FAST>(x[2], x[3], qq); bfly1<true, FAST>(x[4], x[5], qq); bfly1<true, FAST>(x[6], x[7], qq);
-        const felt w1 = ntt_tw<true>(a, 1 + zo, 1);
+        const Tw w1 = ntt_tw<true>(a, 1 + zo, 1);
         bfly1<true, FAST>(x[0], x[2], qq); bfly1<true, FAST>(x[4], x[6], qq);
         bfly2<true, FAST>(x[1], x[3], w1, x[5], x[7], w1, qq);
-        const felt w21 = ntt_tw<true>(a, 1 + zo, 2), w22 = ntt_tw<true>(a, 2 + zo, 2), w23 = ntt_tw<true>(a, 3 + zo, 2);
+        const Tw w21 = ntt_tw<true>(a, 1 + zo, 2), w22 = ntt_tw<true>(a, 2 + zo, 2), w23 = ntt_tw<true>(a, 3 + zo, 2);
         bfly1<true, FAST>(x[0], x[4], qq);
         bfly2<true, FAST>(x[1], x[5], w21, x[2], x[6], w22, qq);
         bfly<true, FAST>(x[3], x[7], w23, qq);
       } else if constexpr (!DIT && smallest) {
-        const felt w21 = ntt_tw<false>(a, 1 + zo, 2), w22 = ntt_tw<false>(a, 2 + zo, 2), w23 = ntt_tw<false>(a, 3 + zo, 2);
+        const Tw w21 = ntt_tw<false>(a, 1 + zo, 2), w22 = ntt_tw<false>(a, 2 + zo, 2), w23 = ntt_tw<false>(a, 3 + zo, 2);
         bfly1<false, FAST>(x[0], x[4], qq);
         bfly2<false, FAST>(x[1], x[5], w21, x[2], x[6], w22, qq);
         bfly<false, FAST>(x[3], x[7], w23, qq);
-        const felt w1 = ntt_tw<false>(a, 1 + zo, 1);
+        const Tw w1 = ntt_tw<false>(a, 1 + zo, 1);
         bfly1<false, FAST>(x[0], x[2], qq); bfly1<false, FAST>(x[4], x[6], qq);
         bfly2<false, FAST>(x[1], x[3], w1, x[5], x[7], w1, qq);
         bfly1<false, FAST>(x[0], x[1], qq); bfly1<false, FAST>(x[2], x[3], qq); bfly1<false, FAST>(x[4], x[5], qq); bfly1<false, FAST>(x[6], x[7], qq);
       } else if constexpr (DIT) {
         {
-          felt w0 = ntt_tw<true>(a, jb, b0);
+          Tw w0 = ntt_tw<true>(a, jb, b0);
           bfly2<true, FAST>(x[0], x[1], w0, x[2], x[3], w0, qq); bfly2<true, FAST>(x[4], x[5], w0, x[6], x[7], w0, qq);
         }
         {
-          felt w1a = ntt_tw<true>(a, jb, b0 + 1);
-          felt w1b = ntt_tw<true>(a, jb | jstep, b0 + 1);
+          Tw w1a = ntt_tw<true>(a, jb, b0 + 1);
+          Tw w1b = ntt_tw<true>(a, jb | jstep, b0 + 1);
           bfly2<true, FAST>(x[0], x[2], w1a, x[1], x[3], w1b, qq); bfly2<true, FAST>(x[4], x[6], w1a, x[5], x[7], w1b, qq);
         }
         static_for<0, 2>([&](auto k2) {
-          felt w2a = ntt_tw<true>(a, jb | ((uint32_t)(2 * k2) << (b0 + lo)), b0 + 2);
-          felt w2b = ntt_tw<true>(a, jb | ((uint32_t)(2 * k2 + 1) << (b0 + lo)), b0 + 2);
+          Tw w2a = ntt_tw<true>(a, jb | ((uint32_t)(2 * k2) << (b0 + lo)), b0 + 2);
+          Tw w2b = ntt_tw<true>(a, jb | ((uint32_t)(2 * k2 + 1) << (b0 + lo)), b0 + 2);
           bfly2<true, FAST>(x[2 * k2], x[2 * k2 + 4], w2a, x[2 * k2 + 1], x[2 * k2 + 5], w2b, qq);
         });
       } else {
         static_for<0, 2>([&](auto k2) {
-          felt w2a = ntt_tw<false>(a, jb | ((uint32_t)(2 * k2) << (b0 + lo)), b0 + 2);
-          felt w2b = ntt_tw<false>(a, jb | ((uint32_t)(2 * k2 + 1) << (b0 + lo)), b0 + 2);
+          Tw w2a = ntt_tw<false>(a, jb | ((uint32_t)(2 * k2) << (b0 + lo)), b0 + 2);
+          Tw w2b = ntt_tw<false>(a, jb | ((uint32_t)(2 * k2 + 1) << (b0 + lo)), b0 + 2);
           bfly2<false, FAST>(x[2 * k2], x[2 * k2 + 4], w2a, x[2 * k2 + 1], x[2 * k2 + 5], w2b, qq);
         });
         {
-          felt w1a = ntt_tw<false>(a, jb, b0 + 1);
-          felt w1b = ntt_tw<false>(a, jb | jstep, b0 + 1);
+          Tw w1a = ntt_tw<false>(a, jb, b0 + 1);
+          Tw w1b = ntt_tw<false>(a, jb | jstep, b0 + 1);
           bfly2<false, FAST>(x[0], x[2], w1a, x[1], x[3], w1b, qq); bfly2<false, FAST>(x[4], x[6], w1a, x[5], x[7], w1b, qq);
         }
         {
-          felt w0 = ntt_tw<false>(a, jb, b0);
+          Tw w0 = ntt_tw<false>(a, jb, b0);
           bfly2<false, FAST>(x[0], x[1], w0, x[2], x[3], w0, qq); bfly2<false, FAST>(x[4], x[5], w0, x[6], x[7], w0, qq);
         }
       }
     } else if constexpr (rb == 2) {
       if constexpr (!DIT && SMALL && last) {
-        const felt w1 = ntt_tw<false>(a, 1 + zo, 1);
+        const Tw w1 = ntt_tw<false>(a, 1 + zo, 1);
 #pragma unroll
         for (int u = 0; u < 2; u++) {
           felt* y = x + 4 * u;
@@ -365,8 +375,8 @@
       for (int u = 0; u < 2; u++) {
         const uint32_t l = l0 + (ggs[u] & (Tl - 1));
         const uint32_t jb = (qlow[u] << lo) | l;
-        felt w0 = ntt_tw<DIT>(a, jb, b0);
-        felt w1a = ntt_tw<DIT>(a, jb, b0 + 1), w1b = ntt_tw<DIT>(a, jb | (1u << (b0 + lo)), b0 + 1);
+        Tw w0 = ntt_tw<DIT>(a, jb, b0);
+        Tw w1a = ntt_tw<DIT>(a, jb, b0 + 1), w1b = ntt_tw<DIT>(a, jb | (1u << (b0 + lo)), b0 + 1);
         felt* y = x + 4 * u;
         if (DIT) {
           bfly2<true, FAST>(y[0], y[1], w0, y[2], y[3], w0, qq);
@@ -426,6 +436,17 @@
   ntt8_tile<DIT, NT, KC, SMALL>(a, bidx, tile, lds);
 }
 
+__global__ __launch_bounds__(TPB) void k_build_twq(felt* __restrict__ twq, const felt* __restrict__ tw, uint64_t count) {
+  const uint64_t i = (uint64_t)blockIdx.x * TPB + threadIdx.x;
+  if (i < count) twq[i] = mul(tw[i], make(0, 1));
+}
+
+}
+
+void launch_build_twq(Prof& prof, hipStream_t s, felt* twq, const felt* tw, uint64_t count) {
+  if (count == 0) return;
+  LAUNCH(prof, "build_twq", s, (double)count * 32.0,
+         hipLaunchKernelGGL(k_build_twq, dim3((uint32_t)((count + TPB - 1) / TPB)), dim3(TPB), 0, s, twq, tw, count));
 }
 
 void preload_ntt_module() {
@@ -491,7 +512,7 @@
   X(false, 256, 9, false) X(false, 512, 9, false)
 
 void launch_ntt(Prof& prof, hipStream_t s, const NttBatch& b, uint32_t logn, bool dit, const felt* tw,
-                uint32_t logN, int only_pass) {
+                uint32_t logN, int only_pass, const felt* twq) {
   if (logN > 28)
     launch_fail(ZKP_ERR_TRACE_SHAPE, "NTT domain over 2^28 points (n * blowup)");
   if (logn < 11) {
@@ -512,6 +533,14 @@
     attr_devs |= 1ull << (dev & 63);
   }
   }
+  felt* own_twq = nullptr;
+  if (!twq) {
+    const uint64_t count = (1ull << logn) - 1;
+    if (hipMalloc((void**)&own_twq, count * sizeof(felt)) != hipSuccess)
+      launch_fail(ZKP_ERR_DEVICE, "NTT: no memory for the twiddle companions");
+    launch_build_twq(prof, s, own_twq, tw, count);
+    twq = own_twq;
+  }
   const NttPlan plan = ntt_plan(logn, dit, b.batches);
   for (uint32_t p = 0; p < plan.n; p++) {
     const NttPass& ps = plan.pass[p];
@@ -522,6 +551,7 @@
     a.dst = b.dst;
     a.scale = first ? b.scale : nullptr;
     a.tw = tw;
+    a.twq = twq;
     a.src_stride = first ? b.src_stride : b.dst_stride;
     a.dst_stride = b.dst_stride;
     a.src_div = first ? b.src_div : 1;
@@ -550,4 +580,8 @@
     launch_fail(ZKP_ERR_DEVICE, "internal: NTT pass of an unplanned size");
 #undef X
   }
-}
+  if (own_twq) {
+    (void)hipStreamSynchronize(s);
+    (void)hipFree(own_twq);
+  }
+}
diff --git a/zk_stark_project_amd/csrc/prover.cpp b/zk_stark_project_amd/csrc/prover.cpp
--- a/zk_stark_project_amd/csrc/prover.cpp
+++ b/zk_stark_project_amd/csrc/prover.cpp
@@ -167,9 +167,9 @@
         continue;
       }
       NttBatch ib{dcol, coef + (size_t)c0 * n, nullptr, n, n, 1, 1, cw};
-      launch_ntt(pf, st, ib, logn, false, ctx->itws(logN), logN);
+      launch_ntt(pf, st, ib, logn, false, ctx->itws(logN), logN, -1, ctx->itwqs(logN, logn));
       NttBatch lb{coef + (size_t)c0 * n, tlde + (size_t)c0 * Bl * n, Sj0, n, n, Bl, Bl, cw * Bl};
-      launch_ntt(pf, st, lb, logn, true, ctx->tws(logN), logN);
+      launch_ntt(pf, st, lb, logn, true, ctx->tws(logN), logN, -1, ctx->twqs(logN, logn));
     }
     if (late_pairs) {
       HIP_CHECK(hipStreamWaitEvent(st, ctx->up_ev[G], 0));
@@ -236,7 +236,7 @@
     felt* cint = derive ? ctx->buf<felt>("comp_int", (size_t)(cel ? cel : 1) * n) : comp;
     if (cel) {
       NttBatch ib{comp, cint, nullptr, n, n, 1, 1, cel};
-      launch_ntt(pf, st, ib, logn, false, ctx->itws(logN), logN);
+      launch_ntt(pf, st, ib, logn, false, ctx->itws(logN), logN, -1, ctx->itwqs(logN, logn));
     }
     felt* recv = cint;
     if (R > 1) recv = composition_exchange(cint, nR);
@@ -265,7 +265,7 @@
       composition_gather_lde(slice, derive, nR, p0);
     } else {
       NttBatch lb{acoef, clde, Sj0, n, n, Bl, Bl, (derive ? C - 1 : C) * Bl};
-      launch_ntt(pf, st, lb, logn, true, ctx->tws(logN), logN);
+      launch_ntt(pf, st, lb, logn, true, ctx->tws(logN), logN, -1, ctx->twqs(logN, logn));
     }
     LastCol lc{};
     if (derive) lc = LastCol{comp, last_col_kappa(ctx, logn, logB, C) + 2 * (size_t)j0, clde + (size_t)(C - 1) * Bl * n};
diff --git a/zk_stark_project_amd/csrc/prover_internal.hpp b/zk_stark_project_amd/csrc/prover_internal.hpp
--- a/zk_stark_project_amd/csrc/prover_internal.hpp
+++ b/zk_stark_project_amd/csrc/prover_internal.hpp
@@ -234,6 +234,28 @@
   }
   felt* tws(uint32_t logN) { return reinterpret_cast<felt*>(bufs["tw_" + std::to_string(logN)].p); }
   felt* itws(uint32_t logN) { return reinterpret_cast<felt*>(bufs["itw_" + std::to_string(logN)].p); }
+  std::map<uint32_t, uint32_t> have_twq;
+  void ensure_twq(uint32_t logN, uint32_t logn) {
+    ensure_twiddles(logN);
+    if (logn > logN) logn = logN;
+    auto it = have_twq.find(logN);
+    if (it != have_twq.end() && it->second >= logn) return;
+    const uint64_t count = (1ull << logn) - 1;
+    for (int dir = 0; dir < 2; dir++) {
+      felt* q = buf<felt>((dir ? "itwq_" : "twq_") + std::to_string(logN), count);
+      launch_build_twq(prof, stream, q, dir ? itws(logN) : tws(logN), count);
+    }
+    sync();
+    have_twq[logN] = logn;
+  }
+  const felt* twqs(uint32_t logN, uint32_t logn) {
+    ensure_twq(logN, logn);
+    return reinterpret_cast<felt*>(bufs["twq_" + std::to_string(logN)].p);
+  }
+  const felt* itwqs(uint32_t logN, uint32_t logn) {
+    ensure_twq(logN, logn);
+    return reinterpret_cast<felt*>(bufs["itwq_" + std::to_string(logN)].p);
+  }
   felt* tw(uint32_t logN) { return tws(logN) + ((1ull << (logN - 1)) - 1); }
   felt* itw(uint32_t logN) { return itws(logN) + ((1ull << (logN - 1)) - 1); }
 
@@ -242,7 +264,7 @@
     auto key = std::make_tuple(logn, logB, logce);
     if (have_coset[key]) return;
     uint32_t logN = logn + logB;
-    ensure_twiddles(logN);
+    ensure_twq(logN, logn);
     uint64_t n = 1ull << logn;
     felt g = felt_u64(3);
     for (int dir = 0; dir < 2; dir++) {
diff --git a/zk_stark_project_amd/csrc/prover_shard.cpp b/zk_stark_project_amd/csrc/prover_shard.cpp
--- a/zk_stark_project_amd/csrc/prover_shard.cpp
+++ b/zk_stark_project_amd/csrc/prover_shard.cpp
@@ -77,14 +77,14 @@
       h_partial = true;
     }
     NttBatch ib{dcol, own + (size_t)k * cpr * n, nullptr, n, n, 1, 1, cpr};
-    launch_ntt(pf, ctx->copy, ib, logn, false, ctx->itws(logN), logN);
+    launch_ntt(pf, ctx->copy, ib, logn, false, ctx->itws(logN), logN, -1, ctx->itwqs(logN, logn));
     HIP_CHECK(hipEventRecord(ctx->up_ev[k], ctx->copy));
     HIP_CHECK(hipStreamWaitEvent(ctx->side, ctx->up_ev[k], 0));
     cm->all_gather(ctx->side, own + (size_t)k * cpr * n, coef + c0 * n, (size_t)cpr * n * 16);
     HIP_CHECK(hipEventRecord(ctx->up_ev[K + k], ctx->side));
     HIP_CHECK(hipStreamWaitEvent(st, ctx->up_ev[K + k], 0));
     NttBatch lb{coef + c0 * n, tlde + c0 * Bl * n, Sj0, n, n, Bl, Bl, R * cpr * Bl};
-    launch_ntt(pf, st, lb, logn, true, ctx->tws(logN), logN);
+    launch_ntt(pf, st, lb, logn, true, ctx->tws(logN), logN, -1, ctx->twqs(logN, logn));
   }
   HIP_CHECK(hipEventRecord(ctx->up_ev[2 * K], ctx->copy));
   HIP_CHECK(hipStreamWaitEvent(st, ctx->up_ev[2 * K], 0));
@@ -156,7 +156,7 @@
     on_copy = on_copy || ls == ctx->copy;
     HIP_CHECK(hipStreamWaitEvent(ls, ctx->up_ev[m], 0));
     NttBatch lb{acoef + (size_t)m * n, clde + (size_t)m * Bl * n, Sj0, n, n, Bl, Bl, Bl};
-    launch_ntt(pf, ls, lb, logn, true, ctx->tws(logN), logN);
+    launch_ntt(pf, ls, lb, logn, true, ctx->tws(logN), logN, -1, ctx->twqs(logN, logn));
   }
   if (on_copy) {
     HIP_CHECK(hipEventRecord(ctx->up_ev[C], ctx->copy));
diff --git a/zk_stark_project_amd/csrc/prover_stages.cpp b/zk_stark_project_amd/csrc/prover_stages.cpp
--- a/zk_stark_project_amd/csrc/prover_stages.cpp
+++ b/zk_stark_project_amd/csrc/prover_stages.cpp
@@ -255,7 +255,7 @@
           const uint64_t k = n / sv[j].stride;
           if (cnt && k > 1) {
             NttBatch ib{vals + off, ntt + off, nullptr, k, k, 1, 1, (uint32_t)cnt};
-            launch_ntt(pf, st, ib, ilog2(k), false, ctx->itws(logN), logN);
+            launch_ntt(pf, st, ib, ilog2(k), false, ctx->itws(logN), logN, -1, ctx->itwqs(logN, ilog2(k)));
           } else if (cnt) {
             HIP_CHECK(hipMemcpyAsync(ntt + off, vals + off, cnt * 16, hipMemcpyDeviceToDevice, st));
           }
@@ -329,7 +329,7 @@
       felt* wev = ctx->buf<felt>("strided_w_ev", (size_t)qa.ngroups * cel * n);
       launch_strided_combine(pf, st, qa, logn, wc);
       NttBatch eb{wc, wev, sce_rows() + (uint64_t)u0 * n, n, n, cel, cel, qa.ngroups * cel};
-      launch_ntt(pf, st, eb, logn, true, ctx->tws(logN), logN);
+      launch_ntt(pf, st, eb, logn, true, ctx->tws(logN), logN, -1, ctx->twqs(logN, logn));
       for (uint32_t gi = 0; gi < sa.ngroups; gi++)
         if (wslot[gi] >= 0) sa.W[gi] = wev + (size_t)wslot[gi] * cel * n;
     }
@@ -363,7 +363,7 @@
     const felt* Sce = sce_rows();
     felt* ev = ctx->buf<felt>("lin_ev", (size_t)narr * cel * n);
     NttBatch eb{lc, ev, Sce + (uint64_t)u0 * n, n, n, cel, cel, narr * cel};
-    launch_ntt(pf, st, eb, logn, true, ctx->tws(logN), logN);
+    launch_ntt(pf, st, eb, logn, true, ctx->tws(logN), logN, -1, ctx->twqs(logN, logn));
     launch_eval_linear_pts(pf, st, ec, la, ev, comp);
   };
   if (air.id == ZKP_AIR_MIMC) {
@@ -453,7 +453,7 @@
   }
   felt* alde = ctx->buf<felt>("deep_alde", (size_t)Bl * n);
   NttBatch lb{acomb, alde, Sj0, n, n, Bl, Bl, Bl};
-  launch_ntt(ctx->prof, st, lb, da.logn, true, ctx->tws(logN), logN);
+  launch_ntt(ctx->prof, st, lb, da.logn, true, ctx->tws(logN), logN, -1, ctx->twqs(logN, da.logn));
   const std::string g1key = "deep_g1_" + std::to_string(da.C);
   felt* g1 = ctx->buf<felt>(g1key, (size_t)da.C + 1);
   if (!ctx->have_cached(g1key)) {
diff --git a/zk_stark_project_amd/csrc/zkp_internal.hpp b/zk_stark_project_amd/csrc/zkp_internal.hpp
--- a/zk_stark_project_amd/csrc/zkp_internal.hpp
+++ b/zk_stark_project_amd/csrc/zkp_internal.hpp
@@ -40,7 +40,8 @@
 };
 
 void launch_ntt(Prof& prof, hipStream_t s, const NttBatch& b, uint32_t logn, bool dit, const felt* tw,
-                uint32_t logN, int only_pass = -1);
+                uint32_t logN, int only_pass = -1, const felt* twq = nullptr);
+void launch_build_twq(Prof& prof, hipStream_t s, felt* twq, const felt* tw, uint64_t count);
 
 void launch_build_levels(Prof& prof, hipStream_t s, felt* tab, uint32_t top);
 void launch_expand_powers(Prof& prof, hipStream_t s, felt* out, uint64_t count, const felt* lo_tab,
```

New measurement: 231.8 proofs/s, median of 3. Within noise of the previous version (+0.3%).
